# GPflow/GPflow

Measured on AMD Instinct MI355X. Metric: svgp_elbo_steps_per_s, higher is better.
Workload: dtype f64; 1 GPU; SVGP RBF(ARD)+Gaussian ELBO, N=1e+06 M=2048 D=8 P=1 whitened, 8192 minibatch rows per GPU per step (BASELINE metric config Cm); global_batch=8192

## Files before the change

gpflow_amd/_lib.py:

```python
from __future__ import annotations

import ctypes as C
import os
from typing import Optional

_HERE = os.path.dirname(os.path.abspath(__file__))
_LIB_PATH = os.environ.get("GPK_LIBRARY") or os.path.join(_HERE, "libgpk.so")

c_void_p, c_int, c_long, c_double, c_size_t = C.c_void_p, C.c_int, C.c_long, C.c_double, C.c_size_t
_dp = C.c_void_p


class GpkError(RuntimeError):
    pass


_SIGS = {
    "gpk_version": (C.c_char_p, []),
    "gpk_kernel_matrix": (c_int, [c_void_p, c_int, _dp, c_int, c_long, _dp, c_int, c_long, c_int,
                                  C.POINTER(c_double), c_int, c_double, c_double, c_int, _dp, c_long]),
    "gpk_kernel_matrix_hadamard": (c_int, [c_void_p, c_int, _dp, c_int, c_long, _dp, c_int, c_long, c_int,
                                           C.POINTER(c_double), c_int, c_double, _dp, c_long, _dp, c_long]),
    "gpk_kernel_matrix_combine": (c_int, [c_void_p, c_int, c_int, _dp, c_int, c_long, _dp, c_int, c_long, c_int,
                                          C.POINTER(c_double), c_int, c_double, c_double, _dp, c_long, _dp, c_long]),
    "gpk_diag_add": (c_int, [c_void_p, _dp, c_int, c_long, _dp]),
    "gpk_invd_elems": (c_size_t, [c_int, c_int]),
    "gpk_potrf": (c_int, [c_void_p, _dp, c_int, c_int, c_long, c_int, c_long, _dp, c_int, _dp]),
    "gpk_combine_parts": (c_int, [c_void_p, _dp, c_int, c_long, c_int, c_int, c_long, c_double, c_int, c_double, _dp, c_long]),
    "gpk_stream_selfcheck": (c_int, [C.POINTER(c_double), C.POINTER(c_double), C.POINTER(c_int)]),
    "gpk_chain_handoff_mode": (c_int, []),
    "gpk_potrf_inv": (c_int, [c_void_p, _dp, c_int, c_int, c_long, _dp, c_int, _dp]),
    "gpk_trtri_blocks": (c_int, [c_void_p, _dp, c_int, c_long, c_int, c_long, _dp]),
    "gpk_trsm": (c_int, [c_void_p, c_int, _dp, c_long, _dp, c_int, _dp, c_int, c_long, c_int, c_long,
                         c_long]),
    "gpk_transpose_factor": (c_int, [c_void_p, _dp, c_long, _dp, c_int, _dp, c_long, _dp]),
    "gpk_gemm_nt": (c_int, [c_void_p, c_int, c_int, c_int, c_double, _dp, c_long, _dp, c_long, c_double,
                            _dp, c_long, c_int, c_int, c_int, c_long, c_long, c_long]),
    "gpk_transpose": (c_int, [c_void_p, _dp, c_int, c_int, c_long, _dp, c_long, c_int, c_int, c_long,
                              c_long]),
    "gpk_row_stats": (c_int, [c_void_p, _dp, c_int, c_int, c_long, _dp, _dp, c_int, c_double, c_double,
                              _dp, _dp, _dp]),
    "gpk_row_dot": (c_int, [c_void_p, _dp, c_long, _dp, c_long, c_int, c_int, c_double, c_double, _dp]),
    "gpk_row_sumsq": (c_int, [c_void_p, _dp, c_int, c_int, c_long, c_double, c_double, _dp]),
    "gpk_project_workspace_bytes": (c_size_t, [c_int, c_int, c_int]),
    "gpk_project": (c_int, [c_void_p, _dp, c_int, c_int, c_long, _dp, c_long, c_int, _dp, _dp, c_size_t]),
    "gpk_project_batched": (c_int, [c_void_p, _dp, c_int, c_int, c_long, c_long, _dp, c_long, c_int, _dp, _dp, c_size_t]),
    "gpk_reduce_workspace_bytes": (c_size_t, [c_int]),
    "gpk_gaussian_varexp_sum": (c_int, [c_void_p, _dp, c_long, _dp, c_int, c_int, _dp, c_int, _dp,
                                        C.POINTER(c_double), c_int, c_double, _dp, c_double, _dp, _dp, _dp,
                                        c_size_t]),
    "gpk_likelihood_varexp_sum": (c_int, [c_void_p, c_int, C.POINTER(c_double), _dp, c_long, _dp, c_int, c_int, _dp, c_int, _dp,
                                          C.POINTER(c_double), c_int, c_double, _dp, _dp, _dp, _dp, _dp, _dp, c_size_t]),
    "gpk_gauss_hermite": (c_int, [c_int, C.POINTER(c_double), C.POINTER(c_double)]),
    "gpk_gauss_kl_white": (c_int, [c_void_p, _dp, _dp, c_int, c_int, c_int, _dp, _dp, c_size_t]),
    "gpk_sum_log_diag": (c_int, [c_void_p, _dp, c_int, c_long, c_int, c_long, _dp]),
    "gpk_sumsq": (c_int, [c_void_p, _dp, c_int, c_int, c_long, c_int, _dp, _dp, c_size_t]),
    "gpk_gpr_lml_workspace_bytes": (c_size_t, [c_int, c_int, c_int]),
    "gpk_gpr_lml": (c_int, [c_void_p, c_int, _dp, c_int, c_int, c_long, _dp, c_int, c_long,
                            C.POINTER(c_double), c_int, c_double, c_double, _dp, c_double, _dp, _dp, _dp,
                            c_size_t]),
    "gpk_svgp_elbo_workspace_bytes": (c_size_t, [c_int, c_int, c_int, c_int, c_int, c_int]),
    "gpk_svgp_elbo_shard": (c_int, [c_void_p, c_int, _dp, c_int, c_long, _dp, _dp, c_int, c_long, c_long,
                                    c_int, c_int, C.POINTER(c_double), c_int, c_double, c_double, _dp,
                                    c_double, c_double, _dp, _dp, c_int, c_int, _dp, _dp, _dp, c_size_t]),
    "gpk_svgp_elbo_shard_lik": (c_int, [c_void_p, c_int, _dp, c_int, c_long, _dp, _dp, c_int, c_long, c_long, c_int, c_int,
                                        C.POINTER(c_double), c_int, c_double, c_int, C.POINTER(c_double), c_double, c_double,
                                        _dp, _dp, c_int, c_int, _dp, _dp, _dp, c_size_t]),
    "gpk_svgp_elbo_sep_workspace_bytes": (c_size_t, [c_int, c_int, c_int, c_int]),
    "gpk_svgp_elbo_shard_sep": (c_int, [c_void_p, C.POINTER(c_int), _dp, c_int, c_long, c_long, _dp, _dp, c_int, c_long, c_long,
                                        c_int, c_int, C.POINTER(c_double), c_int, C.POINTER(c_double), c_double, _dp, c_double,
                                        c_double, _dp, _dp, _dp, _dp, _dp, c_size_t]),
    "gpk_moment_rows": (c_int, [c_void_p, _dp, c_long, c_int, c_int, _dp, c_long]),
    "gpk_stationary_adjoint_tail": (c_int, [c_void_p, _dp, c_long, _dp, c_long, c_int, c_int, _dp, c_double, c_int, _dp, _dp, c_long,
                                            _dp, c_int, c_double]),
    "gpk_adam_step": (c_int, [c_void_p, _dp, _dp, _dp, _dp, c_long, c_double, c_double, c_double, c_double, c_int]),
    "gpk_lowrank_axpy": (c_int, [c_void_p, c_double, _dp, c_long, _dp, c_long, _dp, c_long, c_int, c_int, c_int, _dp, c_long]),
    "gpk_symmetrize": (c_int, [c_void_p, _dp, c_int, c_long]),
    "gpk_publish_host": (c_int, [c_void_p, _dp, c_int, _dp, c_void_p, c_int]),
    "gpk_profile_gemm_enable": (None, [c_int]),
    "gpk_profile_gemm_collect": (c_int, [C.POINTER(c_double), C.POINTER(c_long), C.POINTER(c_double)]),
    "gpk_profile_gemm_collect_min": (c_int, [c_double, c_int, C.POINTER(c_double), C.POINTER(c_long), C.POINTER(c_double)]),
    "gpk_profile_gemm_collect_kind": (c_int, [c_int, c_double, C.POINTER(c_double), C.POINTER(c_long), C.POINTER(c_double)]),
    "gpk_profile_gemm_window": (c_int, [c_double, C.POINTER(c_double), C.POINTER(c_double), C.POINTER(c_double),
                                        C.POINTER(c_long)]),
    "gpk_bench_mfma_f64": (c_int, [c_void_p, c_int, c_int, _dp]),
    "gpk_bench_stream_store": (c_int, [c_void_p, _dp, c_long]),
}

EXPORTED_SYMBOLS = tuple(sorted(_SIGS))

_lib: Optional[C.CDLL] = None


def lib_path() -> str:
    return _LIB_PATH


def load() -> C.CDLL:
    global _lib
    if _lib is not None:
        return _lib
    if not os.path.exists(_LIB_PATH):
        raise ImportError(
            f"{_LIB_PATH} not found: the HIP extension is not built. Run "
            "`python -c 'import __graft_entry__ as g; g.build()'` (or `make -C gpflow_amd/csrc`). "
            "gpflow_amd has no CPU fallback."
        )
    lib = C.CDLL(_LIB_PATH)
    for name, (res, args) in _SIGS.items():
        fn = getattr(lib, name)
        fn.restype = res
        fn.argtypes = args
    _lib = lib
    return lib


def check(rc: int, what: str) -> None:
    if rc == 0:
        return
    if rc < 0:
        names = {-1: "GPK_E_ARG (bad argument)", -2: "GPK_E_WORKSPACE (workspace too small)",
                 -3: "GPK_E_UNSUPPORTED"}
        raise GpkError(f"{what}: {names.get(rc, rc)}")
    raise GpkError(f"{what}: HIP runtime error {rc}")


def host_doubles(values):
    arr = (c_double * len(values))(*[float(v) for v in values])
    return arr
```

gpflow_amd/csrc/drivers.hip:

```cpp
#include "gpk_internal.h"

extern "C" size_t gpk_project_workspace_bytes(int rows, int m, int P) {
  return (size_t)P * 2 * gpk_gemm_tiles_n(m) * rows * sizeof(double);
}

namespace {
int project_parts(hipStream_t s, const double* At, int rows, int m, long ldat, long strideAt, const double* LqT, long ldl, int P, void* ws,
                  size_t ws_bytes) {
  if ((!At && rows > 0) || !LqT || rows < 0 || m <= 0 || P <= 0 || strideAt < 0) return GPK_E_ARG;
  if (!ws || ws_bytes < gpk_project_workspace_bytes(rows, m, P)) return GPK_E_WORKSPACE;
  if (rows == 0) return 0;
  const int nt = 2 * gpk_gemm_tiles_n(m);
  GemmArgs g = gemm_base(rows, m, m, 1.0, At, ldat, LqT, ldl, 0.0, nullptr, 0, P, strideAt, (long)m * ldl, 0);
  g.b_tri = 1;
  g.epi = 1; g.sq_cols = m; g.c2_cols = 0;
  g.part = (double*)ws; g.part_ld = rows; g.stridePart = (long)nt * rows;
  g.C2 = (double*)ws; g.ldc2 = 0; g.strideC2 = 0;
  return gpk_launch_gemm(s, g);
}
}

extern "C" int gpk_project_batched(void* stream, const double* At, int rows, int m, long ldat, long strideAt,
                                   const double* LqT, long ldl, int P, double* ssq, void* ws, size_t ws_bytes) {
  if (!ssq && rows > 0) return GPK_E_ARG;
  hipStream_t s = (hipStream_t)stream;
  const int rc = project_parts(s, At, rows, m, ldat, strideAt, LqT, ldl, P, ws, ws_bytes);
  if (rc || rows == 0) return rc;
  const int nt = 2 * gpk_gemm_tiles_n(m);
  return gpk_launch_sum_parts(s, (const double*)ws, nt, rows, (long)nt * rows, P, ssq);
}

extern "C" int gpk_project(void* stream, const double* At, int rows, int m, long ldat,
                           const double* LqT, long ldl, int P, double* ssq, void* ws,
                           size_t ws_bytes) {
  return gpk_project_batched(stream, At, rows, m, ldat, 0, LqT, ldl, P, ssq, ws, ws_bytes);
}

namespace {
struct Carver {
  uintptr_t base;
  size_t used = 0;
  double* take(size_t bytes) {
    double* p = (double*)(base + used);
    used += gpk_align_up(bytes, 256);
    return p;
  }
};

int final_one(hipStream_t s, const double* part, int count, double scale, double add, double* out) {
  return gpk_launch_final(s, 1, &part, &count, &scale, add, out);
}
}

namespace {
struct LmlWs {
  long ld;
  double *T, *invd, *part, *logdet;
  size_t total;
};
LmlWs lml_layout(void* ws, int n, int P) {
  LmlWs w{};
  Carver c{(uintptr_t)ws};
  w.ld = (long)gpk_align_up((size_t)n, 8);
  w.T = c.take((size_t)(n + P) * w.ld * sizeof(double));
  w.invd = c.take(gpk_invd_elems(n, 1) * sizeof(double));
  w.part = c.take((size_t)GPK_REDUCE_MAXPART * sizeof(double));
  w.logdet = c.take(256);
  w.total = c.used;
  return w;
}
}

extern "C" size_t gpk_gpr_lml_workspace_bytes(int n, int d, int P) {
  (void)d;
  return lml_layout(nullptr, n, P).total;
}

extern "C" int gpk_gpr_lml(void* stream, int family, const double* X, int n, int d, long ldx,
                           const double* Y, int P, long ldy, const double* ls_host, int ard,
                           double variance, double noise_variance, const double* noise_rows, double mean_const,
                           double* out, int* info, void* ws, size_t ws_bytes) {
  if (!X || !Y || !out || !info || n <= 0 || P <= 0) return GPK_E_ARG;
  const LmlWs w = lml_layout(ws, n, P);
  if (!ws || ws_bytes < w.total) return GPK_E_WORKSPACE;
  hipStream_t s = (hipStream_t)stream;
  int rc;
  rc = gpk_kernel_matrix(stream, family, X, n, ldx, nullptr, 0, 0, d, ls_host, ard, variance,
                         noise_rows ? 0.0 : noise_variance, 1, w.T, w.ld);
  if (rc) return rc;
  if (noise_rows) {
    rc = gpk_diag_add(stream, w.T, n, w.ld, noise_rows);
    if (rc) return rc;
  }
  double* alphaT = w.T + (long)n * w.ld;
  rc = gpk_launch_transpose_shift(s, Y, n, P, ldy, alphaT, w.ld, -mean_const);
  if (rc) return rc;
  rc = gpk_potrf_core(s, w.T, n, P, w.ld, 1, 0, w.invd, 0, info);
  if (rc) return rc;
  rc = gpk_sum_log_diag(stream, w.T, n, w.ld, 1, 0, w.logdet);
  if (rc) return rc;
  int cnt = 0;
  rc = gpk_launch_sumsq_stage1(s, alphaT, P, n, w.ld, 0, w.part, &cnt);
  if (rc) return rc;
  const double* parts[2] = {w.part, w.logdet};
  const int counts[2] = {cnt, 1};
  const double scales[2] = {-0.5, -(double)P};
  const double add = -0.5 * (double)n * (double)P * 1.8378770664093453;
  return gpk_launch_final(s, 2, parts, counts, scales, add, out);
}

namespace {
struct KernelDesc {
  int family, d;
  const double* ls_host;
  int ard;
  double variance;
};
struct ElboArgs {
  KernelDesc k;
  const double* Z; int m; long ldz;
  const double *Xb, *Yb; int rows; long ldxb, ldyb;
  int P;
  const double *q_mu, *q_sqrt; int q_diag;
  double noise_variance; const double* noise_rows;
  double jitter, mean_const;
  double* out; int* info;
  int lik = 0;
  const double* lik_params = nullptr;
};
struct ElboWs {
  long ld, strideT;
  double* T;
  double* Kfu;
  double* arow;
  double* LqT;
  double *invd, *s0, *fmean, *ssq;
  double* proj;
  double *part0, *part1;
  double* part2;
  double* V;
  size_t total;
};

ElboWs elbo_layout(void* ws, int m, int rows, int P, int q_diag, int whiten) {
  ElboWs w{};
  Carver c{(uintptr_t)ws};
  w.ld = (long)gpk_align_up((size_t)m, 8);
  const size_t rows_pad = gpk_align_up((size_t)rows, 32);
  const size_t tail_rows = q_diag ? (whiten ? 0 : (size_t)P + m + 32) : (size_t)P + (size_t)P * m + 32;
  w.T = c.take((m + rows_pad + tail_rows) * w.ld * sizeof(double));
  w.Kfu = w.T + (long)m * w.ld;
  w.arow = w.T + (long)(m + (whiten ? rows_pad : (size_t)rows)) * w.ld;
  w.LqT = w.arow + (long)P * w.ld;
  w.invd = c.take(gpk_invd_elems(m, 1) * sizeof(double));
  w.s0 = c.take((size_t)rows * sizeof(double));
  w.fmean = c.take((size_t)rows * P * sizeof(double));
  w.ssq = c.take((size_t)rows * P * sizeof(double));
  w.proj = c.take(q_diag ? (whiten ? 0 : (size_t)rows * w.ld * sizeof(double)) : gpk_project_workspace_bytes(rows, m, P));
  w.part0 = c.take((size_t)GPK_REDUCE_MAXPART * sizeof(double));
  w.part1 = c.take((size_t)GPK_REDUCE_MAXPART * sizeof(double));
  w.part2 = c.take((size_t)(GPK_REDUCE_MAXPART + 64) * sizeof(double));
  w.V = c.take((size_t)m * P * sizeof(double));
  w.total = c.used;
  return w;
}

ElboWs elbo_sep_layout(void* ws, int m, int rows, int P) {
  ElboWs w{};
  Carver c{(uintptr_t)ws};
  w.ld = (long)gpk_align_up((size_t)m, 8);
  w.strideT = (long)(m + rows) * w.ld;
  w.T = c.take((size_t)P * w.strideT * sizeof(double));
  w.Kfu = w.T + (long)m * w.ld;
  w.invd = c.take(gpk_invd_elems(m, P) * sizeof(double));
  w.LqT = c.take((size_t)P * m * w.ld * sizeof(double));
  w.s0 = c.take((size_t)rows * P * sizeof(double));
  w.fmean = c.take((size_t)rows * P * sizeof(double));
  w.ssq = c.take((size_t)rows * P * sizeof(double));
  w.proj = c.take(gpk_project_workspace_bytes(rows, m, P));
  w.part0 = c.take((size_t)GPK_REDUCE_MAXPART * sizeof(double));
  w.part1 = c.take((size_t)GPK_REDUCE_MAXPART * sizeof(double));
  w.total = c.used;
  return w;
}

bool side_schedule(int m, int rows) { return m > GPK_NB && m < 4096 && rows > 256; }

int build_kuu(hipStream_t ps, const KernelDesc& k, const ElboArgs& a, const double* Z, double* T, long ld) {
  return gpk_kernel_matrix((void*)ps, k.family, Z, a.m, a.ldz, nullptr, 0, 0, k.d, k.ls_host, k.ard, k.variance, a.jitter, 1, T, ld);
}
int build_kfu(hipStream_t xs, const KernelDesc& k, const ElboArgs& a, const double* Z, double* Kfu, long ld) {
  return gpk_kernel_matrix((void*)xs, k.family, a.Xb, a.rows, a.ldxb, Z, a.m, a.ldz, k.d, k.ls_host, k.ard, k.variance, 0.0, 0, Kfu, ld);
}
typedef decltype(&build_kuu) BuildFn;
int build_kfu_and_q_mu_rows(hipStream_t xs, const ElboArgs& a, const ElboWs& w) {
  const int r = build_kfu(xs, a.k, a, a.Z, w.Kfu, w.ld);
  if (r) return r;
  return gpk_transpose((void*)xs, a.q_mu, a.m, a.P, a.P, w.arow, w.ld, 0, 1, 0, 0);
}
int transpose_q_sqrt(hipStream_t s, const ElboArgs& a, const ElboWs& w) {
  return gpk_transpose((void*)s, a.q_sqrt, a.m, a.m, a.m, w.LqT, w.ld, 1, a.P, (long)a.m * a.m, (long)a.m * w.ld);
}

int varexp_to_out(hipStream_t s, const ElboArgs& a, const ElboWs& w, const double* knn_host, int per_latent) {
  int count = 0;
  const int rc = a.lik
      ? gpk_launch_likelihood_varexp_stage1(s, a.lik, a.lik_params, a.Yb, a.ldyb, w.fmean, a.rows, a.P, w.s0, per_latent, w.ssq,
                                            knn_host, per_latent, a.mean_const, nullptr, nullptr, nullptr, nullptr, w.part0, nullptr,
                                            &count)
      : gpk_launch_varexp_stage1(s, a.Yb, a.ldyb, w.fmean, a.rows, a.P, w.s0, per_latent, w.ssq, knn_host, per_latent,
                                 a.noise_variance, a.mean_const, nullptr, w.part0, &count, a.noise_rows);
  if (rc) return rc;
  return final_one(s, w.part0, count, 1.0, 0.0, a.out);
}
int kl_white_to_out(hipStream_t s, const ElboArgs& a, const ElboWs& w) {
  int count = 0;
  const int rc = gpk_launch_kl_white_stage1(s, a.q_mu, a.q_sqrt, a.m, a.P, a.q_diag, w.part1, &count);
  if (rc) return rc;
  return final_one(s, w.part1, count, 0.5, -0.5 * (double)a.m * (double)a.P, a.out + 1);
}
int transpose_q_sqrt_and_kl(hipStream_t s, const ElboArgs& a, const ElboWs& w) {
  if (!a.q_diag) {
    const int r = transpose_q_sqrt(s, a, w);
    if (r) return r;
  }
  return kl_white_to_out(s, a, w);
}

int elbo_whitened(hipStream_t s, const ElboArgs& a, const ElboWs& w) {
  const bool side = side_schedule(a.m, a.rows);
  PotrfHooks hk;
  hk.p_prologue = [&a, &w](hipStream_t ps) { return build_kuu(ps, a.k, a, a.Z, w.T, w.ld); };
  hk.x_prologue = [&a, &w](hipStream_t xs) { return build_kfu(xs, a.k, a, a.Z, w.Kfu, w.ld); };
  if (side) hk.late_work = [&a, &w](hipStream_t bs) { return transpose_q_sqrt_and_kl(bs, a, w); };
  int rc = gpk_potrf_core(s, w.T, a.m, a.rows, w.ld, 1, 0, w.invd, 0, a.info, hk);
  if (rc) return rc;
  rc = gpk_row_stats((void*)s, w.Kfu, a.rows, a.m, w.ld, a.q_mu, a.q_diag ? a.q_sqrt : nullptr, a.P, 1.0, 0.0, w.s0, w.fmean,
                     a.q_diag ? w.ssq : nullptr);
  if (rc) return rc;
  if (!a.q_diag) {
    if (!side) {
      rc = transpose_q_sqrt(s, a, w);
      if (rc) return rc;
    }
    rc = gpk_project((void*)s, w.Kfu, a.rows, a.m, w.ld, w.LqT, w.ld, a.P, w.ssq, w.proj, gpk_project_workspace_bytes(a.rows, a.m, a.P));
    if (rc) return rc;
  }
  rc = varexp_to_out(s, a, w, &a.k.variance, 0);
  if (rc || side) return rc;
  return kl_white_to_out(s, a, w);
}

int elbo_unwhitened_full(hipStream_t s, const ElboArgs& a, const ElboWs& w) {
  const int m = a.m, P = a.P;
  PotrfHooks hk;
  hk.p_prologue = [&a, &w](hipStream_t ps) { return build_kuu(ps, a.k, a, a.Z, w.T, w.ld); };
  hk.x_prologue = [&a, &w](hipStream_t xs) {
    const int r = build_kfu_and_q_mu_rows(xs, a, w);
    return r ? r : transpose_q_sqrt(xs, a, w);
  };
  int rc = gpk_potrf_core(s, w.T, m, a.rows + P + P * m, w.ld, 1, 0, w.invd, 0, a.info, hk, P == 1 ? m : 0, true);
  if (rc) return rc;
  rc = gpk_transpose((void*)s, w.arow, P, m, w.ld, w.V, P, 0, 1, 0, 0);
  if (rc) return rc;
  rc = gpk_row_stats((void*)s, w.Kfu, a.rows, m, w.ld, w.V, nullptr, P, 1.0, 0.0, w.s0, w.fmean, nullptr);
  if (rc) return rc;
  rc = gpk_project((void*)s, w.Kfu, a.rows, m, w.ld, w.LqT, w.ld, P, w.ssq, w.proj, gpk_project_workspace_bytes(a.rows, m, P));
  if (rc) return rc;
  rc = varexp_to_out(s, a, w, &a.k.variance, 0);
  if (rc) return rc;
  int cm = 0, ct = 0;
  rc = gpk_launch_sumsq_stage1(s, w.arow, P, m, w.ld, 0, w.part1, &cm);
  if (rc) return rc;
  rc = gpk_launch_sumsq_stage1(s, w.LqT, P * m, m, w.ld, 0, w.part2, &ct);
  if (rc) return rc;
  double* ldq = w.part2 + GPK_REDUCE_MAXPART;
  double* ldl = ldq + P;
  rc = gpk_launch_sum_log_diag_sq(s, a.q_sqrt, m, m, P, (long)m * m, ldq);
  if (rc) return rc;
  rc = gpk_sum_log_diag((void*)s, w.T, m, w.ld, 1, 0, ldl);
  if (rc) return rc;
  const double* kp[4] = {w.part1, w.part2, ldq, ldl};
  const int kc[4] = {cm, ct, P, 1};
  const double ks[4] = {0.5, 0.5, -0.5, (double)P};
  return gpk_launch_final(s, 4, kp, kc, ks, -0.5 * (double)m * (double)P, a.out + 1);
}

int elbo_unwhitened_diag(hipStream_t s, const ElboArgs& a, const ElboWs& w) {
  const int m = a.m, P = a.P, rows = a.rows;
  double* A2 = w.proj;
  PotrfHooks hk;
  hk.p_prologue = [&a, &w](hipStream_t ps) { return build_kuu(ps, a.k, a, a.Z, w.T, w.ld); };
  hk.x_prologue = [&a, &w](hipStream_t xs) { return build_kfu_and_q_mu_rows(xs, a, w); };
  int rc = gpk_potrf_core(s, w.T, m, rows + P + m, w.ld, 1, 0, w.invd, 0, a.info, hk, m);
  if (rc) return rc;
  if (rows > 0) {
    GemmArgs g = gemm_base(rows, m, m, 1.0, w.Kfu, w.ld, w.LqT, w.ld, 0.0, A2, w.ld, 1, 0, 0, 0);
    g.b_tri = 1;
    rc = gpk_launch_gemm(s, g);
    if (rc) return rc;
    rc = gpk_row_sumsq((void*)s, w.Kfu, rows, m, w.ld, 1.0, 0.0, w.s0);
    if (rc) return rc;
    rc = gpk_row_stats((void*)s, A2, rows, m, w.ld, a.q_mu, a.q_sqrt, P, 1.0, 0.0, nullptr, w.fmean, w.ssq);
    if (rc) return rc;
  }
  rc = varexp_to_out(s, a, w, &a.k.variance, 0);
  if (rc) return rc;
  int cm = 0, ct = 0;
  rc = gpk_launch_sumsq_stage1(s, w.arow, P, m, w.ld, 0, w.part1, &cm);
  if (rc) return rc;
  rc = gpk_launch_kl_unwhite_diag_stage1(s, w.LqT, w.ld, m, a.q_sqrt, P, w.part2, &ct);
  if (rc) return rc;
  double* ldl = w.part2 + GPK_REDUCE_MAXPART;
  rc = gpk_sum_log_diag((void*)s, w.T, m, w.ld, 1, 0, ldl);
  if (rc) return rc;
  const double* kp[3] = {w.part1, w.part2, ldl};
  const int kc[3] = {cm, ct, 1};
  const double ks[3] = {0.5, 0.5, (double)P};
  return gpk_launch_final(s, 3, kp, kc, ks, -0.5 * (double)m * (double)P, a.out + 1);
}
}

extern "C" size_t gpk_svgp_elbo_workspace_bytes(int m, int rows, int d, int P, int q_diag, int whiten) {
  (void)d;
  return elbo_layout(nullptr, m, rows, P, q_diag, whiten).total;
}

namespace {
int elbo_shard(void* stream, const ElboArgs& a, int whiten, void* ws, size_t ws_bytes) {
  if (!a.Z || (a.rows > 0 && (!a.Xb || !a.Yb)) || !a.q_mu || !a.q_sqrt || !a.out || !a.info || a.m <= 0 || a.rows < 0 || a.P <= 0 ||
      a.P > 16)
    return GPK_E_ARG;
  if (a.lik) {
    const int rc = gpk_likelihood_check(a.lik, a.lik_params);
    if (rc) return rc;
  }
  const ElboWs w = elbo_layout(ws, a.m, a.rows, a.P, a.q_diag, whiten);
  if (!ws || ws_bytes < w.total) return GPK_E_WORKSPACE;
  hipStream_t s = (hipStream_t)stream;
  if (whiten) return elbo_whitened(s, a, w);
  return a.q_diag ? elbo_unwhitened_diag(s, a, w) : elbo_unwhitened_full(s, a, w);
}
}

extern "C" int gpk_svgp_elbo_shard(void* stream, int family, const double* Z, int m, long ldz,
                                   const double* Xb, const double* Yb, int rows, long ldxb,
                                   long ldyb, int d, int P, const double* ls_host, int ard,
                                   double variance, double noise_variance, const double* noise_rows, double jitter,
                                   double mean_const, const double* q_mu, const double* q_sqrt,
                                   int q_diag, int whiten, double* out, int* info, void* ws,
                                   size_t ws_bytes) {
  const ElboArgs a{{family, d, ls_host, ard, variance}, Z, m, ldz, Xb, Yb, rows, ldxb, ldyb, P, q_mu, q_sqrt, q_diag,
                   noise_variance, noise_rows, jitter, mean_const, out, info};
  return elbo_shard(stream, a, whiten, ws, ws_bytes);
}

extern "C" int gpk_svgp_elbo_shard_lik(void* stream, int family, const double* Z, int m, long ldz, const double* Xb,
                                       const double* Yb, int rows, long ldxb, long ldyb, int d, int P, const double* ls_host,
                                       int ard, double variance, int lik, const double* lik_params_host, double jitter,
                                       double mean_const, const double* q_mu, const double* q_sqrt, int q_diag, int whiten,
                                       double* out, int* info, void* ws, size_t ws_bytes) {
  if (!lik) return GPK_E_UNSUPPORTED;
  ElboArgs a{{family, d, ls_host, ard, variance}, Z, m, ldz, Xb, Yb, rows, ldxb, ldyb, P, q_mu, q_sqrt, q_diag,
             0.0, nullptr, jitter, mean_const, out, info};
  a.lik = lik; a.lik_params = lik_params_host;
  return elbo_shard(stream, a, whiten, ws, ws_bytes);
}

extern "C" size_t gpk_svgp_elbo_sep_workspace_bytes(int m, int rows, int d, int P) {
  (void)d;
  return elbo_sep_layout(nullptr, m, rows, P).total;
}

extern "C" int gpk_svgp_elbo_shard_sep(void* stream, const int* family_host, const double* Z, int m, long ldz, long strideZ,
                                       const double* Xb, const double* Yb, int rows, long ldxb, long ldyb, int d, int P,
                                       const double* ls_host, int ard, const double* variance_host, double noise_variance,
                                       const double* noise_rows, double jitter, double mean_const, const double* q_mu,
                                       const double* q_sqrt, double* out,
                                       int* info, void* ws, size_t ws_bytes) {
  if (!family_host || !Z || (rows > 0 && (!Xb || !Yb)) || !q_mu || !q_sqrt || !ls_host || !variance_host || !out || !info || m <= 0 || rows < 0 ||
      P <= 0 || P > 16 || d <= 0 || strideZ < 0)
    return GPK_E_ARG;
  const ElboWs w = elbo_sep_layout(ws, m, rows, P);
  if (!ws || ws_bytes < w.total) return GPK_E_WORKSPACE;
  const ElboArgs a{{0, d, ls_host, ard, 0.0}, Z, m, ldz, Xb, Yb, rows, ldxb, ldyb, P, q_mu, q_sqrt, 0,
                   noise_variance, noise_rows, jitter, mean_const, out, info};
  hipStream_t s = (hipStream_t)stream;
  const int nls = ard ? d : 1;
  auto each_latent = [&](BuildFn build, hipStream_t st, double* T0) -> int {
    for (int p = 0; p < P; ++p) {
      const KernelDesc kp{family_host[p], d, ls_host + (long)p * nls, ard, variance_host[p]};
      const int r = build(st, kp, a, Z + (long)p * strideZ, T0 + (long)p * w.strideT, w.ld);
      if (r) return r;
    }
    return 0;
  };
  const bool side = side_schedule(m, rows);
  PotrfHooks hk;
  hk.p_prologue = [&](hipStream_t ps) { return each_latent(build_kuu, ps, w.T); };
  hk.x_prologue = [&](hipStream_t xs) { return each_latent(build_kfu, xs, w.Kfu); };
  if (side) hk.late_work = [&a, &w](hipStream_t bs) { return transpose_q_sqrt_and_kl(bs, a, w); };
  int rc = gpk_potrf_core(s, w.T, m, rows, w.ld, P, w.strideT, w.invd, 0, info, hk);
  if (rc) return rc;
  if (!side) {
    rc = transpose_q_sqrt_and_kl(s, a, w);
    if (rc) return rc;
  }
  rc = gpk_launch_row_stats_sep(s, w.Kfu, w.strideT, rows, m, w.ld, q_mu, P, w.s0, w.fmean);
  if (rc) return rc;
  rc = gpk_project_batched(stream, w.Kfu, rows, m, w.ld, w.strideT, w.LqT, w.ld, P, w.ssq, w.proj,
                           gpk_project_workspace_bytes(rows, m, P));
  if (rc) return rc;
  return varexp_to_out(s, a, w, variance_host, 1);
}
```

gpflow_amd/csrc/gemm.hip:

```cpp
#include "gpk_internal.h"
#include <mutex>
#include <stdlib.h>
#include <algorithm>
#include <type_traits>

namespace {

constexpr int BK = 16;
constexpr int LDSS = BK + 2;
thread_local int g_last_kind = 0;
constexpr int GROUP_N = 8;

template <int BM, int BN, int WGM, int WGN>
struct TileCfg {
  static constexpr int WM = BM / WGM, WN = BN / WGN;
  static constexpr int TM = WM / 16, TN = WN / 16;
  static constexpr int A_CH = BM * (BK / 2) / 256;
  static constexpr int B_CH = BN * (BK / 2) / 256;
  static constexpr size_t LDS_BYTES = 2 * (size_t)(BM + BN) * LDSS * sizeof(double);
};

__device__ __forceinline__ void tile_decode(int nl, int gx, int gy, int compact, int& tile_m, int& tile_n) {
  tile_m = 0; tile_n = 0;
  if (compact) {
// ... 282 lines not shown
#pragma unroll
        for (int i = 0; i < TM; ++i)
#pragma unroll
          for (int r = 0; r < 4; ++r) {
            const int row = row_base + i * 16 + 4 * r;
            double s = smem[wn * BM + (row - m0)];
#pragma unroll
            for (int u = 1; u < WPS; ++u) s += smem[(wn + u) * BM + (row - m0)];
            if (row < p.m) part[(long)(tile_n * (BN / 64) + (wn * WN) / 64) * p.part_ld + row] = s;
          }
      }
    }
  }
}


__global__ __launch_bounds__(256, 2) void gemm_nt_pre64(GemmArgs p, int gx, int gy, int total, int compact) {
  constexpr int BM = 64, BN = 64, MAXS = 8;
  constexpr int BUF = (BM + BN) * LDSS;
  extern __shared__ __attribute__((aligned(16))) double smem[];
  if (p.sig_ptr && threadIdx.x == 0 && blockIdx.x == 0 && blockIdx.y == 0)
    __hip_atomic_store(p.sig_ptr, p.sig_val, __ATOMIC_RELAXED, __HIP_MEMORY_SCOPE_SYSTEM);

  const int tid = threadIdx.x, lane = tid & 63, wave = tid >> 6;
  const int bz = blockIdx.y;
  int tile_m, tile_n;
  tile_order(blockIdx.x, 0, gx, gy, total, compact, tile_m, tile_n);
  const int m0 = tile_m * BM, n0 = tile_n * BN;
  if (p.c_lower && n0 > m0 + BM - 1) return;
  if (m0 >= p.m || n0 >= p.n) return;
  const double* __restrict__ A = p.A + (long)bz * p.strideA;
  const double* __restrict__ B = p.B + (long)bz * p.strideB;
  double* __restrict__ C = p.C + (long)bz * p.strideC;
  const int nkt = p.k / BK;

  d2 ra[MAXS][2], rb[MAXS][2];
  const double* pa[2];
  const double* pb[2];
  bool va[2], vb[2];
#pragma unroll
  for (int q = 0; q < 2; ++q) {
    const int c = tid + 256 * q;
    const int rowa = m0 + (c >> 3), rowb = n0 + (c >> 3);
    va[q] = rowa < p.m;
    vb[q] = rowb < p.n;
    pa[q] = A + (long)(va[q] ? rowa : p.m - 1) * p.lda + (c & 7) * 2;
    pb[q] = B + (long)(vb[q] ? rowb : p.n - 1) * p.ldb + (c & 7) * 2;
  }
#pragma unroll
  for (int s = 0; s < MAXS; ++s)
    if (s < nkt) {
#pragma unroll
      for (int q = 0; q < 2; ++q) {
        ra[s][q] = *reinterpret_cast<const d2*>(pa[q] + s * BK);
        rb[s][q] = *reinterpret_cast<const d2*>(pb[q] + s * BK);
      }
    }
  const int row_base = m0 + wave * 16 + (lane >> 4);
  const int col_base = n0 + (lane & 15);
  const double alpha = p.alpha, beta = p.beta;
  double cpre[4][4];
#pragma unroll
  for (int r = 0; r < 4; ++r)
#pragma unroll
    for (int j = 0; j < 4; ++j) {
      const int row = row_base + 4 * r, col = col_base + j * 16;
      cpre[r][j] = (beta != 0.0 && row < p.m && col < p.n) ? C[(long)row * p.ldc + col] : 0.0;
    }

  const d2 zero2 = {0.0, 0.0};
  auto lstore = [&](int buf, const d2 (&xa)[2], const d2 (&xb)[2]) {
#pragma unroll
    for (int q = 0; q < 2; ++q) {
      const int c = tid + 256 * q;
      *reinterpret_cast<d2*>(&smem[buf * BUF + (c >> 3) * LDSS + (c & 7) * 2]) = va[q] ? xa[q] : zero2;
      *reinterpret_cast<d2*>(&smem[buf * BUF + (BM + (c >> 3)) * LDSS + (c & 7) * 2]) = vb[q] ? xb[q] : zero2;
    }
  };
  d4 acc[4];
#pragma unroll
  for (int j = 0; j < 4; ++j) acc[j] = (d4){0.0, 0.0, 0.0, 0.0};
  if (nkt > 0) {
    lstore(0, ra[0], rb[0]);
    __syncthreads();
  }
  const int frag_r = lane & 15, frag_k = lane >> 4;
#pragma unroll
  for (int kt = 0; kt < MAXS; ++kt)
    if (kt < nkt) {
      const int cur = kt & 1;
      const double* as = smem + cur * BUF + (wave * 16 + frag_r) * LDSS + frag_k;
      const double* bs = smem + cur * BUF + (BM + frag_r) * LDSS + frag_k;
#pragma unroll
      for (int kk = 0; kk < BK / 4; ++kk) {
        const double a = as[kk * 4];
        double b[4];
#pragma unroll
        for (int j = 0; j < 4; ++j) b[j] = bs[j * 16 * LDSS + kk * 4];
#pragma unroll
        for (int j = 0; j < 4; ++j) acc[j] = __builtin_amdgcn_mfma_f64_16x16x4f64(a, b[j], acc[j], 0, 0, 0);
      }
      if (kt + 1 < MAXS && kt + 1 < nkt) lstore(cur ^ 1, ra[kt + 1 < MAXS ? kt + 1 : 0], rb[kt + 1 < MAXS ? kt + 1 : 0]);
      __syncthreads();
    }
#pragma unroll
  for (int r = 0; r < 4; ++r) {
    const int row = row_base + 4 * r;
    if (row < p.m) {
#pragma unroll
      for (int j = 0; j < 4; ++j) {
        const int col = col_base + j * 16;
        if (col < p.n) {
          double v = alpha * acc[j][r];
          if (beta != 0.0) v += beta * cpre[r][j];
          C[(long)row * p.ldc + col] = v;
        }
      }
    }
  }
}

bool pre64_ok(const GemmArgs& a) {
  if (a.epi != 0 || a.k <= 0 || a.k > 128 || (a.k & 15) || a.b_tri || a.a_tri || a.k_off_step || a.tile_snake || a.tail_first1) return false;
  if ((a.lda & 1) || (a.ldb & 1) || (a.strideA & 1) || (a.strideB & 1)) return false;
  if ((reinterpret_cast<uintptr_t>(a.A) & 15) || (reinterpret_cast<uintptr_t>(a.B) & 15)) return false;
  return true;
}

int launch_pre64(hipStream_t s, const GemmArgs& a) {
  constexpr size_t LDS_BYTES = 2 * (size_t)(64 + 64) * LDSS * sizeof(double);
  const int gx = gpk_cdiv(a.n, 64), gy = gpk_cdiv(a.m, 64);
  if (gx <= 0 || gy <= 0) return 0;
  int total = gx * gy, compact = 0;
  if (a.c_lower) {
    compact = 1;
    total = 0;
    for (int first = 0; first < gx; first += GROUP_N) {
      const int gsz = (gx - first) < GROUP_N ? (gx - first) : GROUP_N;
      const int avail = gy - first;
      if (avail <= 0) break;
      const int tr = avail < gsz ? avail : gsz;
      total += tr * (tr + 1) / 2 + (avail > gsz ? (avail - gsz) * gsz : 0);
    }
    if (total <= 0) return 0;
  }
  g_last_kind = 6;
  hipLaunchKernelGGL(gemm_nt_pre64, dim3((unsigned)total, (unsigned)(a.batch > 0 ? a.batch : 1), 1), dim3(256), LDS_BYTES, s, a, gx, gy,
                     total, compact);
  GPK_LAUNCH_CHECK();
  return 0;
}


template <int EPI>
__device__ __forceinline__ void fast_tile(const GemmArgs& p, int tile_m, int tile_n, double* smem, int rev = 0, int bz_queue = -1) {
  constexpr int BM = 128, BN = 128;
  constexpr int BUF = (BM + BN) * LDSS;
  const int tid = threadIdx.x, lane = tid & 63, wave = tid >> 6;
  const int wm = wave >> 1, wn = wave & 1;
  const int bz = bz_queue >= 0 ? bz_queue : (p.k_off_step ? (int)gridDim.y - 1 - (int)blockIdx.y : (int)blockIdx.y);
  const int m0 = tile_m * BM, n0 = tile_n * BN;
  if (p.c_lower && n0 > m0 + BM - 1) return;

  const double* __restrict__ A = p.A + (long)bz * p.strideA;
  const double* __restrict__ B = p.B + (long)bz * p.strideB;
  int kb = 0, ke = p.k;
  const int koff = bz * p.k_off_step;
  if (p.b_tri && (n0 + BN < p.n ? n0 + BN : p.n) <= p.b_tri_rows) {
    if (p.b_tri == 1) {
      const int f = n0 + p.b_tri_off - koff;
      kb = (f > 0 ? f : 0) & ~(BK - 1);
    } else {
      const int l = n0 + BN + p.b_tri_off - koff;
      ke = l < p.k ? l : p.k;
    }
  }
  if (p.a_tri == 1) {
    int f = m0 - koff;
    f = (f > 0 ? f : 0) & ~(BK - 1);
    kb = kb > f ? kb : f;
  } else if (p.a_tri == 2) {
    int l = ((m0 + BM + BK - 1) & ~(BK - 1)) - koff;
    l = l < p.k ? l : p.k;
    ke = ke < l ? ke : l;
  }
  const int nk = ke > kb ? (ke - kb) / BK : 0;

  const int srow = tid >> 3, scol = (tid & 7) * 2;
  const int mrows = p.m - m0, nrows = p.n - n0;
  const char* abase = reinterpret_cast<const char*>(A + (long)m0 * p.lda + kb);
  const char* bbase = reinterpret_cast<const char*>(B + (long)n0 * p.ldb + kb);
  unsigned oa[4], ob[4];
#pragma unroll
  for (int q = 0; q < 4; ++q) {
    int ra = srow + 32 * q, rb = srow + 32 * q;
    ra = ra < mrows ? ra : mrows - 1;
    rb = rb < nrows ? rb : nrows - 1;
    oa[q] = (unsigned)(((long)ra * p.lda + scol) * 8);
    ob[q] = (unsigned)(((long)rb * p.ldb + scol) * 8);
  }
  const int woff = srow * LDSS + scol;
  d2 st[8];
  auto gload = [&](int s) {
    const long so = rev ? (long)(nk - 1 - s) : (long)s;
    const char* ab = abase + so * (BK * 8);
    const char* bb = bbase + so * (BK * 8);
#pragma unroll
    for (int q = 0; q < 4; ++q) st[q] = *reinterpret_cast<const d2*>(ab + oa[q]);
#pragma unroll
    for (int q = 0; q < 4; ++q) st[4 + q] = *reinterpret_cast<const d2*>(bb + ob[q]);
  };
  auto lstore1 = [&](int buf, int q) {
    const int row = (q < 4) ? 32 * q : BM + 32 * (q - 4);
    *reinterpret_cast<d2*>(&smem[buf * BUF + row * LDSS + woff]) = st[q];
  };

  d4 acc[4][4];
  const int lane_c = lane & 15, lane_g = lane >> 4;
  const int row_base = m0 + wm * 64 + lane_c;
  const int col_base = n0 + wn * 64 + 2 * lane_g;
  const bool load_c = (p.beta != 0.0) && (EPI == 0 || p.C != nullptr);
  if (nk > 0) gload(0);
  const int c_r0 = wm * 64 + lane_c, c_c0 = wn * 64 + 2 * lane_g;
  const int c_rmax = p.m - 1 - m0, c_cmax = p.n - 1 - n0;
  auto c_roff = [&](int i) -> unsigned {
    const int rr = c_r0 + 16 * i;
    return (unsigned)(((long)(rr < c_rmax ? rr : c_rmax) * p.ldc) * 8);
  };
  auto c_coff = [&](int j, int h) -> unsigned {
    const int c = c_c0 + j * 16 + 8 * h;
    return (unsigned)((c < c_cmax ? c : c_cmax) * 8);
  };
  const bool c_vec = (EPI == 0 || p.C != nullptr) && (n0 + BN <= p.n) && !(p.ldc & 1) && !(p.strideC & 1) &&
                     !(reinterpret_cast<uintptr_t>(p.C) & 15);
  if (load_c) {
    const double* __restrict__ C = p.C + (long)bz * p.strideC;
    const double sc = p.beta / p.alpha;
    const char* cb = reinterpret_cast<const char*>(C + (long)m0 * p.ldc + n0);
    if (c_vec) {
#pragma unroll
      for (int i = 0; i < 4; ++i) {
        const char* rowp = cb + c_roff(i);
#pragma unroll
        for (int j = 0; j < 4; ++j) {
          const d2 lo = *reinterpret_cast<const d2*>(rowp + c_coff(j, 0));
          const d2 hi = *reinterpret_cast<const d2*>(rowp + c_coff(j, 1));
          acc[i][j] = (d4){sc * lo.x, sc * lo.y, sc * hi.x, sc * hi.y};
        }
      }
    } else {
#pragma unroll
      for (int i = 0; i < 4; ++i) {
        const char* rowp = cb + c_roff(i);
#pragma unroll
        for (int j = 0; j < 4; ++j)
#pragma unroll
          for (int r = 0; r < 4; ++r) {
            const int c = c_c0 + j * 16 + 8 * (r >> 1) + (r & 1);
            acc[i][j][r] = sc * *reinterpret_cast<const double*>(rowp + (unsigned)((c < c_cmax ? c : c_cmax) * 8));
          }
      }
    }
  } else {
#pragma unroll
    for (int i = 0; i < 4; ++i)
#pragma unroll
      for (int j = 0; j < 4; ++j) acc[i][j] = (d4){0.0, 0.0, 0.0, 0.0};
  }

  const int bperm = 2 * (lane_c & 3) + ((lane_c >> 2) & 1) + 8 * (lane_c >> 3);
  const double* as = smem + (wm * 64 + lane_c) * LDSS + lane_g;
  const double* bs = smem + (BM + wn * 64 + bperm) * LDSS + lane_g;
  double fa[2][4], fb[2][4];
  auto fload = [&](int buf, int kk, int f) {
#pragma unroll
    for (int i = 0; i < 4; ++i) fa[f][i] = as[buf * BUF + i * 16 * LDSS + kk * 4];
#pragma unroll
    for (int j = 0; j < 4; ++j) fb[f][j] = bs[buf * BUF + j * 16 * LDSS + kk * 4];
  };
#define GPK_MFMA_ROW(f, i)                                                                         \
  _Pragma("unroll") for (int j = 0; j < 4; ++j) acc[i][j] =                                       \
      __builtin_amdgcn_mfma_f64_16x16x4f64(fb[f][j], fa[f][i], acc[i][j], 0, 0, 0)

  if (nk > 0) {
#pragma unroll
    for (int q = 0; q < 8; ++q) lstore1(0, q);
    __syncthreads();
    fload(0, 0, 0);
  }
  auto slab = [&](int s, auto more_tag) {
    constexpr bool MORE = decltype(more_tag)::value;
    const int cur = s & 1;
    if constexpr (MORE) gload(s + 1);
    fload(cur, 1, 1);
#pragma unroll
    for (int i = 0; i < 4; ++i) { GPK_MFMA_ROW(0, i); }
    if constexpr (MORE) __builtin_amdgcn_sched_group_barrier(0x020, 8, 0);
    __builtin_amdgcn_sched_group_barrier(0x100, 8, 0);
    __builtin_amdgcn_sched_group_barrier(0x008, 16, 0);
    __builtin_amdgcn_sched_barrier(0);
    fload(cur, 2, 0);
#pragma unroll
    for (int i = 0; i < 4; ++i) { GPK_MFMA_ROW(1, i); }
    __builtin_amdgcn_sched_group_barrier(0x100, 8, 0);
    __builtin_amdgcn_sched_group_barrier(0x008, 16, 0);
    __builtin_amdgcn_sched_barrier(0);
    fload(cur, 3, 1);
    if constexpr (MORE) {
#pragma unroll
      for (int q = 0; q < 8; ++q) lstore1(cur ^ 1, q);
    }
#pragma unroll
    for (int i = 0; i < 4; ++i) { GPK_MFMA_ROW(0, i); }
    __builtin_amdgcn_sched_group_barrier(0x100, 8, 0);
    if constexpr (MORE) {
      __builtin_amdgcn_sched_group_barrier(0x008, 4, 0);
#pragma unroll
      for (int q = 0; q < 8; ++q) {
        __builtin_amdgcn_sched_group_barrier(0x200, 1, 0);
        __builtin_amdgcn_sched_group_barrier(0x008, 1, 0);
      }
      __builtin_amdgcn_sched_group_barrier(0x008, 4, 0);
    } else {
      __builtin_amdgcn_sched_group_barrier(0x008, 16, 0);
    }
    __builtin_amdgcn_sched_barrier(0);
    if constexpr (MORE) __syncthreads();
    if constexpr (MORE) fload(cur ^ 1, 0, 0);
#pragma unroll
    for (int i = 0; i < 4; ++i) { GPK_MFMA_ROW(1, i); }
    if constexpr (MORE) __builtin_amdgcn_sched_group_barrier(0x100, 8, 0);
    __builtin_amdgcn_sched_group_barrier(0x008, 16, 0);
    __builtin_amdgcn_sched_barrier(0);
  };
  for (int s = 0; s + 1 < nk; ++s) slab(s, std::true_type{});
  if (nk > 0) slab(nk - 1, std::false_type{});
#undef GPK_MFMA_ROW

  if constexpr (EPI == 0) {
    double* __restrict__ C = p.C + (long)bz * p.strideC;
    const double alpha = p.alpha;
    char* cb = reinterpret_cast<char*>(C + (long)m0 * p.ldc + n0);
#pragma unroll
    for (int i = 0; i < 4; ++i) {
      if (c_r0 + 16 * i <= c_rmax) {
        char* rowp = cb + c_roff(i);
        if (c_vec) {
#pragma unroll
          for (int j = 0; j < 4; ++j) {
            *reinterpret_cast<d2*>(rowp + c_coff(j, 0)) = (d2){alpha * acc[i][j][0], alpha * acc[i][j][1]};
            *reinterpret_cast<d2*>(rowp + c_coff(j, 1)) = (d2){alpha * acc[i][j][2], alpha * acc[i][j][3]};
          }
        } else {
#pragma unroll
          for (int j = 0; j < 4; ++j)
#pragma unroll
            for (int r = 0; r < 4; ++r) {
              const int c = c_c0 + j * 16 + 8 * (r >> 1) + (r & 1);
              if (c <= c_cmax) *reinterpret_cast<double*>(rowp + (unsigned)(c * 8)) = alpha * acc[i][j][r];
            }
        }
      }
    }
  } else {
    double* __restrict__ C2 = p.C2 + (long)bz * p.strideC2;
    double* __restrict__ part = p.part + (long)bz * p.stridePart;
    const double alpha = p.alpha;
#pragma unroll
    for (int i = 0; i < 4; ++i) {
      const int row = row_base + i * 16;
      double s = 0.0;
#pragma unroll
      for (int j = 0; j < 4; ++j)
#pragma unroll
        for (int r = 0; r < 4; ++r) {
          const int col = col_base + j * 16 + 8 * (r >> 1) + (r & 1);
          const double v = alpha * acc[i][j][r];
          if (col < p.sq_cols) {
            s += v * v;
          } else if (row < p.m && col - p.sq_cols < p.c2_cols && col < p.n) {
            C2[(long)row * p.ldc2 + (col - p.sq_cols)] = v;
          }
        }
      s += __shfl_xor(s, 16);
      s += __shfl_xor(s, 32);
      if (lane_g == 0 && row < p.m) part[(long)(tile_n * 2 + wn) * p.part_ld + row] = s;
    }
  }
}


template <int EPI, bool PAIR, bool QUEUE = false>
__global__ __launch_bounds__(256, 2) void gemm_nt_fast(GemmArgs p, int gx, int gy, int total, int compact) {
  extern __shared__ __attribute__((aligned(16))) double smem[];
  if (p.sig_ptr && threadIdx.x == 0 && blockIdx.x == 0 && blockIdx.y == 0)
    __hip_atomic_store(p.sig_ptr, p.sig_val, __ATOMIC_RELAXED, __HIP_MEMORY_SCOPE_SYSTEM);
  if constexpr (!PAIR) {
    if (p.stagger_ticks > 0 && (int)blockIdx.x >= p.stagger_first && (int)blockIdx.x < 2 * p.stagger_first && blockIdx.y == 0) {
      const long long t0 = wall_clock64();
      while (wall_clock64() - t0 < p.stagger_ticks) __builtin_amdgcn_s_sleep(32);
    }
    if constexpr (QUEUE) {
      volatile int* s_next = reinterpret_cast<volatile int*>(&smem[BK]);
      const int nbatch = p.batch > 0 ? p.batch : 1;
      const int all = total * nbatch;
      for (;;) {
        if (threadIdx.x == 0) *s_next = (int)((unsigned)atomicAdd(p.queue, 1) - (unsigned)p.queue_base);
        __syncthreads();
        const int t = *s_next;
        __syncthreads();
        if (t >= all || t < 0) break;
        const int zq = t / total, tq = t - zq * total;
        int tile_m, tile_n;
        tile_order(tq, p.b_tri, gx, gy, total, compact, tile_m, tile_n);
        fast_tile<EPI>(p, tile_m, tile_n, smem, 0, nbatch - 1 - zq);
      }
      return;
    }
    for (int t = blockIdx.x; t < total; t += gridDim.x) {
      int tile_m, tile_n;
      if (EPI == 1 && p.tile_snake) {
        const int q = t / gy, half = gx >> 1;
        tile_m = t - q * gy;
        tile_n = q < half ? q : gx - 1 - (q - half);
      } else if (p.k_off_step) {
        int tt = t + (int)blockIdx.y * (total / (int)gridDim.y);
        if (tt >= total) tt -= total;
        tile_order(tt, p.b_tri, gx, gy, total, compact, tile_m, tile_n);
      } else {
        tile_order(t, p.b_tri, gx, gy, total, compact, tile_m, tile_n);
      }
      fast_tile<EPI>(p, tile_m, tile_n, smem);
      if (t + (int)gridDim.x < total) __syncthreads();
    }
  } else {
    const int align = (EPI == 1 && p.b_tri == 1) ? p.pair_k_align : 0;
    const int tile_m = blockIdx.x % gy, j = blockIdx.x / gy;
    fast_tile<EPI>(p, tile_m, j, smem, align);
    if (gx - 1 - j != j) {
      __syncthreads();
      fast_tile<EPI>(p, tile_m, gx - 1 - j, smem, 0);
    }
  }
}

int queue_slot(unsigned fetches, int** out, unsigned* base) {
  constexpr int kRing = 1024, kMaxDev = 16;
  static std::mutex mu;
  static int* ring[kMaxDev] = {};
  static unsigned* value[kMaxDev] = {};
  static unsigned next[kMaxDev] = {};
  int dev = 0;
  GPK_HIP(hipGetDevice(&dev));
  if (dev < 0 || dev >= kMaxDev) return GPK_E_UNSUPPORTED;
  std::lock_guard<std::mutex> lock(mu);
  if (!ring[dev]) {
    GPK_HIP(hipMalloc((void**)&ring[dev], sizeof(int) * kRing));
    GPK_HIP(hipMemset(ring[dev], 0, sizeof(int) * kRing));
    value[dev] = (unsigned*)calloc(kRing, sizeof(unsigned));
    if (!value[dev]) return GPK_E_ARG;
  }
  const unsigned slot = next[dev]++ % kRing;
  *out = ring[dev] + slot;
  *base = value[dev][slot];
  value[dev][slot] += fetches;
  return 0;
}

template <int EPI>
int launch_fast(hipStream_t s, const GemmArgs& a) {
  constexpr size_t LDS_BYTES = 2 * (size_t)256 * LDSS * sizeof(double);
  static const hipError_t attr0 = hipFuncSetAttribute(reinterpret_cast<const void*>(gemm_nt_fast<EPI, false>),
                                                      hipFuncAttributeMaxDynamicSharedMemorySize, 160 * 1024);
  static const hipError_t attr1 = hipFuncSetAttribute(reinterpret_cast<const void*>(gemm_nt_fast<EPI, true>),
                                                      hipFuncAttributeMaxDynamicSharedMemorySize, (int)LDS_BYTES);
  GPK_HIP(attr0);
  GPK_HIP(attr1);
  const int gx = gpk_cdiv(a.n, 128), gy = gpk_cdiv(a.m, 128);
  if (gx <= 0 || gy <= 0) return 0;
  int total = gx * gy, compact = 0;
  if (a.c_lower && EPI == 0) {
    compact = 1;
    total = 0;
    for (int first = 0; first < gx; first += GROUP_N) {
      const int gsz = (gx - first) < GROUP_N ? (gx - first) : GROUP_N;
      const int avail = gy - first;
      if (avail <= 0) break;
      const int tr = avail < gsz ? avail : gsz;
      total += tr * (tr + 1) / 2 + (avail > gsz ? (avail - gsz) * gsz : 0);
    }
    if (total <= 0) return 0;
  }
  const unsigned nb = (unsigned)(a.batch > 0 ? a.batch : 1);
  {
    const bool pair_ok = (EPI == 1) ? (a.b_tri == 1)
                                    : ((a.b_tri == 1 || a.b_tri == 2) && !a.c_lower && a.max_wgs == 0 && a.b_tri_off == 0 && a.k_off_step == 0);
    if (EPI == 1 && pair_ok && gx >= 4 && !(gx & 1) && a.b_tri_rows >= a.n && a.max_wgs == 0 &&
        (long)(gx / 2) * gy * nb <= GPK_TUNE(PROJ_UNPAIR_UPTO, 256)) {
      GemmArgs b = a;
      b.tile_snake = 1;
      b.stagger_first = 256;
      b.stagger_ticks = 0;
      g_last_kind = 2 + 2 * EPI;
      hipLaunchKernelGGL((gemm_nt_fast<EPI, false>), dim3((unsigned)total, nb, 1), dim3(256), LDS_BYTES, s, b, gx, gy, total, compact);
      GPK_LAUNCH_CHECK();
      return 0;
    }
    if (pair_ok && gx >= 4 && a.b_tri_rows >= a.n) {
      total = ((gx + 1) / 2) * gy;
      g_last_kind = 2 + 2 * EPI + 1;
      GemmArgs ap = a;
      ap.pair_k_align = GPK_TUNE(PAIR_K_ALIGN, 1);
      hipLaunchKernelGGL((gemm_nt_fast<EPI, true>), dim3((unsigned)total, nb, 1), dim3(256), LDS_BYTES, s, ap, gx, gy,
                         total, compact);
      GPK_LAUNCH_CHECK();
      return 0;
    }
  }
  int tail_tiles = 0;
  if (EPI == 0 && !a.c_lower && a.max_wgs > 0 && a.max_wgs < total && nb == 1 && !a.b_tri && !a.a_tri &&
      GPK_TUNE(TAIL_SPLIT_CAPPED, 1)) {
    const int r = total % a.max_wgs;
    if (r > 0 && r * 100 <= a.max_wgs * GPK_TUNE(TAIL_SPLIT_CAPPED_PCT, 60)) tail_tiles = r;
  }
  const int total_all = total;
  total -= tail_tiles;
  unsigned nwg = (unsigned)total;
  if (a.max_wgs > 0 && (unsigned)a.max_wgs < nwg) nwg = (unsigned)a.max_wgs;
  GemmArgs b = a;
  g_last_kind = 2 + 2 * EPI;
  {
    const int stagger_on = GPK_TUNE(GEMM_STAGGER, 100);
    if (b.stagger_first <= 0) b.stagger_first = 256;
    b.stagger_ticks = (stagger_on && EPI == 0 && !a.b_tri && total >= 1024 && (nwg == (unsigned)total || nwg >= 2u * (unsigned)b.stagger_first))
                          ? (int)((a.k / 16) * 170 * stagger_on / 200)
                          : 0;
  }
  size_t lds_bytes = LDS_BYTES;
  if (EPI == 0 && a.max_wgs > 0 && nwg < (unsigned)total && nb == 1) {
    const int kb = GPK_TUNE(CAP_EXCL_LDS_KB, 84);
    if (kb > 0 && kb <= 160 && (size_t)kb * 1024 > LDS_BYTES) lds_bytes = (size_t)kb * 1024;
  }
  if (EPI == 0 && tail_tiles == 0 && a.max_wgs == 0 &&
      ((a.k_off_step && GPK_TUNE(KSPLIT_QUEUE, 1)) || (a.tile_queue && (long)total * nb > 512))) {
    b.stagger_ticks = 0;
    const long all = (long)total * nb;
    const long qw = a.stagger_first > 0 ? 2L * a.stagger_first : GPK_TUNE(QUEUE_WGS, 512);
    const unsigned wgs = (unsigned)(all < qw ? all : qw);
    int* q = nullptr;
    unsigned qbase = 0;
    const int rcq = queue_slot((unsigned)all + wgs, &q, &qbase);
    if (rcq) return rcq;
    b.queue = q;
    b.queue_base = (int)qbase;
    if constexpr (EPI == 0) {
      static const hipError_t attrq = hipFuncSetAttribute(reinterpret_cast<const void*>(gemm_nt_fast<0, false, true>),
                                                          hipFuncAttributeMaxDynamicSharedMemorySize, (int)LDS_BYTES);
      GPK_HIP(attrq);
      hipLaunchKernelGGL((gemm_nt_fast<0, false, true>), dim3(wgs, 1, 1), dim3(256), LDS_BYTES, s, b, gx, gy, total, compact);
    }
    GPK_LAUNCH_CHECK();
    return 0;
  }
  hipLaunchKernelGGL((gemm_nt_fast<EPI, false>), dim3(nwg, nb, 1), dim3(256), lds_bytes, s, b, gx, gy, total,
                     compact);
  GPK_LAUNCH_CHECK();
  if (tail_tiles > 0) {
    using Cfg = TileCfg<64, 64, 4, 1>;
    static const hipError_t attrt = hipFuncSetAttribute(reinterpret_cast<const void*>(gemm_nt_kernel<64, 64, 4, 1>),
                                                        hipFuncAttributeMaxDynamicSharedMemorySize, (int)Cfg::LDS_BYTES);
    GPK_HIP(attrt);
    GemmArgs t = a;
    t.tail_first1 = total_all - tail_tiles + 1;
    hipLaunchKernelGGL((gemm_nt_kernel<64, 64, 4, 1>), dim3((unsigned)(4 * tail_tiles), 1, 1), dim3(256), Cfg::LDS_BYTES, s, t, gx,
                       gy, 4 * tail_tiles, compact);
    GPK_LAUNCH_CHECK();
  }
  return 0;
}

bool fast_ok(const GemmArgs& a) {
  if (GPK_TUNE(GEMM_NO_FAST, 0)) return false;
  if (a.k <= 0 || (a.k & 15) || (a.b_tri && (a.b_tri_off & 15))) return false;
  if ((a.lda & 1) || (a.ldb & 1) || (a.strideA & 1) || (a.strideB & 1)) return false;
  if ((reinterpret_cast<uintptr_t>(a.A) & 15) || (reinterpret_cast<uintptr_t>(a.B) & 15)) return false;
  if (a.epi == 0 && a.beta != 0.0 && a.alpha == 0.0) return false;
  if (a.lda > (1L << 21) || a.ldb > (1L << 21)) return false;
  return true;
}


constexpr int SM_BM = 16, SM_BN = 128, SM_THREADS = 512;

__global__ __launch_bounds__(SM_THREADS) void gemm_nt_small(GemmArgs p, int ldk) {
  extern __shared__ __attribute__((aligned(16))) double smem[];
  const int tid = threadIdx.x, lane = tid & 63;
  const int wave = __builtin_amdgcn_readfirstlane(tid >> 6);
  const int bz = blockIdx.z;
  const int n0 = blockIdx.x * SM_BN;
  const double* __restrict__ A = p.A + (long)bz * p.strideA;
  const double* __restrict__ B = p.B + (long)bz * p.strideB;
  int kb = 0, ke = p.k;
  if (p.b_tri && (n0 + SM_BN < p.n ? n0 + SM_BN : p.n) <= p.b_tri_rows) {
    if (p.b_tri == 1) {
      const int f = n0 + p.b_tri_off;
      kb = (f > 0 ? f : 0) & ~(BK - 1);
    } else {
      const int l = n0 + SM_BN + p.b_tri_off;
      ke = l < p.k ? l : p.k;
    }
  }
  const int kc = ke > kb ? ke - kb : 0;
  double* As = smem;
  double* Bs = smem + SM_BM * ldk;
  const int r = lane & 15, g = lane >> 4;
  const int col = n0 + wave * 16 + r;
  double* __restrict__ C = p.C + (long)bz * p.strideC;
  if (p.sig_ptr && tid == 0 && blockIdx.x == 0 && blockIdx.y == 0 && blockIdx.z == 0)
    __hip_atomic_store(p.sig_ptr, p.sig_val, __ATOMIC_RELAXED, __HIP_MEMORY_SCOPE_SYSTEM);
  if (p.wait_ptr) {
    if (tid == 0) {
      const long long t0 = wall_clock64();
      bool timed_out = false;
      while ((int)(__hip_atomic_load(p.wait_ptr, __ATOMIC_RELAXED, __HIP_MEMORY_SCOPE_SYSTEM) - p.wait_val) < 0) {
        if (wall_clock64() - t0 >= 50000000LL) { timed_out = true; break; }
        __builtin_amdgcn_s_sleep(2);
      }
      if (timed_out && p.wait_info) atomicMax(p.wait_info, 0x7fffffff);
    }
    __syncthreads();
    __builtin_amdgcn_fence(__ATOMIC_ACQUIRE, "agent");
  }
  const int nmb = (p.m + SM_BM - 1) / SM_BM;
  bool first = true;
  for (int mb = blockIdx.y; mb < nmb; mb += gridDim.y) {
    const int m0 = mb * SM_BM;
    if (p.c_lower && n0 > m0 + SM_BM - 1) continue;
    d4 acc0 = {0.0, 0.0, 0.0, 0.0}, acc1 = {0.0, 0.0, 0.0, 0.0};
    if (p.beta != 0.0) {
      const double sc = p.beta / p.alpha;
      const int cc = col < p.n ? col : p.n - 1;
#pragma unroll
      for (int e = 0; e < 4; ++e) {
        int row = m0 + g + 4 * e;
        row = row < p.m ? row : p.m - 1;
        acc0[e] = sc * C[(long)row * p.ldc + cc];
      }
    }
    if (2 * lane < kc) {
      for (int q = wave; q < (first ? SM_BM + SM_BN : SM_BM); q += SM_THREADS / 64) {
        const double* src;
        if (q < SM_BM) {
          int rr = m0 + q;
          rr = rr < p.m ? rr : p.m - 1;
          src = A + (long)rr * p.lda + kb;
        } else {
          int rr = n0 + q - SM_BM;
          rr = rr < p.n ? rr : p.n - 1;
          src = B + (long)rr * p.ldb + kb;
        }
        __builtin_amdgcn_global_load_lds((const __attribute__((address_space(1))) void*)(src + 2 * lane),
                                         (__attribute__((address_space(3))) void*)(smem + q * ldk), 16, 0, 0);
      }
    }
    __builtin_amdgcn_s_waitcnt(0x0070);
    __syncthreads();
    const double* ap = As + r * ldk + g;
    const double* bp = Bs + (wave * 16 + r) * ldk + g;
    const int nkk = kc >> 2;
#pragma unroll 4
    for (int kk = 0; kk < nkk; kk += 2) {
      const double a0 = ap[kk * 4], b0 = bp[kk * 4];
      const double a1 = ap[kk * 4 + 4], b1 = bp[kk * 4 + 4];
      acc0 = __builtin_amdgcn_mfma_f64_16x16x4f64(a0, b0, acc0, 0, 0, 0);
      acc1 = __builtin_amdgcn_mfma_f64_16x16x4f64(a1, b1, acc1, 0, 0, 0);
    }
    first = false;
    if (col < p.n) {
#pragma unroll
      for (int e = 0; e < 4; ++e) {
        const int row = m0 + g + 4 * e;
        if (row < p.m) C[(long)row * p.ldc + col] = p.alpha * (acc0[e] + acc1[e]);
      }
    }
    if (mb + (int)gridDim.y < nmb) __syncthreads();
  }
}

int launch_small(hipStream_t s, const GemmArgs& a) {
  const int ldk = a.k + 2;
  const size_t lds = (size_t)(SM_BM + SM_BN) * ldk * sizeof(double);
  static const hipError_t attr = hipFuncSetAttribute(reinterpret_cast<const void*>(gemm_nt_small),
                                                     hipFuncAttributeMaxDynamicSharedMemorySize,
                                                     (int)((SM_BM + SM_BN) * 130 * sizeof(double)));
  GPK_HIP(attr);
  unsigned gy = (unsigned)gpk_cdiv(a.m, SM_BM);
  const unsigned gxs = (unsigned)gpk_cdiv(a.n, SM_BN);
  if (a.max_wgs > 0 && gy * gxs > (unsigned)a.max_wgs) gy = ((unsigned)a.max_wgs + gxs - 1) / gxs;
  else if (a.small_loop && a.max_wgs <= 0 && gy * gxs > 512u) gy = (512u + gxs - 1) / gxs;
  dim3 grid(gxs, gy, (unsigned)(a.batch > 0 ? a.batch : 1));
  g_last_kind = 1;
  hipLaunchKernelGGL(gemm_nt_small, grid, dim3(SM_THREADS), lds, s, a, ldk);
  GPK_LAUNCH_CHECK();
  return 0;
}

struct GroupSolveArgs {
  const double* E; long lde;
  double* Eo; long ldeo;
  const double* L; long ldl;
  const double* X;
  int rows, nb;
  long strideE, strideEo, strideL, strideX;
  int j0, j1;
};

__global__ __launch_bounds__(512) void group_solve_kernel(GroupSolveArgs p) {
  constexpr int LDK = 130, NBK = 128;
  {
// ... 352 lines not shown
  GemmArgs b = a;
  unsigned gridx = (unsigned)total;
  if (b.tile_snake) {
    const int nbatch = a.batch > 0 ? a.batch : 1;
    if (a.b_tri != 1 || compact || total < 256 || (total == 256 && nbatch < 2)) b.tile_snake = 0;
    else if ((gy & 7) == 0 && (total & 255) == 0) b.tile_snake = 2;
    else if (nbatch == 1) { b.tile_snake = 1; gridx = (unsigned)((total + 255) & ~255); }
    else b.tile_snake = 0;
  }
  dim3 grid(gridx, (unsigned)(a.batch > 0 ? a.batch : 1), 1);
  g_last_kind = 6;
  hipLaunchKernelGGL((gemm_nt_kernel<BM, BN, WGM, WGN>), grid, dim3(256), Cfg::LDS_BYTES, s, b, gx, gy, total,
                     compact);
  GPK_LAUNCH_CHECK();
  return 0;
}

}

int gpk_gemm_tiles_n(int n) { return gpk_cdiv(n, 128); }
bool gpk_gemm_takes_latency_kernel(const GemmArgs& a) { return a.m > 0 && a.n > 0 && !a.no_small && small_ok(a); }

int gpk_launch_group_solve(hipStream_t s, const double* E, long lde, double* Eo, long ldeo, int rows, const double* Lgg, long ldl,
                           const double* X, int nb, int batch, long strideE, long strideEo, long strideL, long strideX, int max_wgs,
                           int j0, int j1) {
  return launch_group_solve(s, E, lde, Eo, ldeo, rows, Lgg, ldl, X, nb, batch, strideE, strideEo, strideL, strideX, max_wgs, j0, j1);
}

namespace {
struct ProfRec { hipEvent_t e0, e1; double flops; int kind; };
bool g_prof_on = false;
ProfRec* g_prof = nullptr;
int g_prof_n = 0, g_prof_cap = 0;

double algorithmic_flops(const GemmArgs& a) {
  const double m = a.m, n = a.n, k = a.k;
  double outs = m * n;
  if (a.c_lower) outs = (m >= n) ? n * (n + 1) / 2 + (m - n) * n : m * (m + 1) / 2;
  double kk = k;
  if (a.b_tri) {
    const double nn = (a.b_tri_rows < a.n ? a.b_tri_rows : a.n);
    const double tri = (nn <= k) ? nn * (nn + 1) / 2 + nn * (k - nn) : k * (k + 1) / 2;
    return 2.0 * m * (tri + (n - nn) * k) * (a.batch > 0 ? a.batch : 1);
  }
  return 2.0 * outs * kk * (a.batch > 0 ? a.batch : 1);
}
}

int gpk_profile_gemm_is_on() { return g_prof_on ? 1 : 0; }

extern "C" void gpk_profile_gemm_enable(int on) {
  g_prof_on = on != 0;
  g_prof_n = 0;
}

extern "C" int gpk_profile_gemm_collect_min(double min_flops, int keep, double* total_ms, long* launches,
                                            double* flops) {
  GPK_HIP(hipDeviceSynchronize());
  double ms = 0.0, fl = 0.0;
  long cnt = 0;
  for (int i = 0; i < g_prof_n; ++i) {
    if (g_prof[i].flops < min_flops) continue;
    float t = 0.f;
    GPK_HIP(hipEventElapsedTime(&t, g_prof[i].e0, g_prof[i].e1));
    ms += t;
    fl += g_prof[i].flops;
    ++cnt;
  }
  if (total_ms) *total_ms = ms;
  if (launches) *launches = cnt;
  if (flops) *flops = fl;
  if (!keep) g_prof_n = 0;
  return 0;
}
extern "C" int gpk_profile_gemm_window(double min_flops, double* window_ms, double* flops_all, double* flops_matching,
                                       long* launches_all) {
  GPK_HIP(hipDeviceSynchronize());
  int first = -1, last = -1;
  for (int i = 0; i < g_prof_n; ++i)
    if (g_prof[i].flops >= min_flops) { if (first < 0) first = i; last = i; }
  double fa = 0.0, fm = 0.0;
  float t = 0.f;
  long cnt = 0;
  if (first >= 0) {
    GPK_HIP(hipEventElapsedTime(&t, g_prof[first].e0, g_prof[last].e1));
    for (int i = first; i <= last; ++i) {
      fa += g_prof[i].flops;
      if (g_prof[i].flops >= min_flops) fm += g_prof[i].flops;
      ++cnt;
    }
  }
  if (window_ms) *window_ms = t;
  if (flops_all) *flops_all = fa;
  if (flops_matching) *flops_matching = fm;
  if (launches_all) *launches_all = cnt;
  return 0;
}
extern "C" int gpk_profile_gemm_collect_kind(int kind, double min_flops, double* total_ms, long* launches, double* flops) {
  GPK_HIP(hipDeviceSynchronize());
  double ms = 0.0, fl = 0.0;
  long cnt = 0;
  for (int i = 0; i < g_prof_n; ++i) {
    if (g_prof[i].kind != kind || g_prof[i].flops < min_flops) continue;
    float t = 0.f;
    GPK_HIP(hipEventElapsedTime(&t, g_prof[i].e0, g_prof[i].e1));
    ms += t;
    fl += g_prof[i].flops;
    ++cnt;
  }
  if (total_ms) *total_ms = ms;
  if (launches) *launches = cnt;
  if (flops) *flops = fl;
  return 0;
}
extern "C" int gpk_profile_gemm_collect(double* total_ms, long* launches, double* flops) {
  return gpk_profile_gemm_collect_min(0.0, 0, total_ms, launches, flops);
}

static int launch_select(hipStream_t s, const GemmArgs& a);

static int prof_grow() {
  const int cap = g_prof_cap ? 2 * g_prof_cap : 1024;
  ProfRec* p = (ProfRec*)realloc(g_prof, sizeof(ProfRec) * cap);
  if (!p) return GPK_E_ARG;
  g_prof = p;
  for (int i = g_prof_cap; i < cap; ++i) {
    if (hipEventCreate(&p[i].e0) != hipSuccess) return i > g_prof_n ? 0 : GPK_E_ARG;
    if (hipEventCreate(&p[i].e1) != hipSuccess) {
      (void)hipEventDestroy(p[i].e0);
      return i > g_prof_n ? 0 : GPK_E_ARG;
    }
    g_prof_cap = i + 1;
  }
  return 0;
}

int gpk_launch_gemm(hipStream_t s, const GemmArgs& a) {
  if (a.m <= 0 || a.n <= 0) return 0;
  if (!g_prof_on) return launch_select(s, a);
  if (g_prof_n == g_prof_cap) {
    const int rcg = prof_grow();
    if (rcg) return rcg;
    if (g_prof_n == g_prof_cap) return GPK_E_ARG;
  }
  ProfRec& r = g_prof[g_prof_n++];
  r.flops = algorithmic_flops(a);
  GPK_HIP(hipEventRecord(r.e0, s));
  const int rc = launch_select(s, a);
  r.kind = g_last_kind;
  GPK_HIP(hipEventRecord(r.e1, s));
  return rc;
}

static int launch_select(hipStream_t s, const GemmArgs& a) {
  const long tiles = (long)gpk_cdiv(a.m, 128) * gpk_cdiv(a.n, 128) * (a.batch > 0 ? a.batch : 1);
  if (a.tile64 && a.epi == 0) {
    if (GPK_TUNE(REST_PRE64, 1) && pre64_ok(a)) return launch_pre64(s, a);
    return launch_cfg<64, 64, 4, 1>(s, a);
  }
  if (!a.no_small && small_ok(a)) return launch_small(s, a);
  if (a.epi == 1 && a.beta != 0.0 && a.C && !fast_ok(a)) return GPK_E_UNSUPPORTED;
  if (a.epi == 0 && a.k >= GPK_TUNE(HALF_TILE_KMIN, 1024) && a.m > 64 && a.n > 64 && (a.max_wgs == 0 || a.max_wgs >= tiles)) {
    const long eff = a.c_lower ? tiles / 2 : tiles;
    if (eff < GPK_TUNE(HALF_TILE_BELOW, 300)) return launch_cfg<64, 128, 1, 4>(s, a);
  }
  if (a.epi == 1 && a.b_tri == 1 && !(a.beta != 0.0 && a.C) && a.m > 64) {
    const long pairs = (long)((gpk_cdiv(a.n, 128) + 1) / 2) * gpk_cdiv(a.m, 128) * (a.batch > 0 ? a.batch : 1);
    if (pairs < GPK_TUNE(PROJ_SMALL_TILE_BELOW, 200)) {
      GemmArgs b = a;
      b.tile_snake = GPK_TUNE(PROJ_SNAKE, 1);
      if (gpk_cdiv(a.n, 64) == 2 * gpk_cdiv(a.n, 128)) {
        if (pairs < GPK_TUNE(PROJ_TILE32_BELOW, 100)) return launch_cfg<32, 64, 2, 2>(s, b);
        return launch_cfg<64, 64, 4, 1>(s, b);
      }
      return launch_cfg<64, 128, 2, 2>(s, b);
    }
  }
  if (fast_ok(a) && (a.epi == 1 || (a.n > 64 && (tiles >= 24 || a.m <= 64)))) {
    return a.epi == 1 ? launch_fast<1>(s, a) : launch_fast<0>(s, a);
  }
  if (a.epi == 1) return launch_cfg<128, 128, 2, 2>(s, a);
  if (a.n <= 64) return launch_cfg<128, 64, 2, 2>(s, a);
  const long tiles128 = (long)gpk_cdiv(a.m, 128) * gpk_cdiv(a.n, 128) * (a.batch > 0 ? a.batch : 1);
  if (tiles128 < 192 && a.m > 64) return launch_cfg<64, 128, 1, 4>(s, a);
  return launch_cfg<128, 128, 2, 2>(s, a);
}


namespace {
__global__ __launch_bounds__(256) void gemm_nt_empty_k_kernel(double* __restrict__ C, int row0, int n, long ldc, long strideC,
                                                              double beta, int c_lower) {
  double* Cz = C + (long)blockIdx.z * strideC;
  const int i = row0 + (int)blockIdx.y;
  for (int j = blockIdx.x * 256 + threadIdx.x; j < n; j += gridDim.x * 256) {
    if (c_lower && (j & ~127) > (i & ~127)) continue;
    double* c = Cz + (long)i * ldc + j;
    *c = beta != 0.0 ? beta * *c : 0.0;
  }
}
}

extern "C" int gpk_gemm_nt(void* stream, int m, int n, int k, double alpha, const double* A,
                           long lda, const double* B, long ldb, double beta, double* C, long ldc,
                           int b_tri, int c_lower, int batch, long strideA, long strideB,
                           long strideC) {
  if (m < 0 || n < 0 || k < 0 || batch < 0) return GPK_E_ARG;
  if ((b_tri & ~0x133) || (b_tri & 3) == 3 || ((b_tri >> 4) & 3) == 3 || ((b_tri & 0x100) && (k & 15))) return GPK_E_ARG;
  if (m == 0 || n == 0) return 0;
  if (!C) return GPK_E_ARG;
  if (k == 0) {
    const int nbatch = batch > 0 ? batch : 1;
    if (nbatch > 65535) return GPK_E_ARG;
    for (int i0 = 0; i0 < m; i0 += 65535) {
      dim3 grid((unsigned)std::min(gpk_cdiv(n, 256), 64), (unsigned)std::min(m - i0, 65535), (unsigned)nbatch);
      hipLaunchKernelGGL(gemm_nt_empty_k_kernel, grid, dim3(256), 0, (hipStream_t)stream, C, i0, n, ldc,
                         nbatch > 1 ? strideC : 0L, beta, c_lower);
      GPK_LAUNCH_CHECK();
    }
    return 0;
  }
  if (!A || !B) return GPK_E_ARG;
  GemmArgs g{};
  g.A = A; g.lda = lda; g.strideA = strideA;
  g.B = B; g.ldb = ldb; g.strideB = strideB;
  g.C = C; g.ldc = ldc; g.strideC = strideC;
  g.m = m; g.n = n; g.k = k; g.alpha = alpha; g.beta = beta;
  g.c_lower = c_lower; g.b_tri = b_tri & 3; g.b_tri_off = 0; g.b_tri_rows = n;
  const int ksplit = (b_tri >> 8) & 1;
  g.a_tri = (m <= k * (ksplit ? (batch > 0 ? batch : 1) : 1)) ? ((b_tri >> 4) & 3) : 0;
  g.k_off_step = ksplit ? k : 0;
  g.epi = 0; g.batch = batch > 0 ? batch : 1;
  if (kGpkExp) g.max_wgs = GPK_TUNE(GEMM_NT_MAX_WGS, 0);
  return gpk_launch_gemm((hipStream_t)stream, g);
}
```

gpflow_amd/csrc/gpk_internal.h:

```cpp
#pragma once
#include <hip/hip_runtime.h>
#include <stdint.h>
#include <stddef.h>
#include <functional>
#include "../../include/gpk.h"

typedef double d4 __attribute__((ext_vector_type(4)));
typedef double d2 __attribute__((ext_vector_type(2)));

#include <stdio.h>
#include <stdlib.h>

#ifdef GPK_EXPERIMENTAL
#define GPK_TUNE(name, def)                                                                      \
  ([]() -> int {                                                                                 \
    static const int v__ = getenv("GPK_" #name) ? atoi(getenv("GPK_" #name)) : (int)(def);       \
    return v__;                                                                                  \
  }())
#define GPK_TRACE(...)                                        \
  do {                                                        \
    if (GPK_TUNE(DEBUG, 0)) fprintf(stderr, "[gpk] " __VA_ARGS__); \
  } while (0)
#else
#define GPK_TUNE(name, def) ((int)(def))
#define GPK_TRACE(...) do { } while (0)
#endif

#ifdef GPK_EXPERIMENTAL
constexpr bool kGpkExp = true;
#else
constexpr bool kGpkExp = false;
#endif

#define GPK_HIP(call)                                                                                   \
  do {                                                                                                  \
    hipError_t e__ = (call);                                                                            \
    if (e__ != hipSuccess) {                                                                            \
      GPK_TRACE("%s:%d: %s -> %d\n", __FILE__, __LINE__, #call, (int)e__);                              \
      return (int)e__;                                                                                  \
    }                                                                                                   \
  } while (0)
#define GPK_LAUNCH_CHECK()                                                                              \
  do {                                                                                                  \
    hipError_t e__ = hipGetLastError();                                                                 \
    if (e__ != hipSuccess) {                                                                            \
      GPK_TRACE("%s:%d: kernel launch -> %d\n", __FILE__, __LINE__, (int)e__);                          \
      return (int)e__;                                                                                  \
    }                                                                                                   \
  } while (0)

static inline size_t gpk_align_up(size_t x, size_t a) { return (x + a - 1) / a * a; }
static inline int gpk_cdiv(int a, int b) { return (a + b - 1) / b; }

struct GemmArgs {
  const double* A; long lda; long strideA;
  const double* B; long ldb; long strideB;
  double* C; long ldc; long strideC;
  int m, n, k;
  double alpha, beta;
  int c_lower;
  int b_tri;
  int a_tri;
  int b_tri_off;
  int b_tri_rows;
  int k_off_step;
  int epi;
  int sq_cols;
  double* part; long part_ld; long stridePart;
  double* C2; long ldc2; long strideC2; int c2_cols;
  int batch;
  int stagger_first;
  int stagger_ticks;
  int no_small;
  int small_loop;
  int max_wgs;
  int pair_k_align;
  int* sig_ptr; int sig_val;
  const int* wait_ptr; int wait_val;
  int* wait_info;
  int tile_queue;
  int* queue; int queue_base;
  int tile64;
  int tile_snake;
  int tail_first1;
};
static inline GemmArgs gemm_base(int m, int n, int k, double alpha, const double* A, long lda,
                                 const double* B, long ldb, double beta, double* C, long ldc, int batch,
                                 long sA, long sB, long sC) {
  GemmArgs g{};
  g.A = A; g.lda = lda; g.strideA = sA;
  g.B = B; g.ldb = ldb; g.strideB = sB;
  g.C = C; g.ldc = ldc; g.strideC = sC;
  g.m = m; g.n = n; g.k = k; g.alpha = alpha; g.beta = beta;
  g.b_tri_rows = n; g.batch = batch > 0 ? batch : 1;
  return g;
}
int gpk_launch_gemm(hipStream_t s, const GemmArgs& a);
bool gpk_gemm_takes_latency_kernel(const GemmArgs& a);

int gpk_launch_group_solve(hipStream_t s, const double* E, long lde, double* Eo, long ldeo, int rows, const double* Lgg, long ldl,
                           const double* X, int nb, int batch = 1, long strideE = 0, long strideEo = 0, long strideL = 0,
                           long strideX = 0, int max_wgs = 0, int j0 = 0, int j1 = -1);
int gpk_gemm_tiles_n(int n);
int gpk_profile_gemm_is_on();

int gpk_launch_leaf(hipStream_t s, double* A, long lda, long strideA, int nb, double* invd,
                    long strideInv, int* info, int col0, int batch, int already_factored);

typedef std::function<int(hipStream_t)> StreamWork;
struct PotrfHooks {
  StreamWork x_prologue, p_prologue, late_work;
};
int gpk_potrf_core(hipStream_t S, double* A, int n, int extra, long lda, int batch, long strideA, double* invd, int zero_upper,
                   int* info, const PotrfHooks& hooks = PotrfHooks(), int tri = 0, bool tri_prefilled = false);


int gpk_launch_zero_upper(hipStream_t s, double* A, int n, long lda, int batch, long strideA);
int gpk_launch_set_identity(hipStream_t s, double* A, int n, long lda, int batch = 1, long strideA = 0);
int gpk_probe_concurrent_kernels(hipStream_t a, hipStream_t b, int* scratch, int* concurrent);
int gpk_launch_noop(hipStream_t s);
int gpk_launch_wait_flag(hipStream_t s, const int* ptr, int val, int* info);
int gpk_launch_set_flag(hipStream_t s, int* ptr, int val);
int gpk_launch_sum_parts(hipStream_t s, const double* part, int nt, int rows, long stridePart, int P,
                         double* ssq);
int gpk_launch_final(hipStream_t s, int nterms, const double* const* part, const int* count,
                     const double* scale, double add, double* out);
int gpk_launch_sumsq_stage1(hipStream_t s, const double* A, int rows, int cols, long lda,
                            int upper_only, double* part, int* count);
int gpk_launch_varexp_stage1(hipStream_t s, const double* Y, long ldy, const double* fmean, int rows,
                             int P, const double* s0, int s0_per_latent, const double* ssq,
                             const double* knn_host, int knn_per_latent, double noise,
                             double mean_const, double* fvar_out, double* part, int* count,
                             const double* noise_rows = nullptr);
int gpk_likelihood_check(int lik, const double* params);
int gpk_launch_likelihood_varexp_stage1(hipStream_t s, int lik, const double* params, const double* Y, long ldy, const double* fmean,
                                        int rows, int P, const double* s0, int s0_per_latent, const double* ssq,
                                        const double* knn_host, int knn_per_latent, double mean_const, double* fvar_out,
                                        double* rows_out, double* dmu_out, double* dvar_out, double* part, double* part1, int* count);
int gpk_launch_kl_white_stage1(hipStream_t s, const double* q_mu, const double* q_sqrt, int m, int P,
                               int q_diag, double* part, int* count);
int gpk_launch_kl_unwhite_diag_stage1(hipStream_t s, const double* LinvT, long ldl, int m, const double* W, int P, double* part,
                                      int* count);
int gpk_launch_sum_log_diag_sq(hipStream_t s, const double* L, int n, long ldl, int batch, long strideL, double* out);
int gpk_launch_row_stats_sep(hipStream_t s, const double* At, long strideAt, int rows, int m, long ldat, const double* V, int P,
                             double* sumsq, double* mv);
int gpk_launch_transpose_shift(hipStream_t s, const double* in, int rows, int cols, long ldin,
                               double* out, long ldout, double shift);
#define GPK_REDUCE_MAXPART 1024
```

gpflow_amd/csrc/reduce.hip:

```cpp
#include "gpk_internal.h"

namespace {

constexpr int RB = 256;
constexpr int MAXPART = 1024;

__device__ __forceinline__ double wave_sum(double v) {
#pragma unroll
  for (int o = 32; o > 0; o >>= 1) v += __shfl_down(v, o);
  return v;
}
__device__ __forceinline__ double block_sum(double v, double* sh) {
  v = wave_sum(v);
  const int lane = threadIdx.x & 63, w = threadIdx.x >> 6;
  __syncthreads();
  if (lane == 0) sh[w] = v;
  __syncthreads();
  double r = 0.0;
  if (threadIdx.x == 0) {
    const int nw = (blockDim.x + 63) >> 6;
    for (int i = 0; i < nw; ++i) r += sh[i];
  }
  return r;
}
// ... 51 lines not shown
  const int bx = blockIdx.x * 32, by = blockIdx.y * 32;
  const int tx = threadIdx.x & 31, ty = threadIdx.x >> 5;
  for (int k = ty; k < 32; k += 8) {
    const int r = by + k, c = bx + tx;
    tile[k][tx] = (r < rows && c < cols) ? in[(long)r * ldin + c] + shift : 0.0;
  }
  __syncthreads();
  for (int k = ty; k < 32; k += 8) {
    const int r = bx + k, c = by + tx;
    if (r < cols && c < rows) out[(long)r * ldout + c] = tile[tx][k];
  }
}

template <int PC>
__global__ __launch_bounds__(256) void row_stats_kernel(const double* __restrict__ At, int rows,
                                                        int m, long ldat,
                                                        const double* __restrict__ V,
                                                        const double* __restrict__ W, int P, int p0,
                                                        double alpha, double beta,
                                                        double* __restrict__ sumsq,
                                                        double* __restrict__ mv,
                                                        double* __restrict__ wsq) {
  const int lane = threadIdx.x & 63, w = threadIdx.x >> 6;
  const int row = blockIdx.x * 4 + w;
  if (row >= rows) return;
  const double* a = At + (long)row * ldat;
  double s = 0.0, dv[PC], dw[PC];
#pragma unroll
  for (int q = 0; q < PC; ++q) { dv[q] = 0.0; dw[q] = 0.0; }
  for (int k = lane; k < m; k += 64) {
    const double x = a[k];
    s = fma(x, x, s);
#pragma unroll
    for (int q = 0; q < PC; ++q) {
      if (p0 + q < P) {
        if (V) dv[q] = fma(x, V[(long)k * P + p0 + q], dv[q]);
        if (W) { const double t = x * W[(long)k * P + p0 + q]; dw[q] = fma(t, t, dw[q]); }
      }
    }
  }
  s = wave_sum(s);
#pragma unroll
  for (int q = 0; q < PC; ++q) { dv[q] = wave_sum(dv[q]); dw[q] = wave_sum(dw[q]); }
  if (lane == 0) {
    if (sumsq && p0 == 0) sumsq[row] = (beta != 0.0 ? beta * sumsq[row] : 0.0) + alpha * s;
#pragma unroll
    for (int q = 0; q < PC; ++q)
      if (p0 + q < P) {
        if (V && mv) mv[(long)row * P + p0 + q] = dv[q];
        if (W && wsq) wsq[(long)(p0 + q) * rows + row] = dw[q];
      }
  }
}

__global__ __launch_bounds__(256) void row_stats_sep_kernel(const double* __restrict__ At, long strideAt, int rows, int m, long ldat,
                                                            const double* __restrict__ V, int P, double* __restrict__ sumsq,
                                                            double* __restrict__ mv) {
  const int lane = threadIdx.x & 63, w = threadIdx.x >> 6;
  const int row = blockIdx.x * 4 + w, p = blockIdx.y;
  if (row >= rows) return;
  const double* a = At + (long)p * strideAt + (long)row * ldat;
  double s = 0.0, dv = 0.0;
  for (int k = lane; k < m; k += 64) {
    const double x = a[k];
    s = fma(x, x, s);
    dv = fma(x, V[(long)k * P + p], dv);
  }
  s = wave_sum(s);
  dv = wave_sum(dv);
  if (lane == 0) {
    sumsq[(long)p * rows + row] = s;
    mv[(long)row * P + p] = dv;
  }
}

__global__ __launch_bounds__(256) void row_dot_kernel(const double* __restrict__ A, long lda,
                                                      const double* __restrict__ B, long ldb, int rows,
                                                      int cols, double alpha, double beta,
                                                      double* __restrict__ out) {
  const int lane = threadIdx.x & 63, w = threadIdx.x >> 6;
  const int row = blockIdx.x * 4 + w;
  if (row >= rows) return;
  const double* a = A + (long)row * lda;
  const double* b = B + (long)row * ldb;
  double s = 0.0;
  for (int k = lane; k < cols; k += 64) s = fma(a[k], b[k], s);
  s = wave_sum(s);
  if (lane == 0) out[row] = (beta != 0.0 ? beta * out[row] : 0.0) + alpha * s;
}

__global__ void sum_parts_kernel(const double* part, int nt, int rows, long stridePart, double* ssq) {
  const int b = blockIdx.x * blockDim.x + threadIdx.x, p = blockIdx.y;
  if (b >= rows) return;
  const double* q = part + (long)p * stridePart;
  double s = 0.0;
  for (int t = 0; t < nt; ++t) s += q[(long)t * rows + b];
  ssq[(long)p * rows + b] = s;
}

template <int NP>
__global__ __launch_bounds__(256) void combine_parts_kernel(const double* __restrict__ part, int np, long stridePart, int m,
                                                           int n, long ldp, double alpha, int lower, double diag_scale,
                                                           double* __restrict__ out, long ldo) {
  const int c = (blockIdx.x * 256 + threadIdx.x) * 2;
  if (c >= n) return;
  const bool two = c + 1 < n;
  const bool vec_ok = two && ((ldp & 1) == 0) && ((stridePart & 1) == 0) && ((reinterpret_cast<uintptr_t>(part) & 15) == 0);
  for (int r = blockIdx.y; r < m; r += gridDim.y) {
    const bool k0 = !lower || c <= r, k1 = two && (!lower || c + 1 <= r);
    double s0 = 0.0, s1 = 0.0;
    if (k0 || k1) {
      const double* q = part + (long)r * ldp + c;
      if (vec_ok && k0 && k1) {
        if (NP > 0) {
          d2 v[NP > 0 ? NP : 1];
#pragma unroll
          for (int p = 0; p < NP; ++p) v[p] = *reinterpret_cast<const d2*>(q + (long)p * stridePart);
#pragma unroll
          for (int p = 0; p < NP; ++p) { s0 += v[p].x; s1 += v[p].y; }
        } else {
          for (int p = 0; p < np; ++p, q += stridePart) {
            const d2 v = *reinterpret_cast<const d2*>(q);
            s0 += v.x; s1 += v.y;
          }
        }
      } else {
        for (int p = 0; p < np; ++p, q += stridePart) {
          if (k0) s0 += q[0];
          if (k1) s1 += q[1];
        }
      }
      s0 *= alpha; s1 *= alpha;
      if (lower) {
        if (c == r) s0 *= diag_scale;
        if (c + 1 == r) s1 *= diag_scale;
      }
    }
    double* o = out + (long)r * ldo + c;
    if (two && ((ldo & 1) == 0) && ((reinterpret_cast<uintptr_t>(out) & 15) == 0)) {
      *reinterpret_cast<d2*>(o) = (d2){k0 ? s0 : 0.0, k1 ? s1 : 0.0};
    } else {
      o[0] = k0 ? s0 : 0.0;
      if (two) o[1] = k1 ? s1 : 0.0;
    }
  }
}

struct VarexpArgs {
  const double* Y; long ldy; const double* fmean; int rows, P;
  const double* s0; int s0_per_latent; const double* ssq;
  double knn[16]; int knn_per_latent;
  double noise, mean_const; double* fvar_out; double* part;
  const double* noise_rows;
};
__global__ __launch_bounds__(RB) void varexp_kernel(VarexpArgs a) {
  __shared__ double sh[4];
  const double log2pi = 1.8378770664093453;
  const double c0 = -0.5 * log2pi - 0.5 * log(a.noise);
  double acc = 0.0;
  const long total = (long)a.rows * a.P;
  for (long e = (long)blockIdx.x * RB + threadIdx.x; e < total; e += (long)gridDim.x * RB) {
    const int b = (int)(e / a.P), p = (int)(e - (long)b * a.P);
    double fv = a.knn[a.knn_per_latent ? p : 0];
    if (a.s0) fv -= a.s0_per_latent ? a.s0[(long)p * a.rows + b] : a.s0[b];
    if (a.ssq) fv += a.ssq[(long)p * a.rows + b];
    const double mu = a.fmean[e] + a.mean_const;
    const double dy = a.Y[(long)b * a.ldy + p] - mu;
    if (a.fvar_out) a.fvar_out[e] = fv;
    if (a.noise_rows) {
      const double nv = a.noise_rows[b];
      acc += (-0.5 * log2pi - 0.5 * log(nv)) - 0.5 * (dy * dy + fv) / nv;
    } else {
      acc += c0 - 0.5 * (dy * dy + fv) / a.noise;
    }
  }
  const double r = block_sum(acc, sh);
  if (threadIdx.x == 0) a.part[blockIdx.x] = r;
}

#define GPK_GH20_X                                                                                                          \
  -5.387480890011233, -4.603682449550744, -3.944764040115625, -3.3478545673832163, -2.7888060584281305, -2.2549740020892757, \
      -1.7385377121165861, -1.234076215395323, -0.7374737285453944, -0.24534070830090124, 0.24534070830090124,              \
      0.7374737285453944, 1.234076215395323, 1.7385377121165861, 2.2549740020892757, 2.7888060584281305, 3.3478545673832163, \
      3.944764040115625, 4.603682449550744, 5.387480890011233
#define GPK_GH20_W                                                                                                          \
  2.2293936455341447e-13, 4.3993409922731747e-10, 1.0860693707692782e-07, 7.80255647853206e-06, 0.00022833863601635365,     \
      0.0032437733422378567, 0.024810520887463643, 0.1090172060200233, 0.28667550536283415, 0.4622436696006101,              \
      0.4622436696006101, 0.28667550536283415, 0.1090172060200233, 0.024810520887463643, 0.0032437733422378567,              \
      0.00022833863601635365, 7.80255647853206e-06, 1.0860693707692782e-07, 4.3993409922731747e-10, 2.2293936455341447e-13
constexpr int GH_N = 20;
__constant__ const double gh_x_dev[GH_N] = {GPK_GH20_X};
__constant__ const double gh_w_dev[GH_N] = {GPK_GH20_W};
const double gh_x_host[GH_N] = {GPK_GH20_X};
const double gh_w_host[GH_N] = {GPK_GH20_W};

struct LikVarexpArgs {
  const double* Y; long ldy; const double* fmean; int rows, P;
  const double* s0; int s0_per_latent; const double* ssq;
  double knn[16]; int knn_per_latent;
  double mean_const;
  double par0, par1, c0;
  double *fvar_out, *rows_out, *dmu_out, *dvar_out;
  double *part, *part1;
};

template <int LIK>
__global__ __launch_bounds__(RB) void lik_varexp_kernel(LikVarexpArgs a) {
  constexpr int LPE = (LIK == GPK_LIK_POISSON_EXP) ? 1 : 4;
  constexpr int NPL = GH_N / 4;
  constexpr int G = 64 / LPE;
  __shared__ double sh[4];
  const int lane = threadIdx.x & 63, w = threadIdx.x >> 6;
  const int g = lane / LPE, k = lane % LPE;
  const int rpw = G / a.P;
  const int jr = g / a.P, p = g - jr * a.P;
  const int row_lane0 = (jr * a.P * LPE) & 63;
  const long npass = ((long)a.rows + rpw - 1) / rpw;
  double acc = 0.0, acc1 = 0.0;
  for (long u = (long)blockIdx.x * (RB / 64) + w; u < npass; u += (long)gridDim.x * (RB / 64)) {
    const long b = u * rpw + jr;
    const bool act = jr < rpw && b < a.rows;
    double y = 0.0, mu = 0.0, fv = 1.0;
    if (act) {
      fv = a.knn[a.knn_per_latent ? p : 0];
      if (a.s0) fv -= a.s0_per_latent ? a.s0[(long)p * a.rows + b] : a.s0[b];
      if (a.ssq) fv += a.ssq[(long)p * a.rows + b];
      mu = a.fmean[b * a.P + p] + a.mean_const;
      y = a.Y[b * a.ldy + p];
    }
    const double ynan = y - y;
    double ve, dmu, dvar, dsc = 0.0;
    if (LIK == GPK_LIK_POISSON_EXP) {
      const double e = exp(mu + 0.5 * fv) * a.par0;
      ve = y * mu - e - lgamma(y + 1.0) + y * a.c0;
      dmu = y - e;
      dvar = -0.5 * e;
    } else {
      const double sd = sqrt(2.0 * fv);
      const double sgn = (y == 1.0) ? 1.0 : -1.0;
      double sv = 0.0, sm = 0.0, sx = 0.0, ss = 0.0;
#pragma unroll
      for (int j = 0; j < NPL; ++j) {
        const double x = gh_x_dev[k * NPL + j];
        const double wn = gh_w_dev[k * NPL + j] * 0.5641895835477563;
        const double f = fma(sd, x, mu);
        double gv, gp;
        if (LIK == GPK_LIK_BERNOULLI_PROBIT) {
          const double q = 0.5 * erfc(-sgn * f * 0.7071067811865476) * (1.0 - 2e-3) + 1e-3;
          gv = log(q);
          gp = sgn * ((1.0 - 2e-3) * 0.3989422804014327) * exp(-0.5 * f * f) / q;
        } else {
          const double r = (y - f) / a.par0;
          const double den = a.par1 + r * r;
          gv = a.c0 - 0.5 * (a.par1 + 1.0) * log1p(r * r / a.par1);
          gp = (a.par1 + 1.0) * r / (a.par0 * den);
          ss += wn * (((a.par1 + 1.0) * r * r / den - 1.0) / a.par0);
        }
        sv += wn * gv;
        sm += wn * gp;
        sx += wn * gp * x;
      }
      sv += __shfl_xor(sv, 1); sm += __shfl_xor(sm, 1); sx += __shfl_xor(sx, 1); ss += __shfl_xor(ss, 1);
      sv += __shfl_xor(sv, 2); sm += __shfl_xor(sm, 2); sx += __shfl_xor(sx, 2); ss += __shfl_xor(ss, 2);
      ve = sv;
      dmu = sm;
      dvar = sx / sd;
      dsc = ss;
    }
    ve += ynan; dmu += ynan; dvar += ynan;
    double rs = 0.0;
    for (int q = 0; q < a.P; ++q) rs += __shfl(ve, (row_lane0 + q * LPE) & 63);
    if (act && k == 0) {
      const long e = b * a.P + p;
      if (a.fvar_out) a.fvar_out[e] = fv;
      if (a.dmu_out) a.dmu_out[e] = dmu;
      if (a.dvar_out) a.dvar_out[e] = dvar;
      if (a.rows_out && p == 0) a.rows_out[b] = rs;
      acc += ve;
      acc1 += dsc;
    }
  }
  const double r0 = block_sum(acc, sh);
  if (threadIdx.x == 0) a.part[blockIdx.x] = r0;
  if (a.part1) {
    const double r1 = block_sum(acc1, sh);
    if (threadIdx.x == 0) a.part1[blockIdx.x] = r1;
  }
}

__global__ __launch_bounds__(RB) void kl_white_kernel(const double* q_mu, const double* q_sqrt, int m,
                                                      int P, int q_diag, double* part) {
  __shared__ double sh[4];
  double acc = 0.0;
  const long nmu = (long)m * P;
  const long stride = (long)gridDim.x * RB, start = (long)blockIdx.x * RB + threadIdx.x;
  for (long e = start; e < nmu; e += stride) { const double v = q_mu[e]; acc += v * v; }
  if (q_diag) {
    for (long e = start; e < nmu; e += stride) {
      const double v = q_sqrt[e];
      acc += v * v - log(v * v);
    }
  } else {
    const long tot = (long)P * m * m;
    for (long e = start; e < tot; e += stride) {
      const long w = e % ((long)m * m);
      const int r = (int)(w / m), c = (int)(w - (long)r * m);
      if (c <= r) {
        const double v = q_sqrt[e];
        acc += v * v;
        if (c == r) acc -= log(v * v);
      }
    }
  }
  const double r = block_sum(acc, sh);
  if (threadIdx.x == 0) part[blockIdx.x] = r;
}

__global__ __launch_bounds__(RB) void sum_log_diag_kernel(const double* L, int n, long ldl,
                                                          long strideL, double* out) {
  __shared__ double sh[4];
  const double* M = L + (long)blockIdx.x * strideL;
  double acc = 0.0;
  for (int i = threadIdx.x; i < n; i += RB) acc += log(M[(long)i * ldl + i]);
  const double r = block_sum(acc, sh);
  if (threadIdx.x == 0) out[blockIdx.x] = r;
}

__global__ __launch_bounds__(RB) void sum_log_diag_sq_kernel(const double* L, int n, long ldl, long strideL, double* out) {
  __shared__ double sh[4];
  const double* M = L + (long)blockIdx.x * strideL;
  double acc = 0.0;
  for (int i = threadIdx.x; i < n; i += RB) { const double v = M[(long)i * ldl + i]; acc += log(v * v); }
  const double r = block_sum(acc, sh);
  if (threadIdx.x == 0) out[blockIdx.x] = r;
}

__global__ __launch_bounds__(RB) void sumsq_kernel(const double* A, int rows, int cols, long lda,
                                                   int upper_only, double* part) {
  __shared__ double sh[4];
  double acc = 0.0;
  for (int r = blockIdx.x; r < rows; r += gridDim.x) {
    const double* a = A + (long)r * lda;
    for (int c = (upper_only ? r : 0) + threadIdx.x; c < cols; c += RB) acc = fma(a[c], a[c], acc);
  }
  const double r = block_sum(acc, sh);
  if (threadIdx.x == 0) part[blockIdx.x] = r;
}

int stage2(hipStream_t s, const FinalArgs& f) {
  hipLaunchKernelGGL(final_sum_kernel, dim3(1), dim3(RB), 0, s, f);
  GPK_LAUNCH_CHECK();
  return 0;
}

int nblocks_for(long elems) {
  long b = (elems + RB * 4 - 1) / (RB * 4);
  if (b < 1) b = 1;
  if (b > MAXPART) b = MAXPART;
  return (int)b;
}

}

namespace {
__global__ __launch_bounds__(256) void set_identity_kernel(double* __restrict__ A, int n, long lda, long strideA) {
  const int row = blockIdx.y;
  double* a = A + (long)blockIdx.z * strideA;
  for (int c = blockIdx.x * 256 + threadIdx.x; c < n; c += gridDim.x * 256) a[(long)row * lda + c] = (c == row) ? 1.0 : 0.0;
}
}
namespace {
__global__ void noop_kernel() {}
}
int gpk_launch_noop(hipStream_t s) {
  hipLaunchKernelGGL(noop_kernel, dim3(1), dim3(64), 0, s);
  GPK_LAUNCH_CHECK();
  return 0;
}

namespace {
__global__ void wait_flag_kernel(const int* __restrict__ ptr, int val, int* __restrict__ info) {
  if (threadIdx.x == 0) {
    const long long t0 = wall_clock64();
    while ((int)(__hip_atomic_load(ptr, __ATOMIC_RELAXED, __HIP_MEMORY_SCOPE_SYSTEM) - val) < 0) {
      if (wall_clock64() - t0 >= 50000000LL) {
        if (info) atomicMax(info, 0x7fffffff);
        break;
      }
      __builtin_amdgcn_s_sleep(8);
    }
  }
}
__global__ void set_flag_kernel(int* __restrict__ ptr, int val) {
  __hip_atomic_store(ptr, val, __ATOMIC_RELAXED, __HIP_MEMORY_SCOPE_SYSTEM);
}
}
int gpk_launch_wait_flag(hipStream_t s, const int* ptr, int val, int* info) {
  hipLaunchKernelGGL(wait_flag_kernel, dim3(1), dim3(64), 0, s, ptr, val, info);
  GPK_LAUNCH_CHECK();
  return 0;
}
int gpk_launch_set_flag(hipStream_t s, int* ptr, int val) {
  hipLaunchKernelGGL(set_flag_kernel, dim3(1), dim3(1), 0, s, ptr, val);
  GPK_LAUNCH_CHECK();
  return 0;
}

__global__ void probe_wait_kernel(const int* flag, int* result) {
  const long long t0 = wall_clock64();
  int seen = 0;
  while (!(seen = __hip_atomic_load(flag, __ATOMIC_RELAXED, __HIP_MEMORY_SCOPE_SYSTEM)) && wall_clock64() - t0 < 200000LL)
    __builtin_amdgcn_s_sleep(8);
  *result = seen ? 1 : 0;
}
__global__ void probe_set_kernel(int* flag) { __hip_atomic_store(flag, 1, __ATOMIC_RELAXED, __HIP_MEMORY_SCOPE_SYSTEM); }
int gpk_probe_concurrent_kernels(hipStream_t a, hipStream_t b, int* scratch , int* concurrent) {
  GPK_HIP(hipMemsetAsync(scratch, 0, 2 * sizeof(int), a));
  GPK_HIP(hipStreamSynchronize(a));
  hipLaunchKernelGGL(probe_wait_kernel, dim3(1), dim3(1), 0, a, scratch, scratch + 1);
  GPK_LAUNCH_CHECK();
  hipLaunchKernelGGL(probe_set_kernel, dim3(1), dim3(1), 0, b, scratch);
  GPK_LAUNCH_CHECK();
  GPK_HIP(hipStreamSynchronize(a));
  GPK_HIP(hipStreamSynchronize(b));
  int h[2] = {0, 0};
  GPK_HIP(hipMemcpy(h, scratch, sizeof(h), hipMemcpyDeviceToHost));
  *concurrent = h[1];
  GPK_HIP(hipMemset(scratch, 0, 2 * sizeof(int)));
  return 0;
}

__global__ __launch_bounds__(256) void diag_add_kernel(double* __restrict__ A, int n, long lda, const double* __restrict__ v) {
  const int i = blockIdx.x * 256 + threadIdx.x;
  if (i < n) A[(long)i * lda + i] += v[i];
}
extern "C" int gpk_diag_add(void* stream, double* A, int n, long lda, const double* v) {
  if (!A || !v || n < 0 || lda < n) return GPK_E_ARG;
  if (n == 0) return 0;
  hipLaunchKernelGGL(diag_add_kernel, dim3((n + 255) / 256), dim3(256), 0, (hipStream_t)stream, A, n, lda, v);
  GPK_LAUNCH_CHECK();
  return 0;
}
int gpk_launch_set_identity(hipStream_t s, double* A, int n, long lda, int batch, long strideA) {
  if (n <= 0) return 0;
  dim3 grid((unsigned)gpk_cdiv(n, 256), (unsigned)n, (unsigned)(batch > 0 ? batch : 1));
  hipLaunchKernelGGL(set_identity_kernel, grid, dim3(256), 0, s, A, n, lda, strideA);
  GPK_LAUNCH_CHECK();
  return 0;
}

int gpk_launch_zero_upper(hipStream_t s, double* A, int n, long lda, int batch, long strideA) {
  if (n <= 1) return 0;
  int gx = gpk_cdiv(n, 256);
  if (gx > 16) gx = 16;
  dim3 grid((unsigned)gx, (unsigned)n, (unsigned)(batch > 0 ? batch : 1));
  hipLaunchKernelGGL(zero_upper_kernel, grid, dim3(256), 0, s, A, n, lda, strideA);
  GPK_LAUNCH_CHECK();
  return 0;
}

extern "C" size_t gpk_reduce_workspace_bytes(int n) {
  (void)n;
  return (size_t)4 * MAXPART * sizeof(double);
}

extern "C" int gpk_transpose(void* stream, const double* in, int rows, int cols, long ldin,
                             double* out, long ldout, int mode, int batch, long stride_in,
                             long stride_out) {
  if (rows < 0 || cols < 0) return GPK_E_ARG;
  if (rows == 0 || cols == 0) return 0;
  if (!in || !out) return GPK_E_ARG;
  dim3 grid((unsigned)gpk_cdiv(cols, 32), (unsigned)gpk_cdiv(rows, 32),
            (unsigned)(batch > 0 ? batch : 1));
  hipLaunchKernelGGL(transpose_kernel, grid, dim3(256), 0, (hipStream_t)stream, in, rows, cols, ldin,
                     out, ldout, mode, stride_in, stride_out);
  GPK_LAUNCH_CHECK();
  return 0;
}

extern "C" int gpk_row_stats(void* stream, const double* At, int rows, int m, long ldat,
                             const double* V, const double* W, int P, double alpha, double beta,
                             double* sumsq, double* mv, double* wsq) {
  if (rows < 0 || m < 0) return GPK_E_ARG;
  if (rows == 0) return 0;
  if (!At) return GPK_E_ARG;
  const int np = (V || W) ? P : 0;
  const dim3 grid((unsigned)gpk_cdiv(rows, 4));
  int p0 = 0;
  do {
    hipLaunchKernelGGL((row_stats_kernel<4>), grid, dim3(256), 0, (hipStream_t)stream, At, rows, m,
                       ldat, V, W, np, p0, alpha, beta, sumsq, mv, wsq);
    GPK_LAUNCH_CHECK();
    p0 += 4;
  } while (p0 < np);
  return 0;
}

int gpk_launch_row_stats_sep(hipStream_t s, const double* At, long strideAt, int rows, int m, long ldat, const double* V, int P,
                             double* sumsq, double* mv) {
  if (!At || !V || !sumsq || !mv || rows < 0 || m < 0 || P <= 0) return GPK_E_ARG;
  if (rows == 0) return 0;
  hipLaunchKernelGGL(row_stats_sep_kernel, dim3((unsigned)gpk_cdiv(rows, 4), (unsigned)P), dim3(256), 0, s, At, strideAt, rows, m,
                     ldat, V, P, sumsq, mv);
  GPK_LAUNCH_CHECK();
  return 0;
}

extern "C" int gpk_row_dot(void* stream, const double* A, long lda, const double* B, long ldb,
                           int rows, int cols, double alpha, double beta, double* out) {
  if (rows < 0 || cols < 0) return GPK_E_ARG;
  if (rows == 0) return 0;
  if (!A || !B || !out) return GPK_E_ARG;
  hipLaunchKernelGGL(row_dot_kernel, dim3((unsigned)gpk_cdiv(rows, 4)), dim3(256), 0,
                     (hipStream_t)stream, A, lda, B, ldb, rows, cols, alpha, beta, out);
  GPK_LAUNCH_CHECK();
  return 0;
}

extern "C" int gpk_row_sumsq(void* stream, const double* A, int rows, int cols, long lda,
                             double alpha, double beta, double* out) {
  return gpk_row_stats(stream, A, rows, cols, lda, nullptr, nullptr, 0, alpha, beta, out, nullptr,
                       nullptr);
}

int gpk_launch_sum_parts(hipStream_t s, const double* part, int nt, int rows, long stridePart, int P,
                         double* ssq) {
  if (rows == 0 || P == 0) return 0;
  dim3 grid((unsigned)gpk_cdiv(rows, 256), (unsigned)P);
  hipLaunchKernelGGL(sum_parts_kernel, grid, dim3(256), 0, s, part, nt, rows, stridePart, ssq);
  GPK_LAUNCH_CHECK();
  return 0;
}

extern "C" int gpk_combine_parts(void* stream, const double* parts, int nparts, long stride_part, int m, int n, long ldp,
                                 double alpha, int lower, double diag_scale, double* out, long ldo) {
  if (nparts <= 0 || m < 0 || n < 0 || ldp < n || ldo < n) return GPK_E_ARG;
  if (m == 0 || n == 0) return 0;
  if (!parts || !out) return GPK_E_ARG;
  dim3 grid((unsigned)gpk_cdiv(gpk_cdiv(n, 2), 256), (unsigned)(m < 65535 ? m : 65535));
#define GPK_COMBINE(NP)                                                                                               \
  hipLaunchKernelGGL((combine_parts_kernel<NP>), grid, dim3(256), 0, (hipStream_t)stream, parts, nparts, stride_part, m, n, \
                     ldp, alpha, lower, diag_scale, out, ldo)
  switch (nparts) {
    case 1: GPK_COMBINE(1); break;
    case 2: GPK_COMBINE(2); break;
    case 4: GPK_COMBINE(4); break;
    case 8: GPK_COMBINE(8); break;
    case 16: GPK_COMBINE(16); break;
    case 32: GPK_COMBINE(32); break;
    default: GPK_COMBINE(0); break;
  }
#undef GPK_COMBINE
  GPK_LAUNCH_CHECK();
  return 0;
}

extern "C" int gpk_gaussian_varexp_sum(void* stream, const double* Y, long ldy, const double* fmean,
                                       int rows, int P, const double* s0, int s0_per_latent,
                                       const double* ssq, const double* knn_host,
                                       int knn_per_latent, double noise_variance, const double* noise_rows,
                                       double mean_const, double* fvar_out, double* out, void* ws, size_t ws_bytes) {
  if ((rows > 0 && (!Y || !fmean)) || !knn_host || !out || P <= 0 || P > 16 || rows < 0) return GPK_E_ARG;
  if (!ws || ws_bytes < gpk_reduce_workspace_bytes(rows)) return GPK_E_WORKSPACE;
  VarexpArgs a{};
  a.Y = Y; a.ldy = ldy; a.fmean = fmean; a.rows = rows; a.P = P;
  a.s0 = s0; a.s0_per_latent = s0_per_latent; a.ssq = ssq;
  for (int i = 0; i < (knn_per_latent ? P : 1); ++i) a.knn[i] = knn_host[i];
  a.knn_per_latent = knn_per_latent; a.noise = noise_variance; a.mean_const = mean_const;
  a.fvar_out = fvar_out; a.part = (double*)ws; a.noise_rows = noise_rows;
  const int nb = nblocks_for((long)rows * P);
  hipLaunchKernelGGL(varexp_kernel, dim3(nb), dim3(RB), 0, (hipStream_t)stream, a);
  GPK_LAUNCH_CHECK();
  FinalArgs f{};
  f.nterms = 1; f.part[0] = a.part; f.count[0] = nb; f.scale[0] = 1.0; f.add = 0.0; f.out = out;
  return stage2((hipStream_t)stream, f);
}

extern "C" int gpk_gauss_hermite(int n, double* x_host, double* w_host) {
  if (!x_host || !w_host) return GPK_E_ARG;
  if (n != GH_N) return GPK_E_UNSUPPORTED;
  for (int i = 0; i < GH_N; ++i) { x_host[i] = gh_x_host[i]; w_host[i] = gh_w_host[i]; }
  return 0;
}

int gpk_likelihood_check(int lik, const double* params) {
  switch (lik) {
    case GPK_LIK_BERNOULLI_PROBIT: return 0;
    case GPK_LIK_POISSON_EXP: return (params && params[0] > 0.0) ? 0 : GPK_E_ARG;
    case GPK_LIK_STUDENT_T: return (params && params[0] > 0.0 && params[1] > 0.0) ? 0 : GPK_E_ARG;
    default: return GPK_E_UNSUPPORTED;
  }
}

int gpk_launch_likelihood_varexp_stage1(hipStream_t s, int lik, const double* params, const double* Y, long ldy, const double* fmean,
                                        int rows, int P, const double* s0, int s0_per_latent, const double* ssq,
                                        const double* knn_host, int knn_per_latent, double mean_const, double* fvar_out,
                                        double* rows_out, double* dmu_out, double* dvar_out, double* part, double* part1, int* count) {
  const int rc = gpk_likelihood_check(lik, params);
  if (rc) return rc;
  LikVarexpArgs a{};
  a.Y = Y; a.ldy = ldy; a.fmean = fmean; a.rows = rows; a.P = P;
  a.s0 = s0; a.s0_per_latent = s0_per_latent; a.ssq = ssq;
  for (int i = 0; i < (knn_per_latent ? P : 1); ++i) a.knn[i] = knn_host[i];
  a.knn_per_latent = knn_per_latent; a.mean_const = mean_const;
  a.fvar_out = fvar_out; a.rows_out = rows_out; a.dmu_out = dmu_out; a.dvar_out = dvar_out;
  a.part = part; a.part1 = part1;
  const int per_wave = (lik == GPK_LIK_POISSON_EXP ? 64 : 16) / P;
  long nb = (((long)rows + per_wave - 1) / per_wave + RB / 64 - 1) / (RB / 64);
  if (nb < 1) nb = 1;
  if (nb > MAXPART) nb = MAXPART;
  const dim3 grid((unsigned)nb), block(RB);
  if (lik == GPK_LIK_BERNOULLI_PROBIT) {
    hipLaunchKernelGGL((lik_varexp_kernel<GPK_LIK_BERNOULLI_PROBIT>), grid, block, 0, s, a);
  } else if (lik == GPK_LIK_POISSON_EXP) {
    a.par0 = params[0]; a.c0 = log(params[0]);
    hipLaunchKernelGGL((lik_varexp_kernel<GPK_LIK_POISSON_EXP>), grid, block, 0, s, a);
  } else {
    const double scale = params[0], df = params[1];
    a.par0 = scale; a.par1 = df;
    a.c0 = lgamma(0.5 * (df + 1.0)) - lgamma(0.5 * df) - 0.5 * (log(scale * scale) + log(df) + log(3.141592653589793));
    hipLaunchKernelGGL((lik_varexp_kernel<GPK_LIK_STUDENT_T>), grid, block, 0, s, a);
  }
  GPK_LAUNCH_CHECK();
  *count = (int)nb;
  return 0;
}

extern "C" int gpk_likelihood_varexp_sum(void* stream, int lik, const double* lik_params_host, const double* Y, long ldy,
                                         const double* fmean, int rows, int P, const double* s0, int s0_per_latent,
                                         const double* ssq, const double* knn_host, int knn_per_latent, double mean_const,
                                         double* fvar_out, double* rows_out, double* dmu_out, double* dvar_out, double* out,
                                         void* ws, size_t ws_bytes) {
  if ((rows > 0 && (!Y || !fmean)) || !knn_host || !out || P <= 0 || P > 16 || rows < 0) return GPK_E_ARG;
  if (!ws || ws_bytes < gpk_reduce_workspace_bytes(rows)) return GPK_E_WORKSPACE;
  double* part = (double*)ws;
  int nb = 0;
  const int rc = gpk_launch_likelihood_varexp_stage1((hipStream_t)stream, lik, lik_params_host, Y, ldy, fmean, rows, P, s0,
                                                     s0_per_latent, ssq, knn_host, knn_per_latent, mean_const, fvar_out, rows_out,
                                                     dmu_out, dvar_out, part, part + MAXPART, &nb);
  if (rc) return rc;
  for (int t = 0; t < 2; ++t) {
    FinalArgs f{};
    f.nterms = 1; f.part[0] = part + t * MAXPART; f.count[0] = nb; f.scale[0] = 1.0; f.add = 0.0; f.out = out + t;
    const int r2 = stage2((hipStream_t)stream, f);
    if (r2) return r2;
  }
  return 0;
}

extern "C" int gpk_gauss_kl_white(void* stream, const double* q_mu, const double* q_sqrt, int m,
                                  int P, int q_diag, double* out, void* ws, size_t ws_bytes) {
  if (!q_mu || !q_sqrt || !out || m <= 0 || P <= 0) return GPK_E_ARG;
  if (!ws || ws_bytes < gpk_reduce_workspace_bytes(m)) return GPK_E_WORKSPACE;
  const long elems = q_diag ? (long)m * P : (long)P * m * m;
  const int nb = nblocks_for(elems);
  double* part = (double*)ws;
  hipLaunchKernelGGL(kl_white_kernel, dim3(nb), dim3(RB), 0, (hipStream_t)stream, q_mu, q_sqrt, m, P,
                     q_diag, part);
  GPK_LAUNCH_CHECK();
  FinalArgs f{};
  f.nterms = 1; f.part[0] = part; f.count[0] = nb; f.scale[0] = 0.5;
  f.add = -0.5 * (double)m * (double)P; f.out = out;
  return stage2((hipStream_t)stream, f);
}

extern "C" int gpk_sum_log_diag(void* stream, const double* L, int n, long ldl, int batch,
                                long strideL, double* out) {
  if (!L || !out || n <= 0) return GPK_E_ARG;
  hipLaunchKernelGGL(sum_log_diag_kernel, dim3((unsigned)(batch > 0 ? batch : 1)), dim3(RB), 0,
                     (hipStream_t)stream, L, n, ldl, strideL, out);
  GPK_LAUNCH_CHECK();
  return 0;
}

__global__ __launch_bounds__(RB) void kl_unwhite_diag_kernel(const double* __restrict__ LinvT, long ldl, int m,
                                                            const double* __restrict__ W, int P, double* __restrict__ part) {
  __shared__ double sh[4];
  double acc = 0.0;
  for (int i = blockIdx.x; i < m; i += gridDim.x) {
    double ss = 0.0;
    for (int k = i + threadIdx.x; k < m; k += RB) {
      const double v = LinvT[(long)i * ldl + k];
      ss += v * v;
    }
    const double kinv = block_sum(ss, sh);
    __syncthreads();
    if (threadIdx.x == 0) {
      double w2 = 0.0, lg = 0.0;
      for (int p = 0; p < P; ++p) {
        const double w = W[(long)i * P + p];
        w2 += w * w;
        lg += log(w * w);
      }
      acc += kinv * w2 - lg;
    }
  }
  if (threadIdx.x == 0) part[blockIdx.x] = acc;
}
int gpk_launch_kl_unwhite_diag_stage1(hipStream_t s, const double* LinvT, long ldl, int m, const double* W, int P, double* part,
                                      int* count) {
  const int nb = m < GPK_REDUCE_MAXPART ? m : GPK_REDUCE_MAXPART;
  hipLaunchKernelGGL(kl_unwhite_diag_kernel, dim3(nb), dim3(RB), 0, s, LinvT, ldl, m, W, P, part);
  GPK_LAUNCH_CHECK();
  *count = nb;
  return 0;
}

int gpk_launch_sum_log_diag_sq(hipStream_t s, const double* L, int n, long ldl, int batch, long strideL, double* out) {
  if (!L || !out || n <= 0) return GPK_E_ARG;
  hipLaunchKernelGGL(sum_log_diag_sq_kernel, dim3((unsigned)(batch > 0 ? batch : 1)), dim3(RB), 0, s, L, n, ldl, strideL, out);
  GPK_LAUNCH_CHECK();
  return 0;
}

extern "C" int gpk_sumsq(void* stream, const double* A, int rows, int cols, long lda, int upper_only,
                         double* out, void* ws, size_t ws_bytes) {
  if ((!A && rows > 0 && cols > 0) || !out || rows < 0 || cols < 0) return GPK_E_ARG;
  if (!ws || ws_bytes < gpk_reduce_workspace_bytes(rows)) return GPK_E_WORKSPACE;
  int nb = rows < MAXPART ? rows : MAXPART;
  if (nb < 1) nb = 1;
  double* part = (double*)ws;
  hipLaunchKernelGGL(sumsq_kernel, dim3(nb), dim3(RB), 0, (hipStream_t)stream, A, rows, cols, lda,
                     upper_only, part);
  GPK_LAUNCH_CHECK();
  FinalArgs f{};
  f.nterms = 1; f.part[0] = part; f.count[0] = nb; f.scale[0] = 1.0; f.add = 0.0; f.out = out;
  return stage2((hipStream_t)stream, f);
}

int gpk_launch_final(hipStream_t s, int nterms, const double* const* part, const int* count,
                     const double* scale, double add, double* out) {
  FinalArgs f{};
  f.nterms = nterms;
  for (int t = 0; t < nterms; ++t) { f.part[t] = part[t]; f.count[t] = count[t]; f.scale[t] = scale[t]; }
  f.add = add; f.out = out;
  return stage2(s, f);
}

int gpk_launch_sumsq_stage1(hipStream_t s, const double* A, int rows, int cols, long lda,
                            int upper_only, double* part, int* count) {
  int nb = rows < MAXPART ? rows : MAXPART;
  if (nb < 1) nb = 1;
  hipLaunchKernelGGL(sumsq_kernel, dim3(nb), dim3(RB), 0, s, A, rows, cols, lda, upper_only, part);
  GPK_LAUNCH_CHECK();
  *count = nb;
  return 0;
}
int gpk_launch_varexp_stage1(hipStream_t s, const double* Y, long ldy, const double* fmean, int rows,
                             int P, const double* s0, int s0_per_latent, const double* ssq,
                             const double* knn_host, int knn_per_latent, double noise,
                             double mean_const, double* fvar_out, double* part, int* count, const double* noise_rows) {
  VarexpArgs a{};
  a.Y = Y; a.ldy = ldy; a.fmean = fmean; a.rows = rows; a.P = P;
  a.s0 = s0; a.s0_per_latent = s0_per_latent; a.ssq = ssq;
  for (int i = 0; i < (knn_per_latent ? P : 1); ++i) a.knn[i] = knn_host[i];
  a.knn_per_latent = knn_per_latent; a.noise = noise; a.mean_const = mean_const;
  a.fvar_out = fvar_out; a.part = part; a.noise_rows = noise_rows;
  const int nb = nblocks_for((long)rows * P);
  hipLaunchKernelGGL(varexp_kernel, dim3(nb), dim3(RB), 0, s, a);
  GPK_LAUNCH_CHECK();
  *count = nb;
  return 0;
}
int gpk_launch_kl_white_stage1(hipStream_t s, const double* q_mu, const double* q_sqrt, int m, int P,
                               int q_diag, double* part, int* count) {
  const long elems = q_diag ? (long)m * P : (long)P * m * m;
  const int nb = nblocks_for(elems);
  hipLaunchKernelGGL(kl_white_kernel, dim3(nb), dim3(RB), 0, s, q_mu, q_sqrt, m, P, q_diag, part);
  GPK_LAUNCH_CHECK();
  *count = nb;
  return 0;
}
int gpk_launch_transpose_shift(hipStream_t s, const double* in, int rows, int cols, long ldin,
                               double* out, long ldout, double shift) {
  if (rows == 0 || cols == 0) return 0;
  dim3 grid((unsigned)gpk_cdiv(cols, 32), (unsigned)gpk_cdiv(rows, 32), 1);
  hipLaunchKernelGGL(transpose_shift_kernel, grid, dim3(256), 0, s, in, rows, cols, ldin, out, ldout,
                     shift);
  GPK_LAUNCH_CHECK();
  return 0;
}

namespace {
__global__ void publish_host_kernel(const double* __restrict__ src, int n, const int* __restrict__ info, double* vals, int* tail,
                                    int seq) {
  if (threadIdx.x == 0) {
    for (int i = 0; i < n; ++i) __hip_atomic_store(vals + i, src[i], __ATOMIC_RELAXED, __HIP_MEMORY_SCOPE_SYSTEM);
    __hip_atomic_store(tail, info ? info[0] : 0, __ATOMIC_RELAXED, __HIP_MEMORY_SCOPE_SYSTEM);
    __hip_atomic_store(tail + 1, seq, __ATOMIC_RELEASE, __HIP_MEMORY_SCOPE_SYSTEM);
  }
}
}

extern "C" int gpk_publish_host(void* stream, const double* src, int n, const int* info, void* host_dst, int seq) {
  if (!src || !host_dst || n <= 0 || n > 16) return GPK_E_ARG;
  double* vals = (double*)host_dst;
  hipLaunchKernelGGL(publish_host_kernel, dim3(1), dim3(64), 0, (hipStream_t)stream, src, n, info, vals, (int*)(vals + n), seq);
  GPK_LAUNCH_CHECK();
  return 0;
}

namespace {
__global__ __launch_bounds__(256) void moment_rows_kernel(const double* __restrict__ B, long ldb, int n2, int d, double* __restrict__ Vt,
                                                          long ldv) {
  const int j = blockIdx.x * 256 + threadIdx.x;
  if (j >= n2) return;
  Vt[j] = 1.0;
  for (int c = 0; c < d; ++c) {
    const double b = B[(long)j * ldb + c];
    Vt[(long)(1 + c) * ldv + j] = b;
    Vt[(long)(1 + d + c) * ldv + j] = b * b;
  }
}

constexpr int AT_THREADS = 1024;
__global__ __launch_bounds__(AT_THREADS) void adjoint_tail_kernel(const double* __restrict__ R, long ldr, const double* __restrict__ A,
                                                                  long lda, int n1, int d, const double* __restrict__ ls, double variance,
                                                                  int symmetric, const double* __restrict__ sum_kbar_k,
                                                                  double* __restrict__ Abar, long ldab, double* __restrict__ small,
                                                                  int accumulate, double dvar_add) {
  __shared__ double sh[AT_THREADS];
  __shared__ double sh_rs[AT_THREADS];
  const int t = threadIdx.x;
  const int rpp = AT_THREADS / d;
  const int c = t % d, r0 = t / d;
  double acc = 0.0, acc_rs = 0.0;
  if (r0 < rpp) {
    const double l = ls[c];
    const double il2 = 1.0 / (l * l);
    for (int i = r0; i < n1; i += rpp) {
      const double* Ri = R + (long)i * ldr;
      const double rs = Ri[0], gb = Ri[1 + c], gb2 = Ri[1 + d + c];
      const double a = A[(long)i * lda + c];
      const double T = gb - a * rs;
      double ab;
      if (symmetric) {
        ab = 2.0 * T * il2;
        acc += a * ab;
      } else {
        ab = T * il2;
        acc += gb2 - a * (gb + T);
      }
      double* o = Abar + (long)i * ldab + c;
      *o = accumulate ? *o + ab : ab;
      if (c == 0) acc_rs += rs;
    }
  }
  sh[t] = acc;
  sh_rs[t] = acc_rs;
  __syncthreads();
  if (t < d) {
    double s = 0.0;
    for (int q = 0; q < rpp; ++q) s += sh[q * d + t];
    const double l = ls[t];
    const double r = symmetric ? -s / l : s / (l * l * l);
    small[1 + t] = accumulate ? small[1 + t] + r : r;
  }
  if (t == 0) {
    double s = 0.0;
    if (sum_kbar_k) s = sum_kbar_k[0];
    else
      for (int q = 0; q < rpp; ++q) s += sh_rs[q * d];
    const double r = s / variance + dvar_add;
    small[0] = accumulate ? small[0] + r : r;
  }
}

__global__ __launch_bounds__(256) void adam_kernel(double* __restrict__ p, const double* __restrict__ g, double* __restrict__ m,
                                                   double* __restrict__ v, long n, double b1, double b2, double eps, double step,
                                                   double gsign) {
  for (long i = (long)blockIdx.x * 256 + threadIdx.x; i < n; i += (long)gridDim.x * 256) {
    const double gi = gsign * g[i];
    const double mi = b1 * m[i] + (1.0 - b1) * gi;
    const double vi = b2 * v[i] + (1.0 - b2) * gi * gi;
    m[i] = mi;
    v[i] = vi;
    p[i] -= step * mi / (sqrt(vi) + eps);
  }
}

__global__ __launch_bounds__(256) void lowrank_axpy_kernel(double alpha, const double* __restrict__ X, long ldx, const double* __restrict__ U,
                                                           long ldu, const double* __restrict__ V, long ldv, int m, int n, int k,
                                                           double* __restrict__ out, long ldo) {
  const int c = (blockIdx.x * 256 + threadIdx.x) * 2;
  if (c >= n) return;
  const bool two = c + 1 < n;
  double v0[16], v1[16];
#pragma unroll
  for (int q = 0; q < 16; ++q) {
    v0[q] = q < k ? V[(long)c * ldv + q] : 0.0;
    v1[q] = (q < k && two) ? V[(long)(c + 1) * ldv + q] : 0.0;
  }
  const bool vec = two && !(ldx & 1) && !(ldo & 1) && !(reinterpret_cast<uintptr_t>(X) & 15) && !(reinterpret_cast<uintptr_t>(out) & 15);
  for (int r = blockIdx.y; r < m; r += gridDim.y) {
    double s0 = 0.0, s1 = 0.0;
#pragma unroll
    for (int q = 0; q < 16; ++q)
      if (q < k) {
        const double u = U[(long)r * ldu + q];
        s0 += u * v0[q];
        s1 += u * v1[q];
      }
    const double* x = X + (long)r * ldx + c;
    double* o = out + (long)r * ldo + c;
    if (vec) {
      const d2 xv = *reinterpret_cast<const d2*>(x);
      *reinterpret_cast<d2*>(o) = (d2){alpha * xv.x + s0, alpha * xv.y + s1};
    } else {
      o[0] = alpha * x[0] + s0;
      if (two) o[1] = alpha * x[1] + s1;
    }
  }
}

__global__ __launch_bounds__(256) void symmetrize_kernel(double* __restrict__ S, int n, long lds) {
  __shared__ double ta[32][33], tb[32][33];
  const int bi = blockIdx.y, bj = blockIdx.x;
  if (bj > bi) return;
  const int tx = threadIdx.x & 31, ty = threadIdx.x >> 5;
  for (int r = ty; r < 32; r += 8) {
    const int i = bi * 32 + r, j = bj * 32 + tx;
// ... 69 lines not shown
```

gpflow_amd/ops.py:

```python
from __future__ import annotations

from typing import Optional, Sequence, Tuple

import numpy as np
import torch

from . import _lib

NB = 128
KERNEL_FAMILIES = {"SquaredExponential": 0, "Matern12": 1, "Matern32": 2, "Matern52": 3}
MAX_D = 64


def device() -> torch.device:
    if not torch.cuda.is_available():
        raise _lib.GpkError("gpflow_amd needs a HIP device (torch.cuda.is_available() is False); "
                            "there is no CPU path")
    return torch.device("cuda", torch.cuda.current_device())


def to_device(x, dtype=torch.float64) -> torch.Tensor:
    if isinstance(x, torch.Tensor):
        t = x.to(device=device(), dtype=dtype)
    else:
# ... 188 lines not shown


def check_info(info: torch.Tensor, what: str = "Cholesky") -> None:
    bad = info.cpu().numpy()
    if np.any(bad != 0):
        j = int(bad[np.nonzero(bad)[0][0]])
        if j >= INFO_HANDOFF_TIMEOUT:
            raise _lib.GpkError(f"{what} decomposition failed: an internal stream hand-off timed out (status INT_MAX); "
                                "the result is undefined")
        raise _lib.GpkError(f"{what} decomposition was not successful: non-positive pivot at column {j - 1}")


def trtri_blocks(L: torch.Tensor) -> torch.Tensor:
    lib = _lib.load()
    _chk(L, "L", 2)
    n = L.shape[0]
    invd = invd_alloc(n, 1)
    rc = lib.gpk_trtri_blocks(_stream(), L.data_ptr(), n, _rowmajor(L, "L"), 1, 0, invd.data_ptr())
    _lib.check(rc, "gpk_trtri_blocks")
    return invd


def transpose_factor(L: torch.Tensor, invd: torch.Tensor) -> Tuple[torch.Tensor, torch.Tensor]:
    lib = _lib.load()
    _chk(L, "L", 2)
    n = L.shape[0]
    LT = torch.empty((n, n), dtype=torch.float64, device=L.device)
    invdT = torch.empty_like(invd)
    rc = lib.gpk_transpose_factor(_stream(), L.data_ptr(), _rowmajor(L, "L"), invd.data_ptr(), n,
                                  LT.data_ptr(), n, invdT.data_ptr())
    _lib.check(rc, "gpk_transpose_factor")
    return LT, invdT


def trsm_(B: torch.Tensor, L: torch.Tensor, invd: torch.Tensor, *, trans: int = 0) -> torch.Tensor:
    lib = _lib.load()
    _chk(B, "B", 2)
    _chk(L, "L", 2)
    n = L.shape[0]
    if B.shape[1] != n:
        raise ValueError(f"B has {B.shape[1]} columns, factor is {n}x{n}")
    rc = lib.gpk_trsm(_stream(), int(trans), L.data_ptr(), _rowmajor(L, "L"), invd.data_ptr(), n,
                      B.data_ptr(), B.shape[0], _rowmajor(B, "B"), 1, 0, 0)
    _lib.check(rc, "gpk_trsm")
    return B


def gemm_nt(A: torch.Tensor, B: torch.Tensor, *, alpha: float = 1.0, beta: float = 0.0,
            C: Optional[torch.Tensor] = None, b_tri: int = 0, c_lower: bool = False, a_tri: int = 0,
            k_split: bool = False, zero_skipped: bool = True) -> torch.Tensor:
    lib = _lib.load()
    _chk(A, "A")
    _chk(B, "B")
    batched = A.dim() == 3 or B.dim() == 3
    A3 = A if A.dim() == 3 else A.unsqueeze(0)
    B3 = B if B.dim() == 3 else B.unsqueeze(0)
    batch = max(A3.shape[0], B3.shape[0])
    m, k = A3.shape[1], A3.shape[2]
    n = B3.shape[1]
    if B3.shape[2] != k:
        raise ValueError("inner dimensions differ")
    if C is None:
        if beta != 0.0:
            raise ValueError("beta != 0 needs C")
        C = torch.empty((batch, m, n) if batched else (m, n), dtype=torch.float64, device=A.device)
        if c_lower and zero_skipped:
            C.zero_()
    C3 = C if C.dim() == 3 else C.unsqueeze(0)
    sA = int(A3.stride(0)) if A3.shape[0] > 1 else 0
    sB = int(B3.stride(0)) if B3.shape[0] > 1 else 0
    sC = int(C3.stride(0)) if C3.shape[0] > 1 else 0
    rc = lib.gpk_gemm_nt(_stream(), m, n, k, float(alpha), A3.data_ptr(), _rowmajor(A3[0], "A"),
                         B3.data_ptr(), _rowmajor(B3[0], "B"), float(beta), C3.data_ptr(),
                         _rowmajor(C3[0], "C"), int(b_tri) | (int(a_tri) << 4) | (0x100 if k_split else 0), int(c_lower), batch, sA, sB, sC)
    _lib.check(rc, "gpk_gemm_nt")
    return C


def transpose(X: torch.Tensor, *, mode: int = 0, out: Optional[torch.Tensor] = None) -> torch.Tensor:
    lib = _lib.load()
    _chk(X, "X")
    X3 = X if X.dim() == 3 else X.unsqueeze(0)
    b, r, c = X3.shape
    if out is None:
        out = torch.empty((b, c, r) if X.dim() == 3 else (c, r), dtype=torch.float64, device=X.device)
    O3 = out if out.dim() == 3 else out.unsqueeze(0)
    rc = lib.gpk_transpose(_stream(), X3.data_ptr(), r, c, _rowmajor(X3[0], "X"), O3.data_ptr(),
                           _rowmajor(O3[0], "out"), int(mode), b,
                           int(X3.stride(0)) if b > 1 else 0, int(O3.stride(0)) if b > 1 else 0)
    _lib.check(rc, "gpk_transpose")
    return out


def row_stats(At: torch.Tensor, *, V: Optional[torch.Tensor] = None, W: Optional[torch.Tensor] = None,
              want_sumsq: bool = True):
    lib = _lib.load()
    _chk(At, "At", 2)
    rows, m = At.shape
    P = 0
    for name, t in (("V", V), ("W", W)):
        if t is not None:
            _chk(t, name, 2)
            if t.shape[0] != m or not t.is_contiguous():
                raise ValueError(f"{name} must be contiguous [m, P]")
            P = t.shape[1]
    sumsq = torch.empty(rows, dtype=torch.float64, device=At.device) if want_sumsq else None
    mv = torch.empty((rows, P), dtype=torch.float64, device=At.device) if V is not None else None
    wsq = torch.empty((P, rows), dtype=torch.float64, device=At.device) if W is not None else None
    rc = lib.gpk_row_stats(_stream(), At.data_ptr(), rows, m, _rowmajor(At, "At"),
                           V.data_ptr() if V is not None else None,
                           W.data_ptr() if W is not None else None, P, 1.0, 0.0,
                           sumsq.data_ptr() if sumsq is not None else None,
                           mv.data_ptr() if mv is not None else None,
                           wsq.data_ptr() if wsq is not None else None)
    _lib.check(rc, "gpk_row_stats")
    return sumsq, mv, wsq


def row_dot(A: torch.Tensor, B: torch.Tensor) -> torch.Tensor:
    lib = _lib.load()
    _chk(A, "A", 2)
    _chk(B, "B", 2)
    if A.shape != B.shape:
        raise ValueError("shape mismatch")
    out = torch.empty(A.shape[0], dtype=torch.float64, device=A.device)
    rc = lib.gpk_row_dot(_stream(), A.data_ptr(), _rowmajor(A, "A"), B.data_ptr(), _rowmajor(B, "B"),
                         A.shape[0], A.shape[1], 1.0, 0.0, out.data_ptr())
    _lib.check(rc, "gpk_row_dot")
    return out


def project(At: torch.Tensor, LqT: torch.Tensor) -> torch.Tensor:
    lib = _lib.load()
    _chk(LqT, "LqT", 3)
    P = LqT.shape[0]
    if At.dim() == 3:
        if At.dtype != torch.float64 or At.shape[0] != P or At.stride(2) != 1:
            raise ValueError("batched At must be float64 [P, rows, m] with unit column stride")
        rows, m = At.shape[1], At.shape[2]
        ldat, stride_at = At.stride(1), At.stride(0)
    else:
        _chk(At, "At", 2)
        rows, m = At.shape
        ldat, stride_at = _rowmajor(At, "At"), 0
    if LqT.shape[1] != m or LqT.shape[2] != m or not LqT.is_contiguous():
        raise ValueError("LqT must be contiguous [P, m, m]")
    ssq = torch.empty((P, rows), dtype=torch.float64, device=At.device)
    nbytes = int(lib.gpk_project_workspace_bytes(rows, m, P))
    ws = _ws(nbytes)
    rc = lib.gpk_project_batched(_stream(), At.data_ptr(), rows, m, ldat, stride_at, LqT.data_ptr(), m, P,
                                 ssq.data_ptr(), ws.data_ptr(), ws.numel() * 8)
    _lib.check(rc, "gpk_project_batched")
    return ssq


def gaussian_varexp_sum(Y: torch.Tensor, fmean: torch.Tensor, *, s0: Optional[torch.Tensor],
                        ssq: Optional[torch.Tensor], knn: Sequence[float], noise_variance,
                        mean_const: float = 0.0, s0_per_latent: bool = False, want_fvar: bool = False):
    lib = _lib.load()
    _chk(Y, "Y", 2)
    _chk(fmean, "fmean", 2)
    rows, P = fmean.shape
    if not fmean.is_contiguous():
        raise ValueError("fmean must be contiguous")
    out = torch.empty(1, dtype=torch.float64, device=Y.device)
    fvar = torch.empty((rows, P), dtype=torch.float64, device=Y.device) if want_fvar else None
    ws = _ws(int(lib.gpk_reduce_workspace_bytes(rows)))
    knn = list(np.atleast_1d(np.asarray(knn, dtype=np.float64)))
    per = int(len(knn) > 1)
    nv, nv_rows, _keep = _noise_args(noise_variance, rows)
    rc = lib.gpk_gaussian_varexp_sum(_stream(), Y.data_ptr(), _rowmajor(Y, "Y"), fmean.data_ptr(), rows, P,
                                     s0.data_ptr() if s0 is not None else None, int(s0_per_latent),
                                     ssq.data_ptr() if ssq is not None else None,
                                     _lib.host_doubles(knn), per, nv, nv_rows, float(mean_const),
                                     fvar.data_ptr() if fvar is not None else None, out.data_ptr(),
                                     ws.data_ptr(), ws.numel() * 8)
    _lib.check(rc, "gpk_gaussian_varexp_sum")
    return out, fvar


LIKELIHOOD_CODES = {"bernoulli_probit": 1, "poisson_exp": 2, "student_t": 3}


def _lik_args(lik: str, params):
    if lik not in LIKELIHOOD_CODES:
        raise ValueError(f"unknown likelihood {lik!r}: one of {sorted(LIKELIHOOD_CODES)}")
    params = [float(v) for v in params]
    if len(params) != {"bernoulli_probit": 0, "poisson_exp": 1, "student_t": 2}[lik]:
        raise ValueError(f"likelihood {lik!r}: wrong number of parameters ({len(params)})")
    return LIKELIHOOD_CODES[lik], (_lib.host_doubles(params) if params else None)


def gauss_hermite(n: int = 20) -> Tuple[np.ndarray, np.ndarray]:
    lib = _lib.load()
    x, w = (_lib.c_double * int(n))(), (_lib.c_double * int(n))()
    _lib.check(lib.gpk_gauss_hermite(int(n), x, w), "gpk_gauss_hermite")
    return np.array(x, dtype=np.float64), np.array(w, dtype=np.float64)


def likelihood_varexp_sum(Y: torch.Tensor, fmean: torch.Tensor, *, s0: Optional[torch.Tensor], ssq: Optional[torch.Tensor],
                          knn: Sequence[float], lik: str, params=(), mean_const: float = 0.0, s0_per_latent: bool = False,
                          want_fvar: bool = False, want_rows: bool = False, want_grads: bool = False):
    lib = _lib.load()
    _chk(Y, "Y", 2)
    _chk(fmean, "fmean", 2)
    rows, P = fmean.shape
    if not fmean.is_contiguous():
        raise ValueError("fmean must be contiguous")
    if Y.shape[0] != rows or Y.shape[1] < P:
        raise ValueError("Y must have one row per row of fmean and at least P columns")
    for name, t, shape in (("s0", s0, (P, rows) if s0_per_latent else (rows,)), ("ssq", ssq, (P, rows))):
        if t is not None:
            _chk(t, name)
            if tuple(t.shape) != shape or not t.is_contiguous():
                raise ValueError(f"{name} must be contiguous {shape}")
    code, par = _lik_args(lik, params)

    def new(*shape):
        return torch.empty(shape, dtype=torch.float64, device=Y.device)
    out = new(2)
    fvar = new(rows, P) if want_fvar else None
    rws = new(rows) if want_rows else None
    dmu, dvar = (new(rows, P), new(rows, P)) if want_grads else (None, None)
    ws = _ws(int(lib.gpk_reduce_workspace_bytes(rows)))
    knn = list(np.atleast_1d(np.asarray(knn, dtype=np.float64)))
    ptr = lambda t: t.data_ptr() if t is not None else None
    rc = lib.gpk_likelihood_varexp_sum(_stream(), code, par, Y.data_ptr(), _rowmajor(Y, "Y"), fmean.data_ptr(), rows, P,
                                       ptr(s0), int(s0_per_latent), ptr(ssq), _lib.host_doubles(knn), int(len(knn) > 1),
                                       float(mean_const), ptr(fvar), ptr(rws), ptr(dmu), ptr(dvar), out.data_ptr(),
                                       ws.data_ptr(), ws.numel() * 8)
    _lib.check(rc, "gpk_likelihood_varexp_sum")
    return out, rws, dmu, dvar, fvar


def gauss_kl_white(q_mu: torch.Tensor, q_sqrt: torch.Tensor) -> torch.Tensor:
    lib = _lib.load()
    _chk(q_mu, "q_mu", 2)
    _chk(q_sqrt, "q_sqrt")
    m, P = q_mu.shape
    q_diag = int(q_sqrt.dim() == 2)
    if not (q_mu.is_contiguous() and q_sqrt.is_contiguous()):
        raise ValueError("q_mu / q_sqrt must be contiguous")
    out = torch.empty(1, dtype=torch.float64, device=q_mu.device)
    ws = _ws(int(lib.gpk_reduce_workspace_bytes(m)))
    rc = lib.gpk_gauss_kl_white(_stream(), q_mu.data_ptr(), q_sqrt.data_ptr(), m, P, q_diag,
                                out.data_ptr(), ws.data_ptr(), ws.numel() * 8)
    _lib.check(rc, "gpk_gauss_kl_white")
    return out


def sum_log_diag(L: torch.Tensor) -> torch.Tensor:
    lib = _lib.load()
    _chk(L, "L")
    L3 = L if L.dim() == 3 else L.unsqueeze(0)
    b = L3.shape[0]
    n = min(L3.shape[1], L3.shape[2])
    out = torch.empty(b, dtype=torch.float64, device=L.device)
    rc = lib.gpk_sum_log_diag(_stream(), L3.data_ptr(), n, _rowmajor(L3[0], "L"), b,
                              int(L3.stride(0)) if b > 1 else 0, out.data_ptr())
    _lib.check(rc, "gpk_sum_log_diag")
    return out


def combine_parts(parts: torch.Tensor, *, alpha: float = 1.0, lower: bool = False, diag_scale: float = 1.0,
                  out: Optional[torch.Tensor] = None) -> torch.Tensor:
    lib = _lib.load()
    _chk(parts, "parts")
    p3 = parts if parts.dim() == 3 else parts.unsqueeze(0)
    if p3.dim() != 3:
        raise ValueError("parts must be [np, m, n] or [m, n]")
    npart, m, n = p3.shape
    ldp = _rowmajor(p3[0], "parts")
    stride = int(p3.stride(0)) if npart > 1 else 0
    if out is None:
        out = torch.empty((m, n), dtype=torch.float64, device=parts.device)
    _chk(out, "out", 2)
    rc = lib.gpk_combine_parts(_stream(), p3.data_ptr(), npart, stride, m, n, ldp, float(alpha), int(lower),
                               float(diag_scale), out.data_ptr(), _rowmajor(out, "out"))
    _lib.check(rc, "gpk_combine_parts")
    return out


def sumsq(A: torch.Tensor, *, upper_only: bool = False) -> torch.Tensor:
    lib = _lib.load()
    _chk(A, "A", 2)
    out = torch.empty(1, dtype=torch.float64, device=A.device)
    ws = _ws(int(lib.gpk_reduce_workspace_bytes(A.shape[0])))
    rc = lib.gpk_sumsq(_stream(), A.data_ptr(), A.shape[0], A.shape[1], _rowmajor(A, "A"), int(upper_only),
                       out.data_ptr(), ws.data_ptr(), ws.numel() * 8)
    _lib.check(rc, "gpk_sumsq")
    return out


def moment_rows(B: torch.Tensor) -> torch.Tensor:
    lib = _lib.load()
    _chk(B, "B", 2)
    n2, d = B.shape
    Vt = torch.empty((1 + 2 * d, n2), dtype=torch.float64, device=B.device)
    rc = lib.gpk_moment_rows(_stream(), B.data_ptr(), _rowmajor(B, "B"), n2, d, Vt.data_ptr(), n2)
    _lib.check(rc, "gpk_moment_rows")
    return Vt


def stationary_adjoint_tail(R: torch.Tensor, A: torch.Tensor, ls: torch.Tensor, *, variance: float, symmetric: bool,
                            sum_kbar_k: Optional[torch.Tensor] = None, into: Optional[Tuple[torch.Tensor, torch.Tensor]] = None,
                            dvar_add: float = 0.0) -> Tuple[torch.Tensor, torch.Tensor, torch.Tensor]:
# ... 251 lines not shown
```

include/gpk.h:

```cpp
#ifndef GPK_H
#define GPK_H

#include <stddef.h>
#include <stdint.h>

#ifdef __cplusplus
extern "C" {
#endif
#if defined(__GNUC__) || defined(__clang__)
#pragma GCC visibility push(default)
#endif

#define GPK_NB 128
#define GPK_MAX_D 64

#define GPK_E_ARG (-1)
#define GPK_E_WORKSPACE (-2)
#define GPK_E_UNSUPPORTED (-3)

#define GPK_KERN_SE 0
#define GPK_KERN_MATERN12 1
#define GPK_KERN_MATERN32 2
#define GPK_KERN_MATERN52 3

const char* gpk_version(void);

int gpk_kernel_matrix(void* stream, int family, const double* X1, int n1, long ldx1,
                      const double* X2, int n2, long ldx2, int d, const double* ls_host, int ard,
                      double variance, double diag_add, int lower_only, double* K, long ldk);

int gpk_diag_add(void* stream, double* A, int n, long lda, const double* v);

int gpk_kernel_matrix_combine(void* stream, int family, int op, const double* X1, int n1, long ldx1,
                              const double* X2, int n2, long ldx2, int d, const double* ls_host, int ard,
                              double variance, double diag_add, const double* G, long ldg, double* out, long ldo);

int gpk_kernel_matrix_hadamard(void* stream, int family, const double* X1, int n1, long ldx1,
                               const double* X2, int n2, long ldx2, int d, const double* ls_host, int ard,
                               double variance, const double* G, long ldg, double* out, long ldo);

size_t gpk_invd_elems(int n, int batch);
int gpk_potrf(void* stream, double* A, int n, int extra, long lda, int batch, long strideA,
              double* invd, int zero_upper, int* info);

int gpk_stream_selfcheck(double* us_now, double* us_first, int* recreated);
int gpk_chain_handoff_mode(void);

int gpk_potrf_inv(void* stream, double* A, int n, int extra, long lda, double* invd, int zero_upper, int* info);

int gpk_trtri_blocks(void* stream, const double* L, int n, long ldl, int batch, long strideL,
                     double* invd);

int gpk_trsm(void* stream, int trans, const double* L, long ldl, const double* invd, int n,
             double* B, int m, long ldb, int batch, long strideL, long strideB);
int gpk_transpose_factor(void* stream, const double* L, long ldl, const double* invd, int n,
                         double* LT, long ldlt, double* invdT);

int gpk_gemm_nt(void* stream, int m, int n, int k, double alpha, const double* A, long lda,
                const double* B, long ldb, double beta, double* C, long ldc, int b_tri,
                int c_lower, int batch, long strideA, long strideB, long strideC);

int gpk_transpose(void* stream, const double* in, int rows, int cols, long ldin, double* out,
                  long ldout, int mode, int batch, long stride_in, long stride_out);

int gpk_row_stats(void* stream, const double* At, int rows, int m, long ldat, const double* V,
                  const double* W, int P, double alpha, double beta, double* sumsq, double* mv,
                  double* wsq);
int gpk_row_sumsq(void* stream, const double* A, int rows, int cols, long lda, double alpha,
                  double beta, double* out);
int gpk_row_dot(void* stream, const double* A, long lda, const double* B, long ldb, int rows,
                int cols, double alpha, double beta, double* out);

size_t gpk_project_workspace_bytes(int rows, int m, int P);
int gpk_project(void* stream, const double* At, int rows, int m, long ldat, const double* LqT,
                long ldl, int P, double* ssq, void* ws, size_t ws_bytes);
int gpk_project_batched(void* stream, const double* At, int rows, int m, long ldat, long strideAt,
                        const double* LqT, long ldl, int P, double* ssq, void* ws, size_t ws_bytes);

size_t gpk_reduce_workspace_bytes(int n);
int gpk_gaussian_varexp_sum(void* stream, const double* Y, long ldy, const double* fmean, int rows,
                            int P, const double* s0, int s0_per_latent, const double* ssq,
                            const double* knn_host, int knn_per_latent, double noise_variance,
                            const double* noise_rows, double mean_const, double* fvar_out, double* out, void* ws,
                            size_t ws_bytes);

#define GPK_LIK_BERNOULLI_PROBIT 1
#define GPK_LIK_POISSON_EXP 2
#define GPK_LIK_STUDENT_T 3
int gpk_likelihood_varexp_sum(void* stream, int lik, const double* lik_params_host, const double* Y, long ldy,
                              const double* fmean, int rows, int P, const double* s0, int s0_per_latent, const double* ssq,
                              const double* knn_host, int knn_per_latent, double mean_const, double* fvar_out,
                              double* rows_out, double* dmu_out, double* dvar_out, double* out, void* ws, size_t ws_bytes);
int gpk_gauss_hermite(int n, double* x_host, double* w_host);

int gpk_gauss_kl_white(void* stream, const double* q_mu, const double* q_sqrt, int m, int P,
                       int q_diag, double* out, void* ws, size_t ws_bytes);

int gpk_sum_log_diag(void* stream, const double* L, int n, long ldl, int batch, long strideL,
                     double* out);
int gpk_sumsq(void* stream, const double* A, int rows, int cols, long lda, int upper_only,
              double* out, void* ws, size_t ws_bytes);

int gpk_combine_parts(void* stream, const double* parts, int nparts, long stride_part, int m, int n, long ldp,
                      double alpha, int lower, double diag_scale, double* out, long ldo);

int gpk_moment_rows(void* stream, const double* B, long ldb, int n2, int d, double* Vt, long ldv);
int gpk_stationary_adjoint_tail(void* stream, const double* R, long ldr, const double* A, long lda, int n1, int d,
                                const double* ls_dev, double variance, int symmetric, const double* sum_kbar_k,
                                double* Abar, long ldab, double* small, int accumulate, double dvar_add);
int gpk_adam_step(void* stream, double* p, const double* g, double* m, double* v, long n, double beta1, double beta2,
                  double epsilon, double step, int maximise);
int gpk_lowrank_axpy(void* stream, double alpha, const double* X, long ldx, const double* U, long ldu, const double* V, long ldv,
                     int m, int n, int k, double* out, long ldo);
int gpk_symmetrize(void* stream, double* S, int n, long lds);

size_t gpk_gpr_lml_workspace_bytes(int n, int d, int P);
int gpk_gpr_lml(void* stream, int family, const double* X, int n, int d, long ldx, const double* Y,
                int P, long ldy, const double* ls_host, int ard, double variance,
                double noise_variance, const double* noise_rows, double mean_const, double* out, int* info,
                void* ws, size_t ws_bytes);

size_t gpk_svgp_elbo_workspace_bytes(int m, int rows, int d, int P, int q_diag, int whiten);
int gpk_svgp_elbo_shard(void* stream, int family, const double* Z, int m, long ldz, const double* Xb,
                        const double* Yb, int rows, long ldxb, long ldyb, int d, int P,
                        const double* ls_host, int ard, double variance, double noise_variance,
                        const double* noise_rows, double jitter, double mean_const, const double* q_mu,
                        const double* q_sqrt, int q_diag, int whiten, double* out, int* info,
                        void* ws, size_t ws_bytes);

int gpk_svgp_elbo_shard_lik(void* stream, int family, const double* Z, int m, long ldz, const double* Xb, const double* Yb,
                            int rows, long ldxb, long ldyb, int d, int P, const double* ls_host, int ard, double variance,
                            int lik, const double* lik_params_host, double jitter, double mean_const, const double* q_mu,
                            const double* q_sqrt, int q_diag, int whiten, double* out, int* info, void* ws, size_t ws_bytes);

size_t gpk_svgp_elbo_sep_workspace_bytes(int m, int rows, int d, int P);
int gpk_svgp_elbo_shard_sep(void* stream, const int* family_host, const double* Z, int m, long ldz, long strideZ,
                            const double* Xb, const double* Yb, int rows, long ldxb, long ldyb, int d, int P,
                            const double* ls_host, int ard, const double* variance_host, double noise_variance,
                            const double* noise_rows, double jitter, double mean_const, const double* q_mu,
                            const double* q_sqrt, double* out, int* info, void* ws, size_t ws_bytes);

int gpk_publish_host(void* stream, const double* src, int n, const int* info, void* host_dst, int seq);

void gpk_profile_gemm_enable(int on);
int gpk_profile_gemm_collect(double* total_ms, long* launches, double* flops);
int gpk_profile_gemm_collect_min(double min_flops, int keep, double* total_ms, long* launches, double* flops);
int gpk_profile_gemm_collect_kind(int kind, double min_flops, double* total_ms, long* launches, double* flops);
int gpk_profile_gemm_window(double min_flops, double* window_ms, double* flops_all, double* flops_matching,
                            long* launches_all);

int gpk_bench_mfma_f64(void* stream, int blocks, int iters, double* sink);
int gpk_bench_stream_store(void* stream, double* out, long n_doubles);

#if defined(__GNUC__) || defined(__clang__)
#pragma GCC visibility pop
#endif
#ifdef __cplusplus
}
#endif
#endif
```

Before: 546.7 steps/s.

## Fuse row stats into projection GEMM and varexp reduction tail

Folds the Kfu row sum-of-squares and the mean product (Kfu·q_mu) into the fast projection GEMM's operand-load path, so a separate row_stats pass over Kfu is no longer needed. It also fuses the partial-column sum into the varexp kernel and uses a last-block ticket to finish the reduction in the same kernel. The KL ticket counter is zeroed inside the KL kernel. Together this removes several kernel launches and one full read of the 8192x2048 Kfu matrix, at the cost of extra registers and loads in the GEMM inner loop, which may affect its scheduling or occupancy.

New measurement: 558.2 steps/s, median of 6. +2.1%, better.

```diff
diff --git a/gpflow_amd/_lib.py b/gpflow_amd/_lib.py
--- a/gpflow_amd/_lib.py
+++ b/gpflow_amd/_lib.py
@@ -45,6 +45,7 @@
     "gpk_project_workspace_bytes": (c_size_t, [c_int, c_int, c_int]),
     "gpk_project": (c_int, [c_void_p, _dp, c_int, c_int, c_long, _dp, c_long, c_int, _dp, _dp, c_size_t]),
     "gpk_project_batched": (c_int, [c_void_p, _dp, c_int, c_int, c_long, c_long, _dp, c_long, c_int, _dp, _dp, c_size_t]),
+    "gpk_project_stats": (c_int, [c_void_p, _dp, c_int, c_int, c_long, _dp, c_long, c_int, _dp, _dp, _dp, _dp, _dp, c_size_t]),
     "gpk_reduce_workspace_bytes": (c_size_t, [c_int]),
     "gpk_gaussian_varexp_sum": (c_int, [c_void_p, _dp, c_long, _dp, c_int, c_int, _dp, c_int, _dp,
                                         C.POINTER(c_double), c_int, c_double, _dp, c_double, _dp, _dp, _dp,
diff --git a/gpflow_amd/csrc/drivers.hip b/gpflow_amd/csrc/drivers.hip
--- a/gpflow_amd/csrc/drivers.hip
+++ b/gpflow_amd/csrc/drivers.hip
@@ -6,8 +6,9 @@
 
 namespace {
 int project_parts(hipStream_t s, const double* At, int rows, int m, long ldat, long strideAt, const double* LqT, long ldl, int P, void* ws,
-                  size_t ws_bytes) {
+                  size_t ws_bytes, const double* V = nullptr, double* s0 = nullptr, double* fmean = nullptr) {
   if ((!At && rows > 0) || !LqT || rows < 0 || m <= 0 || P <= 0 || strideAt < 0) return GPK_E_ARG;
+  if (V && ((rows > 0 && (!s0 || !fmean)) || strideAt != 0)) return GPK_E_ARG;
   if (!ws || ws_bytes < gpk_project_workspace_bytes(rows, m, P)) return GPK_E_WORKSPACE;
   if (rows == 0) return 0;
   const int nt = 2 * gpk_gemm_tiles_n(m);
@@ -16,8 +17,26 @@
   g.epi = 1; g.sq_cols = m; g.c2_cols = 0;
   g.part = (double*)ws; g.part_ld = rows; g.stridePart = (long)nt * rows;
   g.C2 = (double*)ws; g.ldc2 = 0; g.strideC2 = 0;
+  if (V) {
+    g.stat_sumsq = s0; g.stat_mv = fmean; g.stat_V = V; g.stat_P = P;
+    if (!gpk_gemm_fuses_row_stats(g)) {
+      g.stat_sumsq = g.stat_mv = nullptr; g.stat_V = nullptr; g.stat_P = 0;
+      const int rc = gpk_row_stats((void*)s, At, rows, m, ldat, V, nullptr, P, 1.0, 0.0, s0, fmean, nullptr);
+      if (rc) return rc;
+    }
+  }
   return gpk_launch_gemm(s, g);
 }
+}
+
+extern "C" int gpk_project_stats(void* stream, const double* At, int rows, int m, long ldat, const double* LqT, long ldl, int P,
+                                 const double* V, double* s0, double* fmean, double* ssq, void* ws, size_t ws_bytes) {
+  if (!V || (rows > 0 && !ssq)) return GPK_E_ARG;
+  hipStream_t s = (hipStream_t)stream;
+  const int rc = project_parts(s, At, rows, m, ldat, 0, LqT, ldl, P, ws, ws_bytes, V, s0, fmean);
+  if (rc || rows == 0) return rc;
+  const int nt = 2 * gpk_gemm_tiles_n(m);
+  return gpk_launch_sum_parts(s, (const double*)ws, nt, rows, (long)nt * rows, P, ssq);
 }
 
 extern "C" int gpk_project_batched(void* stream, const double* At, int rows, int m, long ldat, long strideAt,
@@ -202,7 +221,15 @@
   return gpk_transpose((void*)s, a.q_sqrt, a.m, a.m, a.m, w.LqT, w.ld, 1, a.P, (long)a.m * a.m, (long)a.m * w.ld);
 }
 
-int varexp_to_out(hipStream_t s, const ElboArgs& a, const ElboWs& w, const double* knn_host, int per_latent) {
+int varexp_to_out(hipStream_t s, const ElboArgs& a, const ElboWs& w, const double* knn_host, int per_latent,
+                  const double* slot = nullptr, int nt = 0, int* ticket = nullptr) {
+  if (slot && !a.lik)
+    return gpk_launch_varexp_tail(s, a.Yb, a.ldyb, w.fmean, a.rows, a.P, w.s0, slot, nt, (long)nt * a.rows, knn_host[0],
+                                  a.noise_variance, a.mean_const, a.noise_rows, w.part0, ticket, a.out);
+  if (slot) {
+    const int rc = gpk_launch_sum_parts(s, slot, nt, a.rows, (long)nt * a.rows, a.P, w.ssq);
+    if (rc) return rc;
+  }
   int count = 0;
   const int rc = a.lik
       ? gpk_launch_likelihood_varexp_stage1(s, a.lik, a.lik_params, a.Yb, a.ldyb, w.fmean, a.rows, a.P, w.s0, per_latent, w.ssq,
@@ -213,9 +240,10 @@
   if (rc) return rc;
   return final_one(s, w.part0, count, 1.0, 0.0, a.out);
 }
+int* tail_ticket(const ElboWs& w) { return (int*)(w.part2 + GPK_REDUCE_MAXPART + 32); }
 int kl_white_to_out(hipStream_t s, const ElboArgs& a, const ElboWs& w) {
   int count = 0;
-  const int rc = gpk_launch_kl_white_stage1(s, a.q_mu, a.q_sqrt, a.m, a.P, a.q_diag, w.part1, &count);
+  const int rc = gpk_launch_kl_white_stage1(s, a.q_mu, a.q_sqrt, a.m, a.P, a.q_diag, w.part1, &count, w.part2 ? tail_ticket(w) : nullptr);
   if (rc) return rc;
   return final_one(s, w.part1, count, 0.5, -0.5 * (double)a.m * (double)a.P, a.out + 1);
 }
@@ -235,20 +263,19 @@
   if (side) hk.late_work = [&a, &w](hipStream_t bs) { return transpose_q_sqrt_and_kl(bs, a, w); };
   int rc = gpk_potrf_core(s, w.T, a.m, a.rows, w.ld, 1, 0, w.invd, 0, a.info, hk);
   if (rc) return rc;
-  rc = gpk_row_stats((void*)s, w.Kfu, a.rows, a.m, w.ld, a.q_mu, a.q_diag ? a.q_sqrt : nullptr, a.P, 1.0, 0.0, w.s0, w.fmean,
-                     a.q_diag ? w.ssq : nullptr);
-  if (rc) return rc;
-  if (!a.q_diag) {
-    if (!side) {
-      rc = transpose_q_sqrt(s, a, w);
-      if (rc) return rc;
-    }
-    rc = gpk_project((void*)s, w.Kfu, a.rows, a.m, w.ld, w.LqT, w.ld, a.P, w.ssq, w.proj, gpk_project_workspace_bytes(a.rows, a.m, a.P));
-    if (rc) return rc;
-  }
-  rc = varexp_to_out(s, a, w, &a.k.variance, 0);
-  if (rc || side) return rc;
-  return kl_white_to_out(s, a, w);
+  if (!side) {
+    rc = transpose_q_sqrt_and_kl(s, a, w);
+    if (rc) return rc;
+  }
+  if (a.q_diag) {
+    rc = gpk_row_stats((void*)s, w.Kfu, a.rows, a.m, w.ld, a.q_mu, a.q_sqrt, a.P, 1.0, 0.0, w.s0, w.fmean, w.ssq);
+    if (rc) return rc;
+    return a.lik ? varexp_to_out(s, a, w, &a.k.variance, 0) : varexp_to_out(s, a, w, &a.k.variance, 0, w.ssq, 1, tail_ticket(w));
+  }
+  rc = project_parts(s, w.Kfu, a.rows, a.m, w.ld, 0, w.LqT, w.ld, a.P, w.proj, gpk_project_workspace_bytes(a.rows, a.m, a.P), a.q_mu,
+                     w.s0, w.fmean);
+  if (rc) return rc;
+  return varexp_to_out(s, a, w, &a.k.variance, 0, w.proj, 2 * gpk_gemm_tiles_n(a.m), tail_ticket(w));
 }
 
 int elbo_unwhitened_full(hipStream_t s, const ElboArgs& a, const ElboWs& w) {
@@ -263,9 +290,9 @@
   if (rc) return rc;
   rc = gpk_transpose((void*)s, w.arow, P, m, w.ld, w.V, P, 0, 1, 0, 0);
   if (rc) return rc;
-  rc = gpk_row_stats((void*)s, w.Kfu, a.rows, m, w.ld, w.V, nullptr, P, 1.0, 0.0, w.s0, w.fmean, nullptr);
-  if (rc) return rc;
-  rc = gpk_project((void*)s, w.Kfu, a.rows, m, w.ld, w.LqT, w.ld, P, w.ssq, w.proj, gpk_project_workspace_bytes(a.rows, m, P));
+  rc = project_parts(s, w.Kfu, a.rows, m, w.ld, 0, w.LqT, w.ld, P, w.proj, gpk_project_workspace_bytes(a.rows, m, P), w.V, w.s0, w.fmean);
+  if (rc) return rc;
+  rc = gpk_launch_sum_parts(s, w.proj, 2 * gpk_gemm_tiles_n(m), a.rows, (long)2 * gpk_gemm_tiles_n(m) * a.rows, P, w.ssq);
   if (rc) return rc;
   rc = varexp_to_out(s, a, w, &a.k.variance, 0);
   if (rc) return rc;
diff --git a/gpflow_amd/csrc/gemm.hip b/gpflow_amd/csrc/gemm.hip
--- a/gpflow_amd/csrc/gemm.hip
+++ b/gpflow_amd/csrc/gemm.hip
@@ -458,7 +458,7 @@
 }
 
 
-template <int EPI>
+template <int EPI, int SP = 0>
 __device__ __forceinline__ void fast_tile(const GemmArgs& p, int tile_m, int tile_n, double* smem, int rev = 0, int bz_queue = -1) {
   constexpr int BM = 128, BN = 128;
   constexpr int BUF = (BM + BN) * LDSS;
@@ -507,6 +507,13 @@
   }
   const int woff = srow * LDSS + scol;
   d2 st[8];
+  double ssq[4], smv[4], sv[2];
+  const char* vbase = nullptr;
+  if constexpr (SP > 0) {
+    vbase = reinterpret_cast<const char*>(p.stat_V + (long)(kb + scol) * p.stat_P + bz);
+#pragma unroll
+    for (int q = 0; q < 4; ++q) { ssq[q] = 0.0; smv[q] = 0.0; }
+  }
   auto gload = [&](int s) {
     const long so = rev ? (long)(nk - 1 - s) : (long)s;
     const char* ab = abase + so * (BK * 8);
@@ -515,6 +522,22 @@
     for (int q = 0; q < 4; ++q) st[q] = *reinterpret_cast<const d2*>(ab + oa[q]);
 #pragma unroll
     for (int q = 0; q < 4; ++q) st[4 + q] = *reinterpret_cast<const d2*>(bb + ob[q]);
+    if constexpr (SP > 0) {
+      const char* vb = vbase + so * (BK * 8) * p.stat_P;
+      sv[0] = *reinterpret_cast<const double*>(vb);
+      sv[1] = *reinterpret_cast<const double*>(vb + p.stat_P * 8);
+    }
+  };
+  auto stat_acc = [&]() {
+    if constexpr (SP > 0) {
+#pragma unroll
+      for (int q = 0; q < 4; ++q) {
+        ssq[q] = fma(st[q].x, st[q].x, ssq[q]);
+        ssq[q] = fma(st[q].y, st[q].y, ssq[q]);
+        smv[q] = fma(st[q].x, sv[0], smv[q]);
+        smv[q] = fma(st[q].y, sv[1], smv[q]);
+      }
+    }
   };
   auto lstore1 = [&](int buf, int q) {
     const int row = (q < 4) ? 32 * q : BM + 32 * (q - 4);
@@ -591,6 +614,7 @@
   if (nk > 0) {
 #pragma unroll
     for (int q = 0; q < 8; ++q) lstore1(0, q);
+    stat_acc();
     __syncthreads();
     fload(0, 0, 0);
   }
@@ -601,7 +625,7 @@
     fload(cur, 1, 1);
 #pragma unroll
     for (int i = 0; i < 4; ++i) { GPK_MFMA_ROW(0, i); }
-    if constexpr (MORE) __builtin_amdgcn_sched_group_barrier(0x020, 8, 0);
+    if constexpr (MORE) __builtin_amdgcn_sched_group_barrier(0x020, 8 + 2 * SP, 0);
     __builtin_amdgcn_sched_group_barrier(0x100, 8, 0);
     __builtin_amdgcn_sched_group_barrier(0x008, 16, 0);
     __builtin_amdgcn_sched_barrier(0);
@@ -615,6 +639,7 @@
     if constexpr (MORE) {
 #pragma unroll
       for (int q = 0; q < 8; ++q) lstore1(cur ^ 1, q);
+      stat_acc();
     }
 #pragma unroll
     for (int i = 0; i < 4; ++i) { GPK_MFMA_ROW(0, i); }
@@ -692,11 +717,28 @@
       s += __shfl_xor(s, 32);
       if (lane_g == 0 && row < p.m) part[(long)(tile_n * 2 + wn) * p.part_ld + row] = s;
     }
-  }
-}
-
-
-template <int EPI, bool PAIR, bool QUEUE = false>
+    if constexpr (SP > 0) {
+      if (tile_n == 0) {
+#pragma unroll
+        for (int q = 0; q < 4; ++q) {
+#pragma unroll
+          for (int o = 1; o < 8; o <<= 1) {
+            ssq[q] += __shfl_xor(ssq[q], o);
+            smv[q] += __shfl_xor(smv[q], o);
+          }
+          const int row = m0 + srow + 32 * q;
+          if ((tid & 7) == 0 && row < p.m) {
+            if (bz == 0) p.stat_sumsq[row] = ssq[q];
+            p.stat_mv[(long)row * p.stat_P + bz] = smv[q];
+          }
+        }
+      }
+    }
+  }
+}
+
+
+template <int EPI, bool PAIR, bool QUEUE = false, int SP = 0>
 __global__ __launch_bounds__(256, 2) void gemm_nt_fast(GemmArgs p, int gx, int gy, int total, int compact) {
   extern __shared__ __attribute__((aligned(16))) double smem[];
   if (p.sig_ptr && threadIdx.x == 0 && blockIdx.x == 0 && blockIdx.y == 0)
@@ -736,13 +778,13 @@
       } else {
         tile_order(t, p.b_tri, gx, gy, total, compact, tile_m, tile_n);
       }
-      fast_tile<EPI>(p, tile_m, tile_n, smem);
+      fast_tile<EPI, SP>(p, tile_m, tile_n, smem);
       if (t + (int)gridDim.x < total) __syncthreads();
     }
   } else {
     const int align = (EPI == 1 && p.b_tri == 1) ? p.pair_k_align : 0;
     const int tile_m = blockIdx.x % gy, j = blockIdx.x / gy;
-    fast_tile<EPI>(p, tile_m, j, smem, align);
+    fast_tile<EPI, SP>(p, tile_m, j, smem, align);
     if (gx - 1 - j != j) {
       __syncthreads();
       fast_tile<EPI>(p, tile_m, gx - 1 - j, smem, 0);
@@ -773,15 +815,27 @@
   return 0;
 }
 
+constexpr size_t FAST_LDS_BYTES = 2 * (size_t)256 * LDSS * sizeof(double);
+template <int EPI, bool PAIR, int SP>
+int launch_fast_kernel(hipStream_t s, dim3 grid, size_t lds_bytes, const GemmArgs& a, int gx, int gy, int total, int compact) {
+  static const hipError_t attr = hipFuncSetAttribute(reinterpret_cast<const void*>(gemm_nt_fast<EPI, PAIR, false, SP>),
+                                                     hipFuncAttributeMaxDynamicSharedMemorySize, PAIR ? (int)FAST_LDS_BYTES : 160 * 1024);
+  GPK_HIP(attr);
+  hipLaunchKernelGGL((gemm_nt_fast<EPI, PAIR, false, SP>), grid, dim3(256), lds_bytes, s, a, gx, gy, total, compact);
+  GPK_LAUNCH_CHECK();
+  return 0;
+}
+template <int EPI, bool PAIR>
+int launch_fast_walk(hipStream_t s, dim3 grid, size_t lds_bytes, const GemmArgs& a, int gx, int gy, int total, int compact) {
+  if constexpr (EPI == 1) {
+    if (a.stat_sumsq) return launch_fast_kernel<1, PAIR, 1>(s, grid, lds_bytes, a, gx, gy, total, compact);
+  }
+  return launch_fast_kernel<EPI, PAIR, 0>(s, grid, lds_bytes, a, gx, gy, total, compact);
+}
+
 template <int EPI>
 int launch_fast(hipStream_t s, const GemmArgs& a) {
-  constexpr size_t LDS_BYTES = 2 * (size_t)256 * LDSS * sizeof(double);
-  static const hipError_t attr0 = hipFuncSetAttribute(reinterpret_cast<const void*>(gemm_nt_fast<EPI, false>),
-                                                      hipFuncAttributeMaxDynamicSharedMemorySize, 160 * 1024);
-  static const hipError_t attr1 = hipFuncSetAttribute(reinterpret_cast<const void*>(gemm_nt_fast<EPI, true>),
-                                                      hipFuncAttributeMaxDynamicSharedMemorySize, (int)LDS_BYTES);
-  GPK_HIP(attr0);
-  GPK_HIP(attr1);
+  constexpr size_t LDS_BYTES = FAST_LDS_BYTES;
   const int gx = gpk_cdiv(a.n, 128), gy = gpk_cdiv(a.m, 128);
   if (gx <= 0 || gy <= 0) return 0;
   int total = gx * gy, compact = 0;
@@ -808,19 +862,14 @@
       b.stagger_first = 256;
       b.stagger_ticks = 0;
       g_last_kind = 2 + 2 * EPI;
-      hipLaunchKernelGGL((gemm_nt_fast<EPI, false>), dim3((unsigned)total, nb, 1), dim3(256), LDS_BYTES, s, b, gx, gy, total, compact);
-      GPK_LAUNCH_CHECK();
-      return 0;
+      return launch_fast_walk<EPI, false>(s, dim3((unsigned)total, nb, 1), LDS_BYTES, b, gx, gy, total, compact);
     }
     if (pair_ok && gx >= 4 && a.b_tri_rows >= a.n) {
       total = ((gx + 1) / 2) * gy;
       g_last_kind = 2 + 2 * EPI + 1;
       GemmArgs ap = a;
       ap.pair_k_align = GPK_TUNE(PAIR_K_ALIGN, 1);
-      hipLaunchKernelGGL((gemm_nt_fast<EPI, true>), dim3((unsigned)total, nb, 1), dim3(256), LDS_BYTES, s, ap, gx, gy,
-                         total, compact);
-      GPK_LAUNCH_CHECK();
-      return 0;
+      return launch_fast_walk<EPI, true>(s, dim3((unsigned)total, nb, 1), LDS_BYTES, ap, gx, gy, total, compact);
     }
   }
   int tail_tiles = 0;
@@ -868,9 +917,8 @@
     GPK_LAUNCH_CHECK();
     return 0;
   }
-  hipLaunchKernelGGL((gemm_nt_fast<EPI, false>), dim3(nwg, nb, 1), dim3(256), lds_bytes, s, b, gx, gy, total,
-                     compact);
-  GPK_LAUNCH_CHECK();
+  const int rcw = launch_fast_walk<EPI, false>(s, dim3(nwg, nb, 1), lds_bytes, b, gx, gy, total, compact);
+  if (rcw) return rcw;
   if (tail_tiles > 0) {
     using Cfg = TileCfg<64, 64, 4, 1>;
     static const hipError_t attrt = hipFuncSetAttribute(reinterpret_cast<const void*>(gemm_nt_kernel<64, 64, 4, 1>),
@@ -1529,7 +1577,21 @@
   return rc;
 }
 
+static bool proj_small_tiles(const GemmArgs& a) {
+  if (!(a.epi == 1 && a.b_tri == 1 && !(a.beta != 0.0 && a.C) && a.m > 64)) return false;
+  const long pairs = (long)((gpk_cdiv(a.n, 128) + 1) / 2) * gpk_cdiv(a.m, 128) * (a.batch > 0 ? a.batch : 1);
+  return pairs < GPK_TUNE(PROJ_SMALL_TILE_BELOW, 200);
+}
+
+bool gpk_gemm_fuses_row_stats(const GemmArgs& a) {
+  if (a.epi != 1 || !a.stat_sumsq || !a.stat_mv || !a.stat_V || a.stat_P < 1 || a.stat_P > 4) return false;
+  if (a.m <= 0 || a.n <= 0 || a.k_off_step || a.a_tri || a.b_tri == 2 || (a.b_tri == 1 && a.b_tri_off != 0)) return false;
+  if ((a.beta != 0.0 && a.C) || a.batch != a.stat_P || (a.batch > 1 && a.strideA != 0)) return false;
+  return !proj_small_tiles(a) && fast_ok(a);
+}
+
 static int launch_select(hipStream_t s, const GemmArgs& a) {
+  if (a.stat_sumsq && !gpk_gemm_fuses_row_stats(a)) return GPK_E_UNSUPPORTED;
   const long tiles = (long)gpk_cdiv(a.m, 128) * gpk_cdiv(a.n, 128) * (a.batch > 0 ? a.batch : 1);
   if (a.tile64 && a.epi == 0) {
     if (GPK_TUNE(REST_PRE64, 1) && pre64_ok(a)) return launch_pre64(s, a);
@@ -1541,17 +1603,15 @@
     const long eff = a.c_lower ? tiles / 2 : tiles;
     if (eff < GPK_TUNE(HALF_TILE_BELOW, 300)) return launch_cfg<64, 128, 1, 4>(s, a);
   }
-  if (a.epi == 1 && a.b_tri == 1 && !(a.beta != 0.0 && a.C) && a.m > 64) {
+  if (proj_small_tiles(a)) {
     const long pairs = (long)((gpk_cdiv(a.n, 128) + 1) / 2) * gpk_cdiv(a.m, 128) * (a.batch > 0 ? a.batch : 1);
-    if (pairs < GPK_TUNE(PROJ_SMALL_TILE_BELOW, 200)) {
-      GemmArgs b = a;
-      b.tile_snake = GPK_TUNE(PROJ_SNAKE, 1);
-      if (gpk_cdiv(a.n, 64) == 2 * gpk_cdiv(a.n, 128)) {
-        if (pairs < GPK_TUNE(PROJ_TILE32_BELOW, 100)) return launch_cfg<32, 64, 2, 2>(s, b);
-        return launch_cfg<64, 64, 4, 1>(s, b);
-      }
-      return launch_cfg<64, 128, 2, 2>(s, b);
-    }
+    GemmArgs b = a;
+    b.tile_snake = GPK_TUNE(PROJ_SNAKE, 1);
+    if (gpk_cdiv(a.n, 64) == 2 * gpk_cdiv(a.n, 128)) {
+      if (pairs < GPK_TUNE(PROJ_TILE32_BELOW, 100)) return launch_cfg<32, 64, 2, 2>(s, b);
+      return launch_cfg<64, 64, 4, 1>(s, b);
+    }
+    return launch_cfg<64, 128, 2, 2>(s, b);
   }
   if (fast_ok(a) && (a.epi == 1 || (a.n > 64 && (tiles >= 24 || a.m <= 64)))) {
     return a.epi == 1 ? launch_fast<1>(s, a) : launch_fast<0>(s, a);
diff --git a/gpflow_amd/csrc/gpk_internal.h b/gpflow_amd/csrc/gpk_internal.h
--- a/gpflow_amd/csrc/gpk_internal.h
+++ b/gpflow_amd/csrc/gpk_internal.h
@@ -68,6 +68,7 @@
   int sq_cols;
   double* part; long part_ld; long stridePart;
   double* C2; long ldc2; long strideC2; int c2_cols;
+  double* stat_sumsq; double* stat_mv; const double* stat_V; int stat_P;
   int batch;
   int stagger_first;
   int stagger_ticks;
@@ -97,6 +98,7 @@
 }
 int gpk_launch_gemm(hipStream_t s, const GemmArgs& a);
 bool gpk_gemm_takes_latency_kernel(const GemmArgs& a);
+bool gpk_gemm_fuses_row_stats(const GemmArgs& a);
 
 int gpk_launch_group_solve(hipStream_t s, const double* E, long lde, double* Eo, long ldeo, int rows, const double* Lgg, long ldl,
                            const double* X, int nb, int batch = 1, long strideE = 0, long strideEo = 0, long strideL = 0,
@@ -137,8 +139,11 @@
                                         int rows, int P, const double* s0, int s0_per_latent, const double* ssq,
                                         const double* knn_host, int knn_per_latent, double mean_const, double* fvar_out,
                                         double* rows_out, double* dmu_out, double* dvar_out, double* part, double* part1, int* count);
+int gpk_launch_varexp_tail(hipStream_t s, const double* Y, long ldy, const double* fmean, int rows, int P, const double* s0,
+                           const double* slot, int nt, long strideSlot, double knn, double noise, double mean_const,
+                           const double* noise_rows, double* part, int* ticket, double* out);
 int gpk_launch_kl_white_stage1(hipStream_t s, const double* q_mu, const double* q_sqrt, int m, int P,
-                               int q_diag, double* part, int* count);
+                               int q_diag, double* part, int* count, int* zero_word = nullptr);
 int gpk_launch_kl_unwhite_diag_stage1(hipStream_t s, const double* LinvT, long ldl, int m, const double* W, int P, double* part,
                                       int* count);
 int gpk_launch_sum_log_diag_sq(hipStream_t s, const double* L, int n, long ldl, int batch, long strideL, double* out);
diff --git a/gpflow_amd/csrc/reduce.hip b/gpflow_amd/csrc/reduce.hip
--- a/gpflow_amd/csrc/reduce.hip
+++ b/gpflow_amd/csrc/reduce.hip
@@ -227,9 +227,12 @@
   double knn[16]; int knn_per_latent;
   double noise, mean_const; double* fvar_out; double* part;
   const double* noise_rows;
+  const double* slot; int nt; long strideSlot; int* ticket; double* out;
 };
+template <bool TAIL>
 __global__ __launch_bounds__(RB) void varexp_kernel(VarexpArgs a) {
   __shared__ double sh[4];
+  __shared__ int s_last;
   const double log2pi = 1.8378770664093453;
   const double c0 = -0.5 * log2pi - 0.5 * log(a.noise);
   double acc = 0.0;
@@ -238,7 +241,20 @@
     const int b = (int)(e / a.P), p = (int)(e - (long)b * a.P);
     double fv = a.knn[a.knn_per_latent ? p : 0];
     if (a.s0) fv -= a.s0_per_latent ? a.s0[(long)p * a.rows + b] : a.s0[b];
-    if (a.ssq) fv += a.ssq[(long)p * a.rows + b];
+    if constexpr (TAIL) {
+      const double* q = a.slot + (long)p * a.strideSlot + b;
+      double s = 0.0;
+      int t = 0;
+      for (; t + 16 <= a.nt; t += 16) {
+        double v[16];
+#pragma unroll
+        for (int i = 0; i < 16; ++i) v[i] = q[(long)(t + i) * a.rows];
+#pragma unroll
+        for (int i = 0; i < 16; ++i) s += v[i];
+      }
+      for (; t < a.nt; ++t) s += q[(long)t * a.rows];
+      fv += s;
+    } else if (a.ssq) fv += a.ssq[(long)p * a.rows + b];
     const double mu = a.fmean[e] + a.mean_const;
     const double dy = a.Y[(long)b * a.ldy + p] - mu;
     if (a.fvar_out) a.fvar_out[e] = fv;
@@ -251,6 +267,19 @@
   }
   const double r = block_sum(acc, sh);
   if (threadIdx.x == 0) a.part[blockIdx.x] = r;
+  if constexpr (TAIL) {
+    if (threadIdx.x == 0) {
+      __threadfence();
+      s_last = atomicAdd(a.ticket, 1) == (int)gridDim.x - 1;
+    }
+    __syncthreads();
+    if (!s_last) return;
+    __threadfence();
+    double v = 0.0;
+    for (int i = threadIdx.x; i < (int)gridDim.x; i += RB) v += __hip_atomic_load(a.part + i, __ATOMIC_RELAXED, __HIP_MEMORY_SCOPE_AGENT);
+    const double t = block_sum(v, sh);
+    if (threadIdx.x == 0) *a.out = 0.0 + 1.0 * t;
+  }
 }
 
 #define GPK_GH20_X                                                                                                          \
@@ -364,8 +393,9 @@
 }
 
 __global__ __launch_bounds__(RB) void kl_white_kernel(const double* q_mu, const double* q_sqrt, int m,
-                                                      int P, int q_diag, double* part) {
+                                                      int P, int q_diag, double* part, int* zero_word) {
   __shared__ double sh[4];
+  if (zero_word && blockIdx.x == 0 && threadIdx.x == 0) *zero_word = 0;
   double acc = 0.0;
   const long nmu = (long)m * P;
   const long stride = (long)gridDim.x * RB, start = (long)blockIdx.x * RB + threadIdx.x;
@@ -644,7 +674,7 @@
   a.knn_per_latent = knn_per_latent; a.noise = noise_variance; a.mean_const = mean_const;
   a.fvar_out = fvar_out; a.part = (double*)ws; a.noise_rows = noise_rows;
   const int nb = nblocks_for((long)rows * P);
-  hipLaunchKernelGGL(varexp_kernel, dim3(nb), dim3(RB), 0, (hipStream_t)stream, a);
+  hipLaunchKernelGGL(varexp_kernel<false>, dim3(nb), dim3(RB), 0, (hipStream_t)stream, a);
   GPK_LAUNCH_CHECK();
   FinalArgs f{};
   f.nterms = 1; f.part[0] = a.part; f.count[0] = nb; f.scale[0] = 1.0; f.add = 0.0; f.out = out;
@@ -731,7 +761,7 @@
   const int nb = nblocks_for(elems);
   double* part = (double*)ws;
   hipLaunchKernelGGL(kl_white_kernel, dim3(nb), dim3(RB), 0, (hipStream_t)stream, q_mu, q_sqrt, m, P,
-                     q_diag, part);
+                     q_diag, part, (int*)nullptr);
   GPK_LAUNCH_CHECK();
   FinalArgs f{};
   f.nterms = 1; f.part[0] = part; f.count[0] = nb; f.scale[0] = 0.5;
@@ -832,16 +862,31 @@
   a.knn_per_latent = knn_per_latent; a.noise = noise; a.mean_const = mean_const;
   a.fvar_out = fvar_out; a.part = part; a.noise_rows = noise_rows;
   const int nb = nblocks_for((long)rows * P);
-  hipLaunchKernelGGL(varexp_kernel, dim3(nb), dim3(RB), 0, s, a);
+  hipLaunchKernelGGL(varexp_kernel<false>, dim3(nb), dim3(RB), 0, s, a);
   GPK_LAUNCH_CHECK();
   *count = nb;
   return 0;
 }
+int gpk_launch_varexp_tail(hipStream_t s, const double* Y, long ldy, const double* fmean, int rows, int P, const double* s0,
+                           const double* slot, int nt, long strideSlot, double knn, double noise, double mean_const,
+                           const double* noise_rows, double* part, int* ticket, double* out) {
+  if (!slot || !part || !ticket || !out || nt < 0) return GPK_E_ARG;
+  VarexpArgs a{};
+  a.Y = Y; a.ldy = ldy; a.fmean = fmean; a.rows = rows; a.P = P;
+  a.s0 = s0; a.knn[0] = knn; a.noise = noise; a.mean_const = mean_const;
+  a.part = part; a.noise_rows = noise_rows;
+  a.slot = slot; a.nt = nt; a.strideSlot = strideSlot; a.ticket = ticket; a.out = out;
+  long nb = ((long)rows * P + RB - 1) / RB;
+  nb = nb < 1 ? 1 : (nb > MAXPART ? MAXPART : nb);
+  hipLaunchKernelGGL(varexp_kernel<true>, dim3((unsigned)nb), dim3(RB), 0, s, a);
+  GPK_LAUNCH_CHECK();
+  return 0;
+}
 int gpk_launch_kl_white_stage1(hipStream_t s, const double* q_mu, const double* q_sqrt, int m, int P,
-                               int q_diag, double* part, int* count) {
+                               int q_diag, double* part, int* count, int* zero_word) {
   const long elems = q_diag ? (long)m * P : (long)P * m * m;
   const int nb = nblocks_for(elems);
-  hipLaunchKernelGGL(kl_white_kernel, dim3(nb), dim3(RB), 0, s, q_mu, q_sqrt, m, P, q_diag, part);
+  hipLaunchKernelGGL(kl_white_kernel, dim3(nb), dim3(RB), 0, s, q_mu, q_sqrt, m, P, q_diag, part, zero_word);
   GPK_LAUNCH_CHECK();
   *count = nb;
   return 0;
diff --git a/gpflow_amd/ops.py b/gpflow_amd/ops.py
--- a/gpflow_amd/ops.py
+++ b/gpflow_amd/ops.py
@@ -364,6 +364,27 @@
                                  ssq.data_ptr(), ws.data_ptr(), ws.numel() * 8)
     _lib.check(rc, "gpk_project_batched")
     return ssq
+
+
+def project_stats(At: torch.Tensor, LqT: torch.Tensor, V: torch.Tensor):
+    lib = _lib.load()
+    _chk(At, "At", 2)
+    _chk(LqT, "LqT", 3)
+    _chk(V, "V", 2)
+    rows, m = At.shape
+    P = LqT.shape[0]
+    if LqT.shape[1] != m or LqT.shape[2] != m or not LqT.is_contiguous():
+        raise ValueError("LqT must be contiguous [P, m, m]")
+    if V.shape != (m, P) or not V.is_contiguous():
+        raise ValueError("V must be contiguous [m, P]")
+    s0 = torch.empty(rows, dtype=torch.float64, device=At.device)
+    fmean = torch.empty((rows, P), dtype=torch.float64, device=At.device)
+    ssq = torch.empty((P, rows), dtype=torch.float64, device=At.device)
+    ws = _ws(int(lib.gpk_project_workspace_bytes(rows, m, P)))
+    rc = lib.gpk_project_stats(_stream(), At.data_ptr(), rows, m, _rowmajor(At, "At"), LqT.data_ptr(), m, P, V.data_ptr(),
+                               s0.data_ptr(), fmean.data_ptr(), ssq.data_ptr(), ws.data_ptr(), ws.numel() * 8)
+    _lib.check(rc, "gpk_project_stats")
+    return s0, fmean, ssq
 
 
 def gaussian_varexp_sum(Y: torch.Tensor, fmean: torch.Tensor, *, s0: Optional[torch.Tensor],
diff --git a/include/gpk.h b/include/gpk.h
--- a/include/gpk.h
+++ b/include/gpk.h
@@ -76,6 +76,8 @@
                 long ldl, int P, double* ssq, void* ws, size_t ws_bytes);
 int gpk_project_batched(void* stream, const double* At, int rows, int m, long ldat, long strideAt,
                         const double* LqT, long ldl, int P, double* ssq, void* ws, size_t ws_bytes);
+int gpk_project_stats(void* stream, const double* At, int rows, int m, long ldat, const double* LqT, long ldl, int P,
+                      const double* V, double* s0, double* fmean, double* ssq, void* ws, size_t ws_bytes);
 
 size_t gpk_reduce_workspace_bytes(int n);
 int gpk_gaussian_varexp_sum(void* stream, const double* Y, long ldy, const double* fmean, int rows,
```
